# huangzh13/StyleGAN.pytorch

Hardware: AMD Instinct MI355X
Metric: img/s full G+D train step, 1024x1024 depth-9 bf16 (higher is better)
Workload: dtype bf16; 1 GPU; ffhq1024: StyleGAN 1024x1024, progressive depth index 8, logistic+R1, alpha 0.5, batch 4/GPU, global batch 4; global_batch=4, parallelism=dp1

## Files before the change

include/sgx.h:

```cpp
#ifndef SGX_H
#define SGX_H
#include <stddef.h>
#include <stdint.h>
#ifdef __cplusplus
extern "C" {
#endif

enum { SGX_F32 = 0, SGX_BF16 = 1 };
enum { SGX_ACT_NONE = 0, SGX_ACT_LRELU = 1, SGX_ACT_RELU = 2 };
enum { SGX_EINVAL = -1, SGX_EUNSUPPORTED = -2, SGX_EWORKSPACE = -3 };

int sgx_version(void);
const char* sgx_last_error(void);
int sgx_clear_error(void);
int sgx_stream_wait_stream(void* waiter, void* signaler);
int sgx_selftest_tr16(void* out256, void* stream);

int sgx_prof_start(int mode, int only_of);
int sgx_prof_count(void);
int sgx_prof_get(int i, char* name, int name_cap, float* ms, double* flops, double* bytes, char* desc, int desc_cap);

int sgx_conv3x3(const void* x, const void* w, const float* bias, void* y, int B, int H, int W, int Cin, int Cout,
                int act, const void* mask, int dtype, void* stream);
int sgx_conv4x4s2_down(const void* x, const void* w, const float* bias, void* y, int B, int H, int W, int Cin,
                       int Cout, int act, int dtype, void* stream);
int sgx_conv4x4s2_up(const void* x, const void* w, void* y, int B, int H, int W, int Cin, int Cout, int dtype,
                     void* stream);
int sgx_conv_variant(int geo, const void* x, const void* w, const float* bias, void* y, int B, int H, int W, int Cin, int Cout,
                     int act, int dtype, int variant, void* stream);
size_t sgx_conv_splitk_ws_bytes(int geo, int B, int H, int W, int Cin, int Cout, int dtype);
int sgx_conv_splitk(int geo, const void* x, const void* w, const float* bias, void* y, const void* mask, int B, int H, int W, int Cin, int Cout,
                    int act, int dtype, void* ws, size_t ws_bytes, void* stream);

int sgx_conv_config(int geo, int B, int H, int W, int Cin, int Cout, int dtype, int* cfg5);
enum { SGX_PACK_S = 0, SGX_PACK_D = 1, SGX_PACK_U = 2, SGX_PACK_UF = 3 };
int sgx_pack_weight(const float* w, void* fwd, void* adj, int O, int I, int Ipad, int mode, float scale, int dtype,
                    void* stream);
#define SGX_PACK_ROW 10
int sgx_pack_weight_blocks(int O, int Ipad);
int sgx_pack_weight_multi(const void* table, int n, int total_blocks, int dtype, void* stream);
size_t sgx_wgrad_ws_bytes(int taps, int B, int H, int W, int Ck, int Cn);
int sgx_wgrad3x3_param(const void* x, const void* dy, float* dW, float* db, void* ws, size_t ws_bytes, int B, int H, int W,
                       int Cx, int Cdy, int adjoint, float scale, int O, int I, int accumulate, int dtype, void* stream);
int sgx_wgrad4x4s2_param(const void* fine, const void* coarse, float* dW, float* db, void* ws, size_t ws_bytes, int B, int H,
                         int W, int Cfine, int Ccoarse, int mode, float scale, int O, int I, int accumulate, int dtype,
                         void* stream);

int sgx_bias_act(const void* x, const float* bias, float bscale, void* y, size_t npix, int C, int act, int dtype,
                 void* stream);
int sgx_lrelu_bwd(const void* dy, const void* y, void* dx, size_t n, float slope, float scale, const float* scale_dev, int dtype,
                  void* stream);
int sgx_lrelu_bwd_bits(const void* dy, const void* bits, void* dx, size_t n, float slope, float scale, const float* scale_dev, int dtype,
                       void* stream);
int sgx_conv4x4s2_down_fade_ok(int B, int H, int W, int Cin, int Cout, int dtype);
int sgx_conv4x4s2_down_fade(const void* x, const void* w, const float* bias, const void* resid, float alpha, float beta, const float* ab_dev,
                            void* y, void* bits, int B, int H, int W, int Cin, int Cout, int dtype, void* stream);
int sgx_conv4x4s2_down_fade_rgb(const void* x, const void* w, const float* bias, const float* pimg, const float* wr, float ws, const float* rb,
                                float bs1, float bs2, float alpha, float beta, const float* ab_dev, void* y, void* bits, int B, int H, int W,
                                int Cin, int Cout, int dtype, void* stream);
size_t sgx_fade_rgb_bwd_ws_bytes(size_t npix, int C);
int sgx_fade_rgb_bwd(const void* g, const void* bits, const float* pimg, const float* wr, float ws, float bs, float alpha, float beta,
                     const float* ab_dev, void* gy, float* dwr, float* drb, int acc, float* gpimg, void* wsbuf, size_t ws_bytes, size_t npix, int C,
                     int dtype, void* stream);
int sgx_fade_rgb_bwd_finish(const void* wsbuf, size_t ws_bytes, size_t npix, int C, float ws, float bs, float beta, const float* ab_dev,
                            float* dwr, float* drb, int acc, void* stream);
int sgx_fade_rgb_bwd2(const void* ggy, const float* ggp, const void* bits, const float* wr, float ws, float alpha, float beta, const float* ab_dev,
                      void* out, size_t npix, int C, int dtype, void* stream);
int sgx_axpby(const void* a, const void* b, void* out, float alpha, float beta, size_t n, int dtype, void* stream);
int sgx_axpby_dev(const void* a, const void* b, void* out, const float* alpha_dev, const float* beta_dev, size_t n, int dtype,
                  void* stream);
int sgx_blur3x3(const void* x, void* y, int B, int H, int W, int C, int dtype, void* stream);
int sgx_blur3x3_act(const void* x, const void* z, void* y, int B, int H, int W, int C, int mode, int dtype, void* stream);
int sgx_blur3x3_bits(const void* x, const void* bits, void* y, int B, int H, int W, int C, int mode, int dtype, void* stream);
int sgx_blur_kxk(const void* x, void* y, const float* taps_host, int K, int pad, int B, int IH, int IW, int OH, int OW, int C,
                 int dtype, void* stream);
int sgx_images_u8_to_nhwc(const void* src, void* dst, const int* flip, int B, int H, int W, int src_chw, int dtype, void* stream);
int sgx_pool2(const void* x, void* y, int B, int H, int W, int C, float scale, int dtype, void* stream);
int sgx_up2(const void* x, void* y, int B, int H, int W, int C, float scale, int dtype, void* stream);
int sgx_up2_add(const void* x, const void* a, void* y, int B, int H, int W, int C, float scale, int dtype, void* stream);
size_t sgx_colsum_ws_bytes(size_t npix, int C);
int sgx_colsum(const void* x, float* out, float scale, void* ws, size_t ws_bytes, size_t npix, int C, int dtype,
               void* stream);

int sgx_rgb_in(const float* img, const float* w, int sj, int sc, float wscale, const float* bias, void* y, size_t npix,
               int C, int dtype, void* stream);
int sgx_rgb_out(const void* x, const float* w, int sj, int sc, float wscale, const float* bias, float* img, size_t npix,
                int C, int dtype, void* stream);
int sgx_rgb_in_add(const float* img, const float* w, int sj, int sc, float wscale, const void* add, void* y, size_t npix, int C, int dtype,
                   void* stream);
size_t sgx_rgb_wgrad_ws_bytes(size_t npix, int C);
int sgx_downsample_fade_rgb(const float* x, float* out, int B, int H, int W, float alpha, float beta, const float* ab_dev, void* stream);
size_t sgx_diffaug_ws_bytes(int B, int H, int W);
int sgx_diffaug(const float* x, float* y, const float* u, int B, int H, int W, int policy_bits, int adjoint, int with_bias, void* ws,
                size_t ws_bytes, void* stream);
int sgx_ada_gates(const float* gu, const float* state, int policy_bits, int* img_bits, int B, void* stream);
int sgx_diffaug_gated(const float* x, float* y, const float* u, const int* img_bits, int B, int H, int W, int policy_bits, int adjoint,
                      int with_bias, void* ws, size_t ws_bytes, void* stream);
int sgx_ada_update(const float* real_logits, int B, float* state, float target, float adjust_per_image, int interval, void* stream);
int sgx_rgb_out_fade(const void* x, const float* w, int sj, int sc, float wscale, const float* bias, const float* low, float alpha,
                     float beta, const float* ab_dev, float* img, int B, int H, int W, int C, int dtype, void* stream);
int sgx_rgb_wgrad(const float* img, const void* f, float* dw, int sj, int sc, float wscale, void* ws, size_t ws_bytes,
                  size_t npix, int C, int dtype, void* stream);

enum { SGX_EPI_ACT = 1, SGX_EPI_NORM = 2 };
size_t sgx_gepi_ws_bytes(int B, int HW, int C);
int sgx_gepi_fwd(const void* x, const float* bias, const float* noise, const float* nw, const float* style, void* y,
                 float* mean, float* rstd, void* ws, size_t ws_bytes, const double* pre_part, int pre_npart, int B, int HW,
                 int C, int flags, int dtype, void* stream);
int sgx_blur3x3_stats_nparts(int B, int H, int W, int C, int dtype);
int sgx_conv3x3_stats_nparts(int B, int H, int W, int Cin, int Cout, int dtype);
int sgx_conv3x3_signbits_ok(int B, int H, int W, int Cin, int Cout, int dtype);
int sgx_conv3x3_signbits(const void* x, const void* w, const float* bias, void* y, void* bits, int B, int H, int W, int Cin, int Cout,
                         int act, const void* mask, int dtype, void* stream);
int sgx_conv4x4s2_up_blur_ok(int B, int H, int W, int Cin, int Cout, int dtype);
int sgx_conv4x4s2_up_blur(const void* x, const void* w, void* y, const void* mask, int B, int H, int W, int Cin, int Cout,
                          int dtype, void* stream);
int sgx_pack_upblur(const float* w, void* wc, int O, int I, int mode, int adjoint, float scale, void* stream);
int sgx_conv_upblur_ok(int B, int H, int W, int Cin, int Cout, int dtype);
int sgx_conv_upblur(const void* x, const void* wc, void* y, const void* maskbits, int B, int H, int W, int Cin, int Cout, int dtype, void* stream);
int sgx_conv4x4s2_up_blur_bits(const void* x, const void* w, void* y, const void* bits, int B, int H, int W, int Cin, int Cout,
                               int dtype, void* stream);
int sgx_conv3x3_stats(const void* x, const void* w, void* y, const float* ebias, const float* noise, const float* nw, double* part,
                      size_t part_bytes, int B, int H, int W, int Cin, int Cout, int dtype, void* stream);

int sgx_rgbconv_ok(int B, int H, int W, int C, int dtype);
int sgx_rgbconv_pack(const float* w0, float s0, const float* wr, float sr, const float* br, float bscale, void* wf, void* wd, int C,
                     void* stream);
int sgx_rgbconv_fwd(const float* img, const void* wf, const float* b0, void* y, void* bits, int B, int H, int W, int C, int epi, int ones,
                    int dtype, void* stream);
int sgx_rgbconv_tune(int fwd_variant, int nit, int dbg);
int sgx_rgbconv_dgrad(const void* gz, const void* wd, float* gi, int B, int H, int W, int C, int dtype, void* stream);
size_t sgx_rgbconv_wgrad_ws_bytes(int B, int H, int W, int C);
int sgx_rgbconv_wgrad(const float* img, const void* gz, int ones, const float* w0, float s0, const float* wr, float sr, const float* br,
                      float bscale, float* dw0, float* db0, float* dwr, float* dbr, int acc, void* ws, size_t ws_bytes, int B, int H, int W,
                      int C, int dtype, void* stream);
int sgx_blur3x3_stats(const void* x, void* y, const float* bias, const float* noise, const float* nw, double* part,
                      size_t part_bytes, int B, int H, int W, int C, int act, int dtype, void* stream);
int sgx_gepi_bwd(const void* dy, const void* x, const float* bias, const float* noise, const float* nw,
                 const float* style, const float* mean, const float* rstd, void* dx, float* dstyle, float* dnw,
                 float* dbias, void* ws, size_t ws_bytes, int B, int HW, int C, int flags, int dtype, void* stream);

int sgx_pixelnorm_fwd(const float* x, float* y, int B, int C, void* stream);
int sgx_pixelnorm_bwd(const float* dy, const float* x, float* dx, int B, int C, void* stream);
int sgx_mbstd_fwd(const void* x, void* y, int B, int HW, int C, int Cpad, int dtype, void* stream);
int sgx_mbstd_bwd(const void* dy, const void* x, void* dx, int B, int HW, int C, int Cpad, int dtype, void* stream);
int sgx_mbstd_bwd2(const void* ggx, const void* dy, const void* x, void* ddy, void* gx, int B, int HW, int C, int Cpad,
                   int dtype, void* stream);
size_t sgx_sumsq_ws_bytes(void);
int sgx_sumsq_f32(const float* x, size_t n, void* ws, size_t ws_bytes, float* out, void* stream);
int sgx_scale_dev_f32(const float* x, const float* s, float alpha, float* out, size_t n, void* stream);
int sgx_logistic_loss(const float* fake, int n_fake, const float* real, int n_real, float scale, int generator, float* loss,
                      float* g_fake, float* g_real, void* stream);
size_t sgx_gemm_ws_bytes(int M, int N, int K);
int sgx_gemm_f32(const float* A, const float* Bm, float* C, int M, int N, int K, int ta, int tb, float alpha,
                 void* ws, size_t ws_bytes, void* stream);
int sgx_linear_fwd(const float* x, const float* w, const float* bias, float* y, int B, int N, int K, float w_mul, float b_mul,
                   int act, void* stream);
int sgx_linear_bwd_data(const float* gy, const float* y_act, const float* w, float* gx, int B, int N, int K, float w_mul,
                        void* stream);
int sgx_linear_bwd_param(const float* gy, const float* y_act, const float* x, float* dw, float* db, int B, int N, int K, float w_mul,
                         float b_mul, void* stream);
#define SGX_STYLE_ROW 8
int sgx_style_fwd(const float* lm, const void* table, float* y, int G, int B, int D, int total_tiles, void* stream);
int sgx_style_bwd_data(const float* gy, const void* table, float* glm, int G, int B, int D, int max_n, void* stream);
int sgx_style_bwd_param(const float* gy, const float* lm, const void* table, float* dw, float* db, int G, int B, int D,
                        int total_tiles, void* stream);

int sgx_gepi_stats(const void* x, const float* bias, const float* noise, const float* nw, float* mean, float* rstd, void* ws, size_t ws_bytes,
                   const double* pre_part, int pre_npart, int B, int HW, int C, int flags, int dtype, void* stream);
int sgx_rgb_out_epi(const void* y, const float* ebias, const float* noise, const float* nw, const float* style, const float* mean,
                    const float* rstd, const float* w, int sj, int sc, float wscale, const float* rbias, const float* low, float alpha, float beta,
                    const float* ab_dev, float* img, int B, int H, int W, int C, int dtype, void* stream);
size_t sgx_rgb_wgrad_epi_ws_bytes(int B, int HW, int C);
int sgx_rgb_wgrad_epi(const void* y, const float* g, const float* ebias, const float* noise, const float* nw, const float* style, const float* mean,
                      const float* rstd, float* dw, float* db, int sj, int sc, float scale, float bscale, void* ws, size_t ws_bytes, int B, int HW,
                      int C, int dtype, void* stream);

int sgx_adam_multi(float* const* params, const float* const* grads, float* const* exp_avg, float* const* exp_avg_sq,
                   const int64_t* sizes, int n, float beta1, float beta2, float eps, const float* step_sizes,
                   const float* bc2_sqrts, const float* grad_scale, void* stream);
int sgx_ema_multi(float* const* tgt, const float* const* src, const int64_t* sizes, int n, float beta, void* stream);
int sgx_gradnorm_clip_coef(const float* const* grads, const int64_t* sizes, int n, float max_norm, double* partial,
                           float* out, void* stream);

#ifdef __cplusplus
}
#endif
#endif
```

stylegan/pytorch_amd/GAN.py:

```python
import contextlib
import copy
import datetime
import os
import random
import time
import timeit
from collections import OrderedDict

import numpy as np
import torch
import torch.nn as nn

from . import Losses
from . import functional as F
from .Blocks import DiscriminatorBlock, DiscriminatorTop, GSynthesisBlock, InputBlock
from .CustomLayers import EqualizedConv2d, EqualizedLinear, PixelNormLayer, Truncation, act_code, apply_act
from .data import get_data_loader
from . import native
from .native import ACT_LRELU
from .optim import FusedAdam, clip_and_step, ema_update


class DeferredLoss:

# ... 490 lines not shown
        if isinstance(loss, str):
            loss = loss.lower()
            mean_scale = 1.0 / self.dp.world_size if self.dp is not None else 1.0
            if self.conditional:
                assert loss in ["conditional-loss"]
                return Losses.ConditionalGANLoss(self.dis, mean_scale=mean_scale)
            assert loss in ["logistic", "hinge", "standard-gan", "relativistic-hinge"], "Unknown loss function"
            if loss == "logistic":
                return Losses.LogisticGAN(self.dis, mean_scale=mean_scale)
            if loss == "hinge":
                return Losses.HingeGAN(self.dis, mean_scale=mean_scale)
            if loss == "standard-gan":
                return Losses.StandardGAN(self.dis, mean_scale=mean_scale)
            return Losses.RelativisticAverageHingeGAN(self.dis, mean_scale=mean_scale,
                                                      batch_mean=self.dp.global_mean if self.dp is not None else None)
        return loss

    def progressive_down_sampling(self, real_batch, depth, alpha):
        if self.structure == 'fixed':
            return real_batch
        x = F.nhwc(real_batch, torch.float32)
        levels = self.depth - depth - 1
        for _ in range(levels):
            x = F.call(F.Pool2Fn, x, 0.25)
        if depth > 0:
            if FUSE_RGB_FADE and x.shape[3] == 3 and x.dtype == torch.float32 and not x.requires_grad:
                x = F.downsample_fade_rgb(x, alpha)
            else:
                prior = F.call(F.Up2Fn, F.call(F.Pool2Fn, x, 0.25), 1.0)
                x = F.fade(x, prior, alpha)
        else:
            x = F.fade(x, x, alpha)
        return F.nchw_view(x)

    _StyleGAN__progressive_down_sampling = progressive_down_sampling

    def _zero_grads(self, kind, depth):
        optim = self.dis_optim if kind == "d" else self.gen_optim
        optim.zero_grad()
        gb = self._grad_buckets.get((kind, int(depth))) if self.dp is not None else None
        if gb is not None:
            gb.attach()

    def _sched_begin(self, kind, depth, param_stream):
        from . import dist as D
        self.__dict__["_sched_active"] = None
        if self.dp is None or not self.dp.overlap_buckets or torch.cuda.is_current_stream_capturing():
            return
        if F.GRAD_NOTE is None:
            F.GRAD_NOTE = D.note_grad_write
        net = self.dis if kind == "d" else self.gen
        if not net.__dict__.get("_sgx_grad_hooks"):
            D.install_grad_hooks(net.parameters())
            net.__dict__["_sgx_grad_hooks"] = True
        scheds = self.__dict__.setdefault("_bucket_scheds", {})
        key = (kind, int(depth))
        sched = scheds.get(key)
        gb = self._grad_buckets.get(key)
        if sched is None or (not sched.recording and (gb is None or sched.gb is not gb or not gb.attached())):
            sched = scheds[key] = D.BucketScheduler(self.dp)
        if not sched.recording:
            sched.begin(param_stream)
        self.__dict__["_sched_active"] = sched
        D.set_active_scheduler(sched)

    def _sched_abort(self):
        if self.dp is not None:
            from . import dist as D
            D.set_active_scheduler(None)
            self.__dict__["_sched_active"] = None

    def _note_active_grads(self, kind, depth):
        if self.dp is None:
            return
        from . import dist as D
        D.set_active_scheduler(None)
        sched = self.__dict__.get("_sched_active")
        net = self.dis if kind == "d" else self.gen
        active = [p for p in net.parameters() if p.grad is not None]
        gb = self._grad_buckets.get((kind, int(depth)))
        recorded = sched is not None and sched.recording
        if active and (gb is None or not gb.matches(active) or recorded) and not torch.cuda.is_current_stream_capturing():
            for key in [k for k in self._grad_buckets if k[0] == kind and k[1] != int(depth)
                        and not any(g.depth == k[1] and g.graph is not None for g in self._step_graphs.values())]:
                del self._grad_buckets[key]
                self.__dict__.get("_bucket_scheds", {}).pop(key, None)
            new = None
            if sched is not None and sched.recording:
                new = sched.layout(self.dp.bucket_elems, only=active, canonical=list(net.parameters()))
                if new is None or not new.matches(active):
                    new = None
                    self.__dict__.get("_bucket_scheds", {}).pop((kind, int(depth)), None)
            self._grad_buckets[(kind, int(depth))] = new if new is not None else D.GradBuckets(active, self.dp.bucket_elems)
            self.__dict__["_sched_active"] = None

    def _aux_stream(self):
        if not self.aux_stream:
            return None
        st = self.__dict__.get("_aux_compute_stream")
        if st is None:
            st = self.__dict__["_aux_compute_stream"] = torch.cuda.Stream(device=self.device)
            quiet = getattr(torch.autograd.graph, "set_warn_on_accumulate_grad_stream_mismatch", None)
            if quiet is not None:
                quiet(False)
        return st

    def _param_stream(self, two_branches=False):
        if not self.param_stream:
            return torch.cuda.current_stream() if two_branches else None
        st = self.__dict__.get("_param_side_stream")
        if st is None:
            st = self.__dict__["_param_side_stream"] = torch.cuda.Stream(device=self.device)
        return st

    def _graphable(self, labels):
        return (self.use_graphs and labels is None and self.d_repeats == 1 and self.structure == "linear"
                and (self.dp is None or (self.gen.truncation is None
                                         and not isinstance(self.loss, Losses.RelativisticAverageHingeGAN))))

    def _d_grads(self, noise, real_batch, depth, alpha, labels=None):
        real_samples = self.progressive_down_sampling(real_batch, depth, alpha)

        def make_fakes():
            self._wait_update("g")
            with torch.no_grad():
                out = self.gen(noise, depth, alpha, labels)
            return out

        aux = self._aux_stream()
        lazy = isinstance(self.loss, Losses.LogisticGAN)
        self._wait_update("d")
        if aux is not None and lazy:
            self.dis.prepack(depth, (real_samples.shape[0], real_samples.shape[2], real_samples.shape[3], real_samples.shape[1]))
            cur = torch.cuda.current_stream()
            aux.wait_stream(cur)
            with torch.cuda.stream(aux):
                f_preds = self.dis(make_fakes(), depth, alpha)

            def fake_logits():
                cur.wait_stream(aux)
                f_preds.record_stream(cur)
                return f_preds
            loss = self.loss.dis_loss(real_samples, None, depth, alpha, fake_logits=fake_logits)
        elif self.conditional:
            loss = self.loss.dis_loss(real_samples, make_fakes(), labels, depth, alpha)
        else:
            loss = self.loss.dis_loss(real_samples, make_fakes if lazy else make_fakes(), depth, alpha)
        if self._ada_on():
            self.dis.ada_step()
        self._zero_grads("d", depth)
        side = self._param_stream(two_branches=aux is not None and lazy)
        self._sched_begin("d", depth, side)
        try:
            with F.accumulate_param_grads(), F.param_grad_stream(side):
                loss.backward()
        except BaseException:
            self._sched_abort()
            raise
        if side is not None:
            torch.cuda.current_stream().wait_stream(side)
        self._note_active_grads("d", depth)
        return loss.detach()

    def _reduce(self, kind):
        if self.dp is None:
            return
        sched = self.__dict__.pop("_sched_active", None)
        if sched is not None and not sched.recording and sched.gb is not None and sched.gb.attached():
            try:
                sched.finish()
            except RuntimeError:
                for key in [k for k, v in self.__dict__.get("_bucket_scheds", {}).items() if v is sched]:
                    self._bucket_scheds.pop(key, None)
                    self._grad_buckets.pop(key, None)
                raise
            self.__dict__["_last_sched"] = sched
            return
        gb = next((g for (k, _), g in self._grad_buckets.items() if k == kind and g.attached()), None)
        if gb is not None:
            self.dp.all_reduce_buckets(gb)
        else:
            self.dp.all_reduce_grads((self.dis if kind == "d" else self.gen).parameters())

    def _d_reduce(self):
        self._reduce("d")

    def _d_update(self):
        self.dis_optim.step()

    def _g_grads(self, noise, real_batch, depth, alpha, labels=None):
        real_samples = None
        if not isinstance(self.loss, (Losses.LogisticGAN, Losses.HingeGAN, Losses.StandardGAN, Losses.ConditionalGANLoss)):
            real_samples = self.progressive_down_sampling(real_batch, depth, alpha)
        self._wait_update("g")
        fake_samples = self.gen(noise, depth, alpha, labels)
        self._wait_update("d")
        d_all = self.__dict__.get("_sgx_dis_params")
        if d_all is None:
            d_all = self.__dict__["_sgx_dis_params"] = list(self.dis.parameters())
        d_params = [p for p in d_all if p.requires_grad]
        for p in d_params:
            p.requires_grad_(False)
        try:
            if self.conditional:
                loss = self.loss.gen_loss(real_samples, fake_samples, labels, depth, alpha)
            else:
                loss = self.loss.gen_loss(real_samples, fake_samples, depth, alpha)
            self._zero_grads("g", depth)
            side = self._param_stream()
            self._sched_begin("g", depth, side)
            try:
                with F.accumulate_param_grads(), F.param_grad_stream(side):
                    loss.backward()
            except BaseException:
                self._sched_abort()
                raise
            if side is not None:
                torch.cuda.current_stream().wait_stream(side)
            self._note_active_grads("g", depth)
        finally:
            for p in d_params:
                p.requires_grad_(True)
        return loss.detach()

    def _g_reduce(self):
        self._reduce("g")

    def _g_update(self):
        clip_and_step(self.gen_optim, max_norm=10.)
        if self.use_ema:
            self.ema_updater(self.gen_shadow, self.gen, self.ema_decay)

    def _async_update(self, kind, loss):
        upd = self.__dict__.get("_update_stream")
        if upd is None:
            upd = self.__dict__["_update_stream"] = torch.cuda.Stream(device=self.device)
        upd.wait_stream(torch.cuda.current_stream())
        with torch.cuda.stream(upd):
            (self._d_reduce if kind == "d" else self._g_reduce)()
            loss.record_stream(upd)
            loss = self.dp.all_reduce_scalar(loss)
            (self._d_update if kind == "d" else self._g_update)()
        ev = torch.cuda.Event()
        ev.record(upd)
        self.__dict__.setdefault("_pending_updates", {})[kind] = ev
        self.__dict__["_loss_stream"] = upd
        return loss

    def _wait_update(self, kind):
        ev = self.__dict__.get("_pending_updates", {}).pop(kind, None)
        if ev is not None:
            torch.cuda.current_stream().wait_event(ev)

    def _d_body(self, noise, real_batch, depth, alpha, labels=None):
        loss = self._d_grads(noise, real_batch, depth, alpha, labels)
        if self.dp is not None and not torch.cuda.is_current_stream_capturing():
            return self._async_update("d", loss)
        self._d_reduce()
        self._d_update()
        return loss

    def _g_body(self, noise, real_batch, depth, alpha, labels=None):
        loss = self._g_grads(noise, real_batch, depth, alpha, labels)
        if self.dp is not None and not torch.cuda.is_current_stream_capturing():
            return self._async_update("g", loss)
        self._g_reduce()
        self._g_update()
        return loss

    def _graphed(self, kind, noise, real_batch, depth, alpha):
        self._wait_update("d"); self._wait_update("g")
        key = (kind, int(depth), tuple(noise.shape), tuple(real_batch.shape), tuple(real_batch.stride()), real_batch.dtype,
               self.aux_stream, self.param_stream,
               self.dis._diffaug_bits, self.dis.training,
               None if self.dis.diffaug_override is None else self.dis.diffaug_override.data_ptr(),
               (self.dis.ada_target, self.dis.ada_interval, self.dis.ada_kimg) if self._ada_on() else None,
               None if not self._ada_on() or self.dis.ada_gate_override is None else self.dis.ada_gate_override.data_ptr())
        g = self._step_graphs.get(key)
        if g is None:
            g = self._step_graphs[key] = _StepGraph(self, kind, depth)
        return g.run(noise, real_batch, alpha)

    deferred_losses = False

    alpha_on_device = False

    def _alpha_arg(self, alpha):
        if not self.alpha_on_device or isinstance(alpha, torch.Tensor):
            return alpha
        return native.upload(torch.tensor([float(alpha), 1.0 - float(alpha)], dtype=torch.float32), self.device)[0]

    def _loss_out(self, deferred):
        return deferred if self.deferred_losses else deferred.item()

    def optimize_discriminator(self, noise, real_batch, depth, alpha, labels=None):
        if self._graphable(labels):
            return self._loss_out(self._graphed("d", noise, real_batch, depth, alpha))
        loss_val = None
        alpha = self._alpha_arg(alpha)
        for _ in range(self.d_repeats):
            loss = self._d_body(noise, real_batch, depth, alpha, labels)
            if loss_val is not None and self.__dict__.get("_loss_stream") is not None:
                torch.cuda.current_stream().wait_stream(self.__dict__.pop("_loss_stream"))
            loss_val = loss if loss_val is None else loss_val + loss
        return self._loss_out(DeferredLoss(loss_val, 1.0 / self.d_repeats, stream=self.__dict__.pop("_loss_stream", None)))

    def optimize_generator(self, noise, real_batch, depth, alpha, labels=None):
        if self._graphable(labels):
            return self._loss_out(self._graphed("g", noise, real_batch, depth, alpha))
        loss = self._g_body(noise, real_batch, depth, self._alpha_arg(alpha), labels)
        return self._loss_out(DeferredLoss(loss, stream=self.__dict__.pop("_loss_stream", None)))

    @staticmethod
    def fade_point_of(fade_in_percentage, epochs, total_batches):
        return int((fade_in_percentage / 100) * epochs * total_batches)

    @staticmethod
    def alpha_at(ticker, fade_point):
        return ticker / fade_point if ticker <= fade_point else 1

    @staticmethod
    def is_feedback_batch(i, total_batches, feedback_factor):
        return i % int(total_batches / feedback_factor + 1) == 0 or i == 1

    @staticmethod
    def is_checkpoint_epoch(epoch, epochs, checkpoint_factor):
        return epoch % checkpoint_factor == 0 or epoch == 1 or epoch == epochs

    @staticmethod
    def create_grid(samples, scale_factor, img_file):
        samples = samples.detach().float().cpu()
        if scale_factor > 1:
            samples = torch.nn.functional.interpolate(samples, scale_factor=scale_factor)
        n, c, h, w = samples.shape
        nrow = max(1, int(np.sqrt(n)))
        ncol = (n + nrow - 1) // nrow
        pad = 1
        grid = torch.full((c, ncol * (h + pad) + pad, nrow * (w + pad) + pad), 128.0)
        for k in range(n):
            t = samples[k]
            lo, hi = float(t.min()), float(t.max())
            t = (t - lo) / max(hi - lo, 1e-5)
            y, x = (k // nrow) * (h + pad) + pad, (k % nrow) * (w + pad) + pad
            grid[:, y:y + h, x:x + w] = t
        try:
            from PIL import Image
            arr = grid.mul(255).add_(0.5).clamp_(0, 255).permute(1, 2, 0).to(torch.uint8).numpy()
            Image.fromarray(arr[:, :, 0] if c == 1 else arr).save(img_file)
        except ImportError:
            torch.save(grid, img_file + ".pt")

    train_graphs = {"0": False, "1": True}.get(os.environ.get("SGX_TRAIN_GRAPHS", "auto"), "auto")

    def train(self, dataset, num_workers, epochs, batch_sizes, fade_in_percentage, logger, output,
              num_samples=36, start_depth=0, feedback_factor=100, checkpoint_factor=1):
        assert self.depth <= len(epochs), "epochs not compatible with depth"
        assert self.depth <= len(batch_sizes), "batch_sizes not compatible with depth"
        assert self.depth <= len(fade_in_percentage), "fade_in_percentage not compatible with depth"
        self.gen.train()
        self.dis.train()
        if self.use_ema:
            self.gen_shadow.train()
        was_deferred, self.deferred_losses = self.deferred_losses, True
        was_graphs = getattr(self, "use_graphs", False)
        self.use_graphs = bool(was_graphs or self.train_graphs is True)
        self._train_forced_graphs = self.use_graphs
# ... 282 lines not shown
```

stylegan/pytorch_amd/csrc/conv.hip:

```cpp
#include "common.h"
#include <stdlib.h>

enum { G3X3 = 0, GDOWN = 1, GUP = 2, GUPA = 3 };
int sgx_wgrad2_plan(int geo, int B, int H, int W, int Ck, int Cn, int* nct_n, int* nct_k, int* kbw, int* ntiles);
int sgx_wgrad2_launch(int geo, const void* kside, const void* nside, float* ws, size_t ws_bytes, int B, int H, int W, int Ck, int Cn,
                      int want_bias, hipStream_t st, int* nsplit_out);
int sgx_conv2_try(int geo, const void* x, const void* w, const float* bias, void* y, int B, int H, int W, int Cin, int Cout, int act,
                  const void* mask, int variant, hipStream_t st, int* launched);
int sgx_conv2_takes(int geo, int B, int H, int W, int Cin, int Cout);

template <typename T, int KC> struct Frag;
template <> struct Frag<float, 16> {
    static constexpr int NK = 4;
    static constexpr int rowb_w() { return 68; }
    static constexpr int rowb_in(int) { return 68; }
    static constexpr bool swz_w() { return false; }
    static constexpr bool swz_in(int) { return false; }
    typedef float frag_t;
    static constexpr int pad_pw(int pw, int) { return pw; }
    __device__ static __forceinline__ int rd_off(int row, int rowb, bool, int q) { return row * rowb + q * 4; }
    __device__ static __forceinline__ frag_t ld(const char* p, int kk) { return *reinterpret_cast<const float*>(p + kk * 16); }
    __device__ static __forceinline__ f32x4 mma(frag_t a, frag_t b, f32x4 c) {
        return __builtin_amdgcn_mfma_f32_16x16x4f32(a, b, c, 0, 0, 0);
    }
    __device__ static __forceinline__ int lds_off(int row, int rowb, bool, int v) { return row * rowb + v * 16; }
    __device__ static __forceinline__ void lstore_at(char* p, uint4 val) {
        unsigned* d = reinterpret_cast<unsigned*>(p);
        d[0] = val.x; d[1] = val.y; d[2] = val.z; d[3] = val.w;
    }
};
template <> struct Frag<bf16_t, 32> {
    static constexpr int NK = 1;
    static constexpr int rowb_w() { return 64; }
    static constexpr int rowb_in(int is) { return is == 1 ? 64 : 80; }
    static constexpr bool swz_w() { return true; }
    static constexpr bool swz_in(int is) { return is == 1; }
    typedef bf16x8 frag_t;
    static constexpr int pad_pw(int pw, int is) { return is == 1 ? (pw + 7) / 8 * 8 : pw; }
    __device__ static __forceinline__ int rd_off(int row, int rowb, bool sw, int q) {
        return row * rowb + (sw ? (q ^ ((row >> 1) & 3)) : q) * 16;
    }
    __device__ static __forceinline__ frag_t ld(const char* p, int) { return *reinterpret_cast<const bf16x8*>(p); }
    __device__ static __forceinline__ f32x4 mma(frag_t a, frag_t b, f32x4 c) {
        return __builtin_amdgcn_mfma_f32_16x16x32_bf16(a, b, c, 0, 0, 0);
    }
    __device__ static __forceinline__ int lds_off(int row, int rowb, bool sw, int v) {
        return row * rowb + (sw ? (v ^ ((row >> 1) & 3)) : v) * 16;
    }
    __device__ static __forceinline__ void lstore_at(char* p, uint4 val) { *reinterpret_cast<uint4*>(p) = val; }
};
template <> struct Frag<bf16_t, 16> {
    static constexpr int NK = 1;
    static constexpr int rowb_w() { return 32; }
    static constexpr int rowb_in(int is) { return is == 1 ? 32 : 48; }
    static constexpr bool swz_w() { return true; }
    static constexpr bool swz_in(int is) { return is == 1; }
    typedef s16x4 frag_t;
    static constexpr int pad_pw(int pw, int is) { return is == 1 ? (pw + 15) / 16 * 16 : pw; }
    __device__ static __forceinline__ int rd_off(int row, int rowb, bool sw, int q) {
        const int half = sw ? ((q >> 1) ^ ((row >> 3) & 1)) : (q >> 1);
        return row * rowb + half * 16 + (q & 1) * 8;
    }
    __device__ static __forceinline__ frag_t ld(const char* p, int) { return *reinterpret_cast<const s16x4*>(p); }
    __device__ static __forceinline__ f32x4 mma(frag_t a, frag_t b, f32x4 c) {
        return __builtin_amdgcn_mfma_f32_16x16x16bf16_1k(a, b, c, 0, 0, 0);
    }
    __device__ static __forceinline__ int lds_off(int row, int rowb, bool sw, int v) {
        return row * rowb + (sw ? (v ^ ((row >> 3) & 1)) : v) * 16;
    }
    __device__ static __forceinline__ void lstore_at(char* p, uint4 val) { *reinterpret_cast<uint4*>(p) = val; }
};

struct ConvArgs {
    const void* x; const void* w; const float* bias; void* y;
    int B, H, W, OH, OW, OHc, OWc, Cin, Cout, act, tiles_x, tiles_y, ntiles;
    const void* mask;
    int dbg;
    int bands;
    int ksplit; float* kws;
};

template <int GEO> struct Geo;
template <> struct Geo<G3X3> { static constexpr int IS = 1, TK = 3, NCLS = 1; };
template <> struct Geo<GDOWN> { static constexpr int IS = 2, TK = 4, NCLS = 1; };
template <> struct Geo<GUP> { static constexpr int IS = 1, TK = 2, NCLS = 4; };
template <> struct Geo<GUPA> { static constexpr int IS = 1, TK = 3, NCLS = 1; };

#ifndef SGX_CONV_OCC_SMALL
#define SGX_CONV_OCC_SMALL 3
#endif
constexpr int conv_min_waves(int tsize, int CT, int BP, int GEO, int KC) {
    if (KC > 32) return 2;
    if (GEO == GUPA) return CT * BP >= 512 ? 1 : 2;
    if (GEO == GDOWN && tsize == 2 && KC == 16) return 3;
    if (CT * BP >= 1024 || GEO == GDOWN) return 1;
    if (tsize == 2 && CT * BP <= 256) return SGX_CONV_OCC_SMALL;
    return 2;
}
template <typename T>
constexpr bool conv_bands_ok(int GEO, int TH, int TW, int BP) {
    return sizeof(T) == 2 && (GEO == G3X3 || GEO == GUPA) && TH == 16 && TW == 16 && BP == 256;
}
template <typename T, int KC, int GEO, int TH, int TW, int BP, int CT, bool SK = false>
__global__ __launch_bounds__(256, conv_min_waves(sizeof(T), CT, BP, GEO, KC)) void conv_kernel(ConvArgs a) {
    constexpr int FK = (sizeof(T) == 2 && KC > 32) ? 32 : KC;
    constexpr int NPL = KC / FK;
    using F = Frag<T, FK>;
    constexpr int IS = Geo<GEO>::IS, TK = Geo<GEO>::TK, NT = TK * TK;
    constexpr int PH = (TH - 1) * IS + TK, PW = (TW - 1) * IS + TK, PWP = F::pad_pw(PW, IS);
    constexpr int NI = BP / (TH * TW), SPW = BP / 64, BCO = CT * 16;
    constexpr int VE = 16 / (int)sizeof(T), VPP = KC / VE, VPR = FK / VE;
    constexpr int ROWI = F::rowb_in(IS), ROWW = F::rowb_w();
    constexpr bool SWI = F::swz_in(IS), SWW = F::swz_w();
    constexpr bool UPA = GEO == GUPA;
    constexpr int NTW = UPA ? 16 : NT;
    constexpr int NCL = UPA ? 4 : 1;
    constexpr int IN_PLANE = (NI * PH * PWP * ROWI + 15) / 16 * 16, W_PLANE = NTW * BCO * ROWW;
    constexpr int IN_BYTES = NPL * IN_PLANE;
    extern __shared__ __attribute__((aligned(16))) char smem[];
    char* in_lds = smem;
    char* w_lds = smem + IN_BYTES;

    const int tid = threadIdx.x, lane = tid & 63, wave = tid >> 6, q = lane >> 4, l15 = lane & 15;
    const int co0 = blockIdx.y * BCO;
    int py = 0, px = 0;
    constexpr int NCLS_Z = Geo<GEO>::NCLS;
    if (GEO == GUP) { py = (SK ? (int)(blockIdx.z % NCLS_Z) : (int)blockIdx.z) >> 1; px = blockIdx.z & 1; }
    int split = 0, k_lo = 0, k_hi = a.Cin;
    if constexpr (SK) {
        const int nkc = a.Cin / KC;
        split = (int)blockIdx.z / NCLS_Z;
        k_lo = (split * nkc / a.ksplit) * KC; k_hi = ((split + 1) * nkc / a.ksplit) * KC;
    }
    constexpr int NIN = (NI * PH * PW * VPP + 255) / 256, NWT = (NTW * BCO * VPP + 255) / 256;
    int in_rel[NIN], in_pos[NIN], in_dst[NIN], w_rel[NWT];
    const int w_dst0 = ((tid % VPP) / VPR) * W_PLANE + F::lds_off(tid / VPP, ROWW, SWW, (tid % VPP) % VPR);
#pragma unroll
    for (int j = 0; j < NIN; ++j) {
        const int idx = tid + j * 256;
        const int v = idx % VPP, pixel = idx / VPP;
        const int il = pixel / (PH * PW), rem = pixel % (PH * PW);
        const int pr = rem / PW, pc = rem % PW;
        const bool in_range = idx < NI * PH * PW * VPP;
        in_rel[j] = ((il * a.H + pr) * a.W + pc) * a.Cin + v * VE;
        in_pos[j] = in_range ? ((il << 20) | (pr << 10) | pc) : -1;
        in_dst[j] = (v / VPR) * IN_PLANE + F::lds_off((il * PH + pr) * PWP + pc, ROWI, SWI, v % VPR);
    }
#pragma unroll
    for (int j = 0; j < NWT; ++j) {
        const int idx = tid + j * 256;
        const int v = idx % VPP, row = idx / VPP;
        const int n = row % BCO, t = row / BCO;
        int tg = t;
        if (GEO == GUP) tg = (3 - py - 2 * (t >> 1)) * 4 + (3 - px - 2 * (t & 1));
// ... 706 lines not shown
        for (int j = 0; j < NNV; ++j) {
            const int idx = tid + j * 256;
            if (idx < BP * (NCH / VE)) *reinterpret_cast<uint4*>(n_lds + (idx / (NCH / VE)) * NROW + (idx % (NCH / VE)) * 16) = rn[j];
        }
#pragma unroll
        for (int j = 0; j < NKV; ++j) {
            const int idx = tid + j * 256;
            if (idx < NI * PH * PW * (KCH / VE)) *reinterpret_cast<uint4*>(k_lds + (idx / (KCH / VE)) * KROW + (idx % (KCH / VE)) * 16) = rk[j];
        }
    };
    if ((int)blockIdx.y < a.ntiles) gload(blockIdx.y);
    for (int tile = blockIdx.y; tile < a.ntiles; tile += gridDim.y) {
        __syncthreads();
        lstore();
        __syncthreads();
        if (tile + (int)gridDim.y < a.ntiles) gload(tile + gridDim.y);
        if constexpr (TR) {
            for (int ks = 0; ks < BP / 32; ++ks) {
                int noff2[2], koff2[2];
#pragma unroll
                for (int h = 0; h < 2; ++h) {
                    const int m = ks * 32 + h * 16 + q * 4 + (l15 >> 2);
                    const int il = m / (TH * TW), r = (m / TW) % TH, c = m % TW;
                    noff2[h] = m * NROW + (l15 & 3) * 8;
                    koff2[h] = ((il * PH + r * IS) * PW + c * IS) * KROW + (l15 & 3) * 8;
                }
                bf16x8 fa8[NSUB];
#pragma unroll
                for (int ns = 0; ns < NSUB; ++ns)
                    fa8[ns] = cat8(lds_tr16(n_lds + noff2[0] + ns * 32), lds_tr16(n_lds + noff2[1] + ns * 32));
                if (do_bias) {
                    const bf16x8 one8 = cat8(WFrag<bf16_t>::ones(), WFrag<bf16_t>::ones());
#pragma unroll
                    for (int ns = 0; ns < NSUB; ++ns) bacc[ns] = __builtin_amdgcn_mfma_f32_16x16x32_bf16(fa8[ns], one8, bacc[ns], 0, 0, 0);
                }
#pragma unroll
                for (int i = 0; i < TPW; ++i) {
                    const int t = wave + 4 * i;
                    if (t < NT) {
                        const int toff = ((t / TK) * PW + (t % TK)) * KROW;
#pragma unroll
                        for (int kk = 0; kk < KSUB; ++kk) {
                            const bf16x8 fb8 = cat8(lds_tr16(k_lds + toff + koff2[0] + kk * 32), lds_tr16(k_lds + toff + koff2[1] + kk * 32));
#pragma unroll
                            for (int ns = 0; ns < NSUB; ++ns)
                                acc[i][ns][kk] = __builtin_amdgcn_mfma_f32_16x16x32_bf16(fa8[ns], fb8, acc[i][ns][kk], 0, 0, 0);
                        }
                    }
                }
            }
        } else
        for (int ks = 0; ks < BP / F::KPS; ++ks) {
            int noff[4], koff[4];
#pragma unroll
            for (int j = 0; j < PPL; ++j) {
                const int m = ks * F::KPS + q * PPL + j;
                const int il = m / (TH * TW), r = (m / TW) % TH, c = m % TW;
                noff[j] = m * NROW;
                koff[j] = ((il * PH + r * IS) * PW + c * IS) * KROW;
            }
            typename F::frag_t fa[NSUB];
#pragma unroll
            for (int ns = 0; ns < NSUB; ++ns) fa[ns] = F::load(n_lds, noff, q, ns * 16 + l15);
            if (do_bias) {
#pragma unroll
                for (int ns = 0; ns < NSUB; ++ns) bacc[ns] = F::mma(fa[ns], F::ones(), bacc[ns]);
            }
#pragma unroll
            for (int i = 0; i < TPW; ++i) {
                const int t = wave + 4 * i;
                if (t < NT) {
                    const int toff = ((t / TK) * PW + (t % TK)) * KROW;
#pragma unroll
                    for (int kk = 0; kk < KSUB; ++kk) {
                        typename F::frag_t fb = F::load(k_lds + toff, koff, q, kk * 16 + l15);
#pragma unroll
                        for (int ns = 0; ns < NSUB; ++ns) acc[i][ns][kk] = F::mma(fa[ns], fb, acc[i][ns][kk]);
                    }
                }
            }
        }
    }
    if (a.direct) {
        constexpr int KP = KCH + 1;
        float* accl = reinterpret_cast<float*>(smem);
        __syncthreads();
#pragma unroll
        for (int i = 0; i < TPW; ++i) {
            const int t = wave + 4 * i;
            if (t < NT) {
#pragma unroll
                for (int ns = 0; ns < NSUB; ++ns)
#pragma unroll
                    for (int kk = 0; kk < KSUB; ++kk)
#pragma unroll
                        for (int r = 0; r < 4; ++r) accl[(t * NCH + ns * 16 + q * 4 + r) * KP + kk * 16 + l15] = acc[i][ns][kk][r];
            }
        }
        __syncthreads();
        const float c = a.scale * (a.mode == SGX_PACK_D ? 0.25f : 1.f);
        for (int idx = tid; idx < NCH * KCH * 9; idx += 256) {
            const int tap = idx % 9, kl = (idx / 9) % KCH, nl = idx / (9 * KCH);
            const int n = n0 + nl, k = kc0 + kl;
            const int o = a.transposed ? k : n, i = a.transposed ? n : k;
            if (i >= a.I || o >= a.O) continue;
            float v;
            if (NT == 9) {
                v = accl[((a.flip_t ? 8 - tap : tap) * NCH + nl) * KP + kl];
            } else {
                const int y = tap / 3, x = tap % 3;
                const float* pp = accl + nl * KP + kl;
                v = (pp[(y * 4 + x) * NCH * KP] + pp[(y * 4 + x + 1) * NCH * KP]) +
                    (pp[((y + 1) * 4 + x) * NCH * KP] + pp[((y + 1) * 4 + x + 1) * NCH * KP]);
            }
            float* d = a.dw + ((size_t)o * a.I + i) * 9 + (a.mode == SGX_PACK_UF ? 8 - tap : tap);
            *d = (a.accumulate & 1) ? *d + c * v : c * v;
        }
        if (do_bias && l15 == 0) {
#pragma unroll
            for (int ns = 0; ns < NSUB; ++ns)
#pragma unroll
                for (int r = 0; r < 4; ++r) {
                    float* d = a.db + n0 + ns * 16 + q * 4 + r;
                    *d = (a.accumulate & 2) ? *d + bacc[ns][r] : bacc[ns][r];
                }
        }
        return;
    }
    float* out = a.out + (size_t)blockIdx.y * ((size_t)NT * a.Cn * a.Ck + a.Cn);
    if (do_bias && l15 == 0) {
#pragma unroll
        for (int ns = 0; ns < NSUB; ++ns)
#pragma unroll
            for (int r = 0; r < 4; ++r) out[(size_t)NT * a.Cn * a.Ck + n0 + ns * 16 + q * 4 + r] = bacc[ns][r];
    }
#pragma unroll
    for (int i = 0; i < TPW; ++i) {
        const int t = wave + 4 * i;
        if (t < NT) {
#pragma unroll
            for (int ns = 0; ns < NSUB; ++ns)
#pragma unroll
                for (int kk = 0; kk < KSUB; ++kk)
#pragma unroll
                    for (int r = 0; r < 4; ++r)
                        out[((size_t)t * a.Cn + n0 + ns * 16 + q * 4 + r) * a.Ck + kc0 + kk * 16 + l15] = acc[i][ns][kk][r];
        }
    }
}

struct FinishArgs { const float* ws; float* dw; float* db; int nsplit, O, I, Ip, mode, transposed, flip_t; float scale; int accumulate; };

template <int EPB>
__global__ __launch_bounds__(256) void wgrad_finish_kernel(FinishArgs f) {
    constexpr int NSL = 256 / EPB;
    __shared__ float red[NSL][EPB][9];
    const int pl = threadIdx.x % EPB, sl = threadIdx.x / EPB;
    const int A = f.transposed ? f.Ip : f.O, Bd = f.transposed ? f.O : f.Ip;
    const int e = blockIdx.x * EPB + pl;
    const int taps = f.mode == SGX_PACK_S ? 9 : 16;
    const size_t tstride = (size_t)f.O * f.Ip, total = (size_t)taps * tstride + A;
    if ((int)blockIdx.x >= (A * Bd + EPB - 1) / EPB) {
        const int o = ((int)blockIdx.x - (A * Bd + EPB - 1) / EPB) * EPB + pl;
        float b = 0.f;
        if (o < f.O)
            for (int s = sl; s < f.nsplit; s += NSL) b += f.ws[(size_t)s * total + (size_t)taps * tstride + o];
        red[sl][pl][0] = b;
        __syncthreads();
        if (sl == 0 && o < f.O) {
            float sum = 0.f;
            for (int l = 0; l < NSL; ++l) sum += red[l][pl][0];
            f.db[o] = (f.accumulate & 2) ? f.db[o] + sum : sum;
        }
        return;
    }
    float acc[9];
#pragma unroll
    for (int k = 0; k < 9; ++k) acc[k] = 0.f;
    if (e < A * Bd) {
#pragma unroll 4
        for (int s = sl; s < f.nsplit; s += NSL) {
            const float* p = f.ws + (size_t)s * total + e;
            if (f.mode == SGX_PACK_S) {
#pragma unroll
                for (int t = 0; t < 9; ++t) acc[t] += p[(size_t)(f.flip_t ? 8 - t : t) * tstride];
            } else {
                float v[16];
#pragma unroll
                for (int t = 0; t < 16; ++t) v[t] = p[(size_t)t * tstride];
#pragma unroll
                for (int y = 0; y < 3; ++y)
#pragma unroll
                    for (int x = 0; x < 3; ++x)
                        acc[y * 3 + x] += (v[y * 4 + x] + v[y * 4 + x + 1]) + (v[(y + 1) * 4 + x] + v[(y + 1) * 4 + x + 1]);
            }
        }
    }
#pragma unroll
    for (int k = 0; k < 9; ++k) red[sl][pl][k] = acc[k];
    __syncthreads();
    for (int t = threadIdx.x; t < EPB * 9; t += 256) {
        const int el = t / 9, k = t % 9;
        const int ee = blockIdx.x * EPB + el;
        if (ee >= A * Bd) continue;
        const int a = ee / Bd, bb = ee % Bd;
        const int o = f.transposed ? bb : a, i = f.transposed ? a : bb;
        if (i >= f.I) continue;
        float sum = 0.f;
#pragma unroll 8
        for (int l = 0; l < NSL; ++l) sum += red[l][el][k];
        const float c = f.scale * (f.mode == SGX_PACK_D ? 0.25f : 1.f);
        float* d = f.dw + ((size_t)o * f.I + i) * 9 + (f.mode == SGX_PACK_UF ? 8 - k : k);
        *d = (f.accumulate & 1) ? *d + c * sum : c * sum;
    }
}

static int wgrad_nsplit(int pairs, int ntiles, size_t elems_per_split) {
    static const int env_target = [] { const char* e = getenv("SGX_WGRAD_BLOCKS"); return e && atoi(e) > 0 ? atoi(e) : 0; }();
    static const int env_cap = [] { const char* e = getenv("SGX_WGRAD_MAXSPLIT"); return e && atoi(e) > 0 ? atoi(e) : 0; }();
    const bool tiny = elems_per_split <= (size_t)16 * 32 * 32;
    static const int env_mid = [] { const char* e = getenv("SGX_WGRAD_BLOCKS_MID"); return e && atoi(e) > 0 ? atoi(e) : 0; }();
    const int target = env_target ? env_target : (tiny ? 2048 : (env_mid ? env_mid : 512)), cap = env_cap ? env_cap : (tiny ? 1024 : 512);
    int want = (target + pairs - 1) / pairs;
    if (!env_target && pairs >= 512 && ntiles <= 64) want = 1;
    if (want > cap) want = cap;
    if (want > ntiles) want = ntiles;
    if (want < 1) want = 1;
    return want;
}

template <typename T, int GEO, int TH, int TW, int BP, int NSUB, int KSUB, bool TR>
static int launch_wgrad(WgradArgs& a, void* ws, size_t ws_bytes, int* nsplit_out, hipStream_t st) {
    using F = WFrag<T>;
    constexpr int IS = Geo<GEO>::IS, TK = Geo<GEO>::TK, NT = TK * TK;
    constexpr int PH = (TH - 1) * IS + TK, PW = (TW - 1) * IS + TK, NI = BP / (TH * TW);
    constexpr int OPER = BP * wgrad_pitch<T>(NSUB * 16, TR, 1) + NI * PH * PW * wgrad_pitch<T>(KSUB * 16, TR, IS);
    constexpr int FOLD = NT * NSUB * 16 * (KSUB * 16 + 1) * 4;
    constexpr int LDS = OPER > FOLD ? OPER : FOLD;
    static_assert(LDS <= 160 * 1024, "LDS budget");
    a.tiles_y = (a.Hn + TH - 1) / TH; a.tiles_x = (a.Wn + TW - 1) / TW;
    a.ntiles = ((a.B + NI - 1) / NI) * a.tiles_y * a.tiles_x;
    const int pairs = (a.Cn / (NSUB * 16)) * (a.Ck / (KSUB * 16));
    int nsplit = wgrad_nsplit(pairs, a.ntiles, (size_t)NT * a.Cn * a.Ck);
    const size_t total = (size_t)NT * a.Cn * a.Ck + a.Cn;
    size_t fit = ws_bytes / (total * sizeof(float));
    if ((size_t)nsplit > fit) nsplit = (int)fit;
    SGX_REQUIRE(nsplit >= 1, SGX_EWORKSPACE, "wgrad: workspace too small (%zu bytes, need >= %zu)", ws_bytes, total * sizeof(float));
    a.out = static_cast<float*>(ws);
    a.direct = (nsplit == 1 && a.dw != nullptr) ? 1 : 0;
    auto kern = wgrad_kernel<T, GEO, TH, TW, BP, NSUB, KSUB, TR>;
    sgx_lds_opt_in<wgrad_kernel<T, GEO, TH, TW, BP, NSUB, KSUB, TR>>(LDS);
    hipLaunchKernelGGL(kern, dim3(pairs, nsplit), dim3(256), LDS, st, a);
    SGX_LAUNCH_CHECK("wgrad_kernel");
    *nsplit_out = nsplit;
    return 0;
}

template <typename T, int GEO, int BP, int NSUB, int KSUB, bool TR>
static int wgrad_tile(WgradArgs& a, void* ws, size_t wsb, int* ns, hipStream_t st) {
    if (a.Hn >= 16 && a.Wn >= 16) return launch_wgrad<T, GEO, BP / 16, 16, BP, NSUB, KSUB, TR>(a, ws, wsb, ns, st);
    if (a.Hn >= 8 && a.Wn >= 8) return launch_wgrad<T, GEO, (BP >= 64 ? 8 : BP / 8), 8, BP, NSUB, KSUB, TR>(a, ws, wsb, ns, st);
    return launch_wgrad<T, GEO, (BP >= 16 ? 4 : BP / 4), 4, BP, NSUB, KSUB, TR>(a, ws, wsb, ns, st);
}

static bool wgrad_use_tr() {
    static const int v = [] { const char* e = getenv("SGX_WGRAD_TR"); return e ? atoi(e) : 1; }();
    return v != 0;
}

template <typename T, int GEO, int BP, bool TR = false>
static int wgrad_ch(WgradArgs& a, void* ws, size_t wsb, int* ns, hipStream_t st) {
    SGX_REQUIRE(a.Cn % 16 == 0 && a.Ck % 16 == 0, SGX_EUNSUPPORTED, "wgrad: channels must be multiples of 16");
    const bool n32 = a.Cn % 32 == 0, k32 = a.Ck % 32 == 0;
    if (GEO == GDOWN) {
        if (n32) return wgrad_tile<T, GEO, BP, 2, 1, TR>(a, ws, wsb, ns, st);
        return wgrad_tile<T, GEO, BP, 1, 1, TR>(a, ws, wsb, ns, st);
    }
    const long npix = (long)a.B * a.Hn * a.Wn;
    const bool lowres_big = npix <= 64L * BP && (long)(a.Cn / 32) * (a.Ck / 32) < 512 && (long)(a.Cn / 32) * (a.Ck / 16) >= 512;
    if (n32 && k32 && !lowres_big) return wgrad_tile<T, GEO, BP, 2, 2, TR>(a, ws, wsb, ns, st);
    if (n32) return wgrad_tile<T, GEO, BP, 2, 1, TR>(a, ws, wsb, ns, st);
    if (k32) return wgrad_tile<T, GEO, BP, 1, 2, TR>(a, ws, wsb, ns, st);
    return wgrad_tile<T, GEO, BP, 1, 1, TR>(a, ws, wsb, ns, st);
}

static int wgrad_pre_groups() { static const int v = [] { const char* e = getenv("SGX_WGRAD_PRE"); return e ? atoi(e) : 32; }(); return v; }
static int wgrad_pre_min() { static const int v = [] { const char* e = getenv("SGX_WGRAD_PRE_MIN"); return e ? atoi(e) : 256; }(); return v; }
__global__ __launch_bounds__(256) void wgrad_prereduce_kernel(const float* __restrict__ ws, float* __restrict__ out, size_t total4,
                                                              int nsplit) {
    const size_t e = (size_t)blockIdx.x * 256 + threadIdx.x;
    if (e >= total4) return;
    const int g = blockIdx.y, per = (nsplit + (int)gridDim.y - 1) / (int)gridDim.y;
    const int s0 = g * per, s1 = (s0 + per < nsplit) ? s0 + per : nsplit;
    float4 acc = make_float4(0.f, 0.f, 0.f, 0.f);
#pragma unroll 4
    for (int sp = s0; sp < s1; ++sp) {
        const float4 v = reinterpret_cast<const float4*>(ws)[(size_t)sp * total4 + e];
        acc.x += v.x; acc.y += v.y; acc.z += v.z; acc.w += v.w;
    }
    reinterpret_cast<float4*>(out)[(size_t)g * total4 + e] = acc;
}
static size_t wgrad_pre_bytes(size_t total_floats, int nsplit) {
    const int G = wgrad_pre_groups();
    return (G > 0 && nsplit >= wgrad_pre_min() && nsplit > G && total_floats % 4 == 0) ? (size_t)G * total_floats * sizeof(float) : 0;
}

static int wgrad_finish(const void* ws, float* dw, float* db, int nsplit, int O, int I, int Ip, int mode, int transposed, int flip_t,
                        float scale, int accumulate, hipStream_t st, size_t ws_bytes = 0) {
    {
        const size_t total = (size_t)(mode == SGX_PACK_S ? 9 : 16) * O * Ip + (transposed ? Ip : O);
        const size_t pre = wgrad_pre_bytes(total, nsplit), used = (size_t)nsplit * total * sizeof(float);
        if (pre && ws_bytes >= used + pre) {
            float* out = reinterpret_cast<float*>(const_cast<char*>(static_cast<const char*>(ws)) + used);
            hipLaunchKernelGGL(wgrad_prereduce_kernel, dim3((unsigned)((total / 4 + 255) / 256), wgrad_pre_groups()), dim3(256), 0, st,
                               static_cast<const float*>(ws), out, total / 4, nsplit);
            SGX_LAUNCH_CHECK("wgrad_prereduce_kernel");
            ws = out;
            nsplit = wgrad_pre_groups();
        }
    }
    FinishArgs f{static_cast<const float*>(ws), dw, db, nsplit, O, I, Ip, mode, transposed, flip_t, scale, accumulate};
    SGX_NOTE(0.0, 4.0 * ((double)nsplit * (mode == SGX_PACK_S ? 9 : 16) * O * Ip + 9.0 * O * I), "finish %dx%d m%d tr%d ns%d", O, I, mode, transposed, nsplit);
    const int ne = O * Ip, nb = db ? O : 0;
    if (ne / 64 >= 128) hipLaunchKernelGGL(wgrad_finish_kernel<64>, dim3((unsigned)((ne + 63) / 64 + (nb + 63) / 64)), dim3(256), 0, st, f);
    else if (ne / 16 >= 128) hipLaunchKernelGGL(wgrad_finish_kernel<16>, dim3((unsigned)((ne + 15) / 16 + (nb + 15) / 16)), dim3(256), 0, st, f);
    else if (ne / 8 >= 128) hipLaunchKernelGGL(wgrad_finish_kernel<8>, dim3((unsigned)((ne + 7) / 8 + (nb + 7) / 8)), dim3(256), 0, st, f);
    else hipLaunchKernelGGL(wgrad_finish_kernel<4>, dim3((unsigned)((ne + 3) / 4 + (nb + 3) / 4)), dim3(256), 0, st, f);
    SGX_LAUNCH_CHECK("wgrad_finish_kernel");
    return 0;
}

extern "C" size_t sgx_wgrad_ws_bytes(int taps, int B, int H, int W, int Ck, int Cn) {
    size_t total = ((size_t)taps * Ck * Cn + Cn) * sizeof(float);
    int pairs = (Ck / 32 > 0 ? Ck / 32 : 1) * (Cn / 32 > 0 ? Cn / 32 : 1);
    size_t ntiles = (size_t)B * ((H + 3) / 4) * ((W + 3) / 4);
    size_t ns = (size_t)wgrad_nsplit(pairs, ntiles > (1u << 30) ? (1 << 30) : (int)ntiles, (size_t)taps * Ck * Cn);
    size_t need = total * ns + wgrad_pre_bytes(total / sizeof(float), (int)ns);
    int a0, a1, a2, a3;
    const int ns2 = taps == 9 ? sgx_wgrad2_plan(0, B, H, W, Ck, Cn, &a0, &a1, &a2, &a3) : sgx_wgrad2_plan(1, B, H / 2, W / 2, Ck, Cn, &a0, &a1, &a2, &a3);
    const size_t need2 = ns2 ? total * ns2 + wgrad_pre_bytes(total / sizeof(float), ns2) : 0;
    return need > need2 ? need : need2;
}

extern "C" int sgx_wgrad3x3_param(const void* x, const void* dy, float* dW, float* db, void* ws, size_t ws_bytes, int B, int H,
                                  int W, int Cx, int Cdy, int adjoint, float scale, int O, int I, int accumulate, int dtype,
                                  void* stream) {
    hipStream_t st = (hipStream_t)stream;
    const int Ip = adjoint ? Cdy : Cx;
    SGX_REQUIRE(!db || !adjoint, SGX_EINVAL, "wgrad3x3_param: bias gradient asked of the adjoint launch");
    SGX_REQUIRE((adjoint ? Cx : Cdy) == O && Ip >= I, SGX_EINVAL, "wgrad3x3_param: channel mismatch (Cx=%d Cdy=%d O=%d I=%d adj=%d)", Cx, Cdy, O, I, adjoint);
    WgradArgs a{x, dy, nullptr, B, H, W, H, W, Cx, Cdy, 0, 0, 0, db ? 1 : 0,
                0, dW, db, O, I, SGX_PACK_S, adjoint, adjoint, accumulate, scale};
    SGX_NOTE(2.0 * 9 * Cx * Cdy * B * H * W, (dtype == SGX_F32 ? 4.0 : 2.0) * B * H * W * (Cx + Cdy), "wgradS B%d %dx%d %dx%d", B, H, W, Cx, Cdy);
    int ns = 0, rc;
    if (dtype == SGX_BF16) {
        rc = sgx_wgrad2_launch(0, x, dy, static_cast<float*>(ws), ws_bytes, B, H, W, Cx, Cdy, db ? 1 : 0, st, &ns);
        if (rc) return rc;
        if (ns) return wgrad_finish(ws, dW, db, ns, O, I, Ip, SGX_PACK_S, adjoint, adjoint, scale, accumulate, st, ws_bytes);
    }
    if (dtype == SGX_F32) rc = wgrad_ch<float, G3X3, 128>(a, ws, ws_bytes, &ns, st);
    else if (dtype == SGX_BF16) rc = wgrad_use_tr() ? wgrad_ch<bf16_t, G3X3, 128, true>(a, ws, ws_bytes, &ns, st) : wgrad_ch<bf16_t, G3X3, 128>(a, ws, ws_bytes, &ns, st);
    else { SGX_REQUIRE(false, SGX_EINVAL, "wgrad3x3_param: bad dtype"); }
    if (rc) return rc;
    if (a.direct) return 0;
    return wgrad_finish(ws, dW, db, ns, O, I, Ip, SGX_PACK_S, adjoint, adjoint, scale, accumulate, st, ws_bytes);
}

extern "C" int sgx_wgrad4x4s2_param(const void* fine, const void* coarse, float* dW, float* db, void* ws, size_t ws_bytes, int B,
                                    int H, int W, int Cfine, int Ccoarse, int mode, float scale, int O, int I, int accumulate,
                                    int dtype, void* stream) {
    hipStream_t st = (hipStream_t)stream;
    SGX_REQUIRE(H % 2 == 0 && W % 2 == 0, SGX_EINVAL, "wgrad4x4s2_param: odd fine size");
    SGX_REQUIRE(mode == SGX_PACK_D || mode == SGX_PACK_U || mode == SGX_PACK_UF, SGX_EINVAL, "wgrad4x4s2_param: bad mode %d", mode);
    const int transposed = mode != SGX_PACK_D;
    SGX_REQUIRE(!db || !transposed, SGX_EINVAL, "wgrad4x4s2_param: bias gradient only for mode D (dy is the coarse side)");
    SGX_REQUIRE(transposed ? (Ccoarse == I && Cfine == O) : (Ccoarse == O && Cfine == I), SGX_EINVAL,
                "wgrad4x4s2_param: channel mismatch (fine %d coarse %d O %d I %d mode %d)", Cfine, Ccoarse, O, I, mode);
    WgradArgs a{fine, coarse, nullptr, B, H, W, H / 2, W / 2, Cfine, Ccoarse, 0, 0, 0, db ? 1 : 0,
                0, dW, db, O, I, mode, transposed, 0, accumulate, scale};
    SGX_NOTE(2.0 * 16 * Cfine * Ccoarse * B * (H / 2) * (W / 2), (dtype == SGX_F32 ? 4.0 : 2.0) * B * H * W * (Cfine + Ccoarse / 4.0), "wgradD B%d fine%dx%d %dx%d", B, H, W, Cfine, Ccoarse);
    int ns = 0, rc;
    if (dtype == SGX_BF16) {
        rc = sgx_wgrad2_launch(1, fine, coarse, static_cast<float*>(ws), ws_bytes, B, H / 2, W / 2, Cfine, Ccoarse, db ? 1 : 0, st, &ns);
        if (rc) return rc;
        if (ns) return wgrad_finish(ws, dW, db, ns, O, I, I, mode, transposed, 0, scale, accumulate, st, ws_bytes);
    }
    if (dtype == SGX_F32) rc = wgrad_ch<float, GDOWN, 64>(a, ws, ws_bytes, &ns, st);
    else if (dtype == SGX_BF16) rc = wgrad_use_tr() ? wgrad_ch<bf16_t, GDOWN, 64, true>(a, ws, ws_bytes, &ns, st) : wgrad_ch<bf16_t, GDOWN, 64>(a, ws, ws_bytes, &ns, st);
    else { SGX_REQUIRE(false, SGX_EINVAL, "wgrad4x4s2_param: bad dtype"); }
    if (rc) return rc;
    if (a.direct) return 0;
    return wgrad_finish(ws, dW, db, ns, O, I, I, mode, transposed, 0, scale, accumulate, st, ws_bytes);
}

#define PACK_T 32
__device__ __forceinline__ float pack_tap(const float (*raw)[PACK_T][PACK_T + 1], int r, int il, int t, int mode, float scale) {
    if (mode == SGX_PACK_S) return scale * raw[t][r][il];
    const int ky = t >> 2, kx = t & 3;
    float v = 0.f;
#pragma unroll
    for (int a = 0; a < 2; ++a)
#pragma unroll
        for (int b = 0; b < 2; ++b) {
            const int y = ky - a, x = kx - b;
            if (y >= 0 && y < 3 && x >= 0 && x < 3) v += raw[mode == SGX_PACK_UF ? (2 - y) * 3 + (2 - x) : y * 3 + x][r][il];
        }
    return v * scale * (mode == SGX_PACK_D ? 0.25f : 1.f);
}
template <typename T>
__device__ __forceinline__ void pack_weight_tile(const float* __restrict__ w, T* __restrict__ fwd, T* __restrict__ adj, int O, int I,
                                                 int Ip, int mode, float scale, unsigned tile) {
    __shared__ float raw[9][PACK_T][PACK_T + 1];
    const int tiles_i = (Ip + PACK_T - 1) / PACK_T;
    const int o0 = (int)(tile / tiles_i) * PACK_T, i0 = (int)(tile % tiles_i) * PACK_T;
    const int ni = (I - i0 < PACK_T ? (I - i0 > 0 ? I - i0 : 0) : PACK_T);
    if (ni == PACK_T && (I * 9) % 4 == 0 && ((size_t)i0 * 9) % 4 == 0) {
        constexpr int PER = PACK_T * (PACK_T * 9 / 4) / 256;
        static_assert(PER * 256 == PACK_T * (PACK_T * 9 / 4), "a tile is a whole number of 16-byte loads per thread");
        float4 v[PER];
#pragma unroll
        for (int u = 0; u < PER; ++u) {
            const int idx = threadIdx.x + u * 256, r = idx / (PACK_T * 9 / 4), c4 = (idx % (PACK_T * 9 / 4)) * 4;
            v[u] = *reinterpret_cast<const float4*>(w + ((size_t)(o0 + r < O ? o0 + r : O - 1) * I + i0) * 9 + c4);
        }
#pragma unroll
        for (int u = 0; u < PER; ++u) {
            const int idx = threadIdx.x + u * 256, r = idx / (PACK_T * 9 / 4), c4 = (idx % (PACK_T * 9 / 4)) * 4;
            const bool ok = o0 + r < O;
            const float e[4] = {ok ? v[u].x : 0.f, ok ? v[u].y : 0.f, ok ? v[u].z : 0.f, ok ? v[u].w : 0.f};
#pragma unroll
            for (int j = 0; j < 4; ++j) raw[(c4 + j) % 9][r][(c4 + j) / 9] = e[j];
        }
    } else
    for (int idx = threadIdx.x; idx < PACK_T * PACK_T * 9; idx += blockDim.x) {
        const int r = idx / (PACK_T * 9), c = idx % (PACK_T * 9);
        const int il = c / 9, k = c % 9;
        float v = 0.f;
        if (o0 + r < O && il < ni) v = w[((size_t)(o0 + r) * I + i0) * 9 + c];
        raw[k][r][il] = v;
    }
    __syncthreads();
    const int taps = mode == SGX_PACK_S ? 9 : 16;
    constexpr int VE = 16 / (int)sizeof(T), VPR = PACK_T / VE;
    const bool full = (o0 + PACK_T <= O) && (i0 + PACK_T <= Ip) && (O % VE == 0) && (Ip % VE == 0);
    if (full) {
        for (int e = threadIdx.x; e < taps * PACK_T * VPR; e += blockDim.x) {
            const int t = e / (PACK_T * VPR), r = (e / VPR) % PACK_T, v = e % VPR;
            float val[VE];
#pragma unroll
            for (int j = 0; j < VE; ++j) val[j] = pack_tap(raw, r, v * VE + j, t, mode, scale);
            VecTraits<T>::store(fwd + ((size_t)t * O + o0 + r) * Ip + i0 + v * VE, val);
        }
        for (int e = threadIdx.x; e < taps * PACK_T * VPR; e += blockDim.x) {
            const int t = e / (PACK_T * VPR), il = (e / VPR) % PACK_T, v = e % VPR;
            const int ta = mode == SGX_PACK_S ? 8 - t : t;
            float val[VE];
#pragma unroll
            for (int j = 0; j < VE; ++j) val[j] = pack_tap(raw, v * VE + j, il, t, mode, scale);
            VecTraits<T>::store(adj + ((size_t)ta * Ip + i0 + il) * O + o0 + v * VE, val);
        }
        return;
    }
    for (int e = threadIdx.x; e < taps * PACK_T * PACK_T; e += blockDim.x) {
        const int t = e / (PACK_T * PACK_T), r = (e / PACK_T) % PACK_T, il = e % PACK_T;
        if (o0 + r < O && i0 + il < Ip)
            fwd[((size_t)t * O + o0 + r) * Ip + i0 + il] = from_f<T>(pack_tap(raw, r, il, t, mode, scale));
    }
    for (int e = threadIdx.x; e < taps * PACK_T * PACK_T; e += blockDim.x) {
        const int t = e / (PACK_T * PACK_T), il = (e / PACK_T) % PACK_T, r = e % PACK_T;
        const int ta = mode == SGX_PACK_S ? 8 - t : t;
        if (o0 + r < O && i0 + il < Ip)
            adj[((size_t)ta * Ip + i0 + il) * O + o0 + r] = from_f<T>(pack_tap(raw, r, il, t, mode, scale));
    }
}
static inline unsigned pack_tiles(int O, int Ip) { return (unsigned)(((O + PACK_T - 1) / PACK_T) * ((Ip + PACK_T - 1) / PACK_T)); }
template <typename T>
__global__ __launch_bounds__(256) void pack_weight_kernel(const float* __restrict__ w, T* __restrict__ fwd, T* __restrict__ adj, int O,
                                                          int I, int Ip, int mode, float scale) {
    pack_weight_tile<T>(w, fwd, adj, O, I, Ip, mode, scale, blockIdx.x);
}
template <typename T>
// ... 36 lines not shown
```

stylegan/pytorch_amd/functional.py:

```python
import contextlib
import functools
import os
import weakref

import numpy as np
import torch
from torch.autograd import Function
from torch.autograd.function import once_differentiable

from . import native as N

_DATA_GRAD_ONLY = 0


@contextlib.contextmanager
def data_grad_only():
    global _DATA_GRAD_ONLY
    _DATA_GRAD_ONLY += 1
    try:
        yield
    finally:
        _DATA_GRAD_ONLY -= 1


def _c(t):
    return t if t.is_contiguous() else t.contiguous()


class _NoGradCtx:
    needs_input_grad = (False,) * 16
    saved_tensors = ()

    def save_for_backward(self, *tensors):
        pass

    def mark_non_differentiable(self, *tensors):
        pass

    def set_materialize_grads(self, value):
        pass


def call(fn, *args):
    if torch.is_grad_enabled():
        for a in args:
            if isinstance(a, torch.Tensor) and a.requires_grad:
                return fn.apply(*args)
    return fn.forward(_NoGradCtx(), *args)


_bcall = call if os.environ.get("SGX_BWD_BYPASS", "1") != "0" else (lambda fn, *args: fn.apply(*args))


MODES = {"S": N.PACK_S, "D": N.PACK_D, "U": N.PACK_U, "UF": N.PACK_UF}
FWD_GEO = {"S": "S", "D": "D", "U": "U", "UF": "U"}
ADJ_GEO = {"S": "S", "D": "U", "U": "D", "UF": "D"}
_PACKS = {}
GRAD_NOTE = None
_WEIGHT_GEN = 0
_ACCUM_PARAM_GRADS = False
_PARAM_GRAD_STREAM = None


@contextlib.contextmanager
def param_grad_stream(stream):
    global _PARAM_GRAD_STREAM
    prev, _PARAM_GRAD_STREAM = _PARAM_GRAD_STREAM, stream
    try:
        yield
    finally:
        _PARAM_GRAD_STREAM = prev


_FAST_FORK = os.environ.get("SGX_FAST_FORK", "1") != "0"
_STREAMS = {}
_set_stream = torch._C._cuda_setStream if hasattr(torch._C, "_cuda_setStream") else None


def _stream_of(raw):
    st = _STREAMS.get(raw)
    if st is None:
        st = _STREAMS[raw] = torch.cuda.current_stream()
        assert st.cuda_stream == raw
    return st


def _param_grads(mode, adjoint, x, gy, weight, scale, want_bias, into):
    side = _PARAM_GRAD_STREAM
    if side is None:
        return _wgrad_param(mode, adjoint, x, gy, weight, scale, want_bias, into)
    if not _FAST_FORK:
        cur = torch.cuda.current_stream()
        side.wait_stream(cur)
        with torch.cuda.stream(side):
            dW, db = _wgrad_param(mode, adjoint, x, gy, weight, scale, want_bias, into)
        for t in (x, gy):
            t.record_stream(side)
        for t in (dW, db):
            if t is not None:
                t.record_stream(cur)
        return dW, db
    cur_raw = N.stream()
    if side.cuda_stream == cur_raw:
        return _wgrad_param(mode, adjoint, x, gy, weight, scale, want_bias, into)
    cur = _stream_of(cur_raw)
    N.check(N.lib().sgx_stream_wait_stream(side.cuda_stream, cur_raw), "sgx_stream_wait_stream")
    _set_stream(stream_id=side.stream_id, device_index=side.device_index, device_type=side.device_type)
    try:
        dW, db = _wgrad_param(mode, adjoint, x, gy, weight, scale, want_bias, into)
    finally:
        _set_stream(stream_id=cur.stream_id, device_index=cur.device_index, device_type=cur.device_type)
    x.record_stream(side); gy.record_stream(side)
    dW.record_stream(cur)
    if db is not None:
        db.record_stream(cur)
    return dW, db


def _fork_to(side, cur_raw, launch, reads=(), fresh=()):
    if not _FAST_FORK or _set_stream is None:
        cur = torch.cuda.current_stream()
        side.wait_stream(cur)
        with torch.cuda.stream(side):
            launch()
    else:
        cur = _stream_of(cur_raw)
        N.check(N.lib().sgx_stream_wait_stream(side.cuda_stream, cur_raw), "sgx_stream_wait_stream")
        _set_stream(stream_id=side.stream_id, device_index=side.device_index, device_type=side.device_type)
        try:
            launch()
        finally:
            _set_stream(stream_id=cur.stream_id, device_index=cur.device_index, device_type=cur.device_type)
    for t in reads:
        t.record_stream(side)
    for t in fresh:
        t.record_stream(cur)


@contextlib.contextmanager
def accumulate_param_grads():
    global _ACCUM_PARAM_GRADS
    prev, _ACCUM_PARAM_GRADS = _ACCUM_PARAM_GRADS, True
    try:
        yield
    finally:
        _ACCUM_PARAM_GRADS = prev


def bump_weight_generation(params=None):
    global _WEIGHT_GEN
    if params is None:
        _WEIGHT_GEN += 1
        return
    for p in params:
        p._sgx_gen = getattr(p, "_sgx_gen", 0) + 1


def _pack_tag(weight):
    return (weight._version, _WEIGHT_GEN, getattr(weight, "_sgx_gen", 0), weight.data_ptr())


def _pack_alloc(weight, sub):
    mode, _, ipad, dtype = sub
    taps = 9 if mode == "S" else 16
    O = weight.shape[0]
    return (torch.empty((taps, O, ipad), dtype=dtype, device=weight.device), torch.empty((taps, ipad, O), dtype=dtype, device=weight.device))


def _pack_mark():
    ev = torch.cuda.Event()
    ev.record()
    raw = N.stream()
    return (ev, raw, {raw})


def prepack(weights):
    rows, blk, dtype, touched = [], 0, None, []
    for w in weights:
        ent = _PACKS.get(id(w))
        if ent is None or ent[0]() is not w or not ent[3]:
            continue
        tag = _pack_tag(w)
        if ent[1] == tag:
            continue
        if w.dtype != torch.float32 or not w.is_contiguous():
            raise N.SgxError("parameters must be contiguous fp32")
        ent[1], ent[2] = tag, {}
        touched.append(ent)
        for sub in ent[3]:
            if dtype is None:
                dtype = sub[3]
            if sub[3] != dtype:
                continue
            fwd, adj = _pack_alloc(w, sub)
            ent[2][sub] = (fwd, adj)
            O, I = w.shape[0], w.shape[1]
            nb = ((O + 31) // 32) * ((sub[2] + 31) // 32)
            rows.append([w.data_ptr(), fwd.data_ptr(), adj.data_ptr(), O, I, sub[2], MODES[sub[0]],
                         int(np.float32(sub[1]).view(np.uint32)), blk, nb])
            blk += nb
    if rows:
        table, _ = N.upload(torch.tensor(rows, dtype=torch.int64), weights[0].device)
        N.check(N.lib().sgx_pack_weight_multi(N.ptr(table), len(rows), blk, N.F32 if dtype == torch.float32 else N.BF16, N.stream()),
                "sgx_pack_weight_multi")
        if not N.capturing():
            table.record_stream(torch.cuda.current_stream())
        mark = _pack_mark()
        for ent in touched:
            ent[4] = mark


def packs(weight, mode, scale, ipad, dtype):
    key = id(weight)
    ent = _PACKS.get(key)
    tag = _pack_tag(weight)
    if ent is None or ent[0]() is not weight:
        ent = [weakref.ref(weight, lambda _r, k=key: _PACKS.pop(k, None)), tag, {}, set(), None]
        _PACKS[key] = ent
    elif ent[1] != tag:
        ent[1], ent[2] = tag, {}
    sub = (mode, float(scale), int(ipad), dtype)
    ent[3].add(sub)
    got = ent[2].get(sub)
    if got is not None and ent[4] is not None:
        raw = N.stream()
        if raw not in ent[4][2] or (not _FAST_FORK and raw != ent[4][1]):
            _stream_of(raw).wait_event(ent[4][0])
            ent[4][2].add(raw)
    if got is None:
        w = _c(weight.detach())
        if w.dtype != torch.float32:
            raise N.SgxError("parameters must be fp32")
        O, I = w.shape[0], w.shape[1]
        fwd, adj = _pack_alloc(w, sub)
        N.check(N.lib().sgx_pack_weight(N.ptr(w), N.ptr(fwd), N.ptr(adj), O, I, ipad, MODES[mode], float(scale),
                                        N.F32 if dtype == torch.float32 else N.BF16, N.stream()), "sgx_pack_weight")
        got = (fwd, adj)
        ent[2][sub] = got
        ent[4] = _pack_mark()
    return got


def clear_pack_cache():
    for ent in _PACKS.values():
        ent[1], ent[2] = None, {}
    _UPBLUR_PACKS.clear()


_UPBLUR_PACKS = {}


def upblur_pack(weight, mode, scale, ipad, adjoint):
    key = (id(weight), mode, float(scale), int(ipad), bool(adjoint))
    tag = _pack_tag(weight)
    ent = _UPBLUR_PACKS.get(key)
    if ent is not None and ent[0]() is weight and ent[1] == tag:
        raw = N.stream()
        if raw not in ent[3][2] or (not _FAST_FORK and raw != ent[3][1]):
            _stream_of(raw).wait_event(ent[3][0])
            ent[3][2].add(raw)
        return ent[2]
    w = _c(weight.detach())
    if w.dtype != torch.float32 or int(ipad) != w.shape[1]:
        raise N.SgxError("conv+blur composite pack: contiguous fp32 parameter without channel padding expected")
    O, I = w.shape[0], w.shape[1]
    Nn, K = (I, O) if adjoint else (O, I)
    wc = torch.empty(((9 * 4 + 22 * 2) * Nn * K,), dtype=torch.bfloat16, device=w.device)
    N.check(N.lib().sgx_pack_upblur(N.ptr(w), N.ptr(wc), O, I, MODES[mode], int(bool(adjoint)), float(scale) / 16.0, N.stream()), "sgx_pack_upblur")
    _UPBLUR_PACKS[key] = [weakref.ref(weight, lambda _r, k=key: _UPBLUR_PACKS.pop(k, None)), tag, wc, _pack_mark()]
    return wc


@functools.lru_cache(maxsize=None)
def _splitk_ws_bytes(gi, B, H, W, Cin, Cout, dt):
    return int(N.lib().sgx_conv_splitk_ws_bytes(gi, B, H, W, Cin, Cout, dt))


def _conv_launch(geo, x, wq, bias, act, mask=None):
    B, H, W, Cin = x.shape
    taps, Cout, K = wq.shape
    if K != Cin:
        raise N.SgxError(f"conv: weight pack expects {K} input channels, activation has {Cin}")
    L = N.lib()
    gi = "SDU".index(geo)
    wsb = _splitk_ws_bytes(gi, B, H, W, Cin, Cout, N.dt(x))
    if wsb:
        oh, ow = (H, W) if geo == "S" else ((H // 2, W // 2) if geo == "D" else (2 * H, 2 * W))
        y = torch.empty((B, oh, ow, Cout), dtype=x.dtype, device=x.device)
        if mask is not None and (geo != "S" or mask.shape != y.shape or mask.dtype != y.dtype):
            raise N.SgxError("conv: the output mask must have the output's shape and dtype (3x3 geometry)")
        ws = N.workspace(wsb, x.device)
        N.check(L.sgx_conv_splitk(gi, N.ptr(x), N.ptr(wq), N.ptr(bias), N.ptr(y), N.ptr(mask), B, H, W, Cin, Cout, act, N.dt(x), N.ptr(ws), wsb, N.stream()),
                "sgx_conv_splitk")
        return y
    if geo == "S":
        y = torch.empty((B, H, W, Cout), dtype=x.dtype, device=x.device)
        if mask is not None and (mask.shape != y.shape or mask.dtype != y.dtype):
            raise N.SgxError("conv: the output mask must have the output's shape and dtype")
        N.check(L.sgx_conv3x3(N.ptr(x), N.ptr(wq), N.ptr(bias), N.ptr(y), B, H, W, Cin, Cout, act, N.ptr(mask), N.dt(x), N.stream()), "sgx_conv3x3")
    elif geo == "D":
        assert mask is None
        y = torch.empty((B, H // 2, W // 2, Cout), dtype=x.dtype, device=x.device)
        N.check(L.sgx_conv4x4s2_down(N.ptr(x), N.ptr(wq), N.ptr(bias), N.ptr(y), B, H, W, Cin, Cout, act, N.dt(x), N.stream()), "sgx_conv4x4s2_down")
    else:
        assert bias is None and act == 0 and mask is None
        y = torch.empty((B, 2 * H, 2 * W, Cout), dtype=x.dtype, device=x.device)
        N.check(L.sgx_conv4x4s2_up(N.ptr(x), N.ptr(wq), N.ptr(y), B, H, W, Cin, Cout, N.dt(x), N.stream()), "sgx_conv4x4s2_up")
    return y


def _wgrad_param(mode, adjoint, x, gy, weight, scale, want_bias=False, into=None):
    L = N.lib()
    O, I = weight.shape[0], weight.shape[1]
    acc_w = into is not None and into[0] is not None
    acc_b = want_bias and into is not None and into[1] is not None
    dW = into[0] if acc_w else torch.empty((O, I, 3, 3), dtype=torch.float32, device=x.device)
    db = (into[1] if acc_b else torch.empty((O,), dtype=torch.float32, device=x.device)) if want_bias else None
    acc = (1 if acc_w else 0) | (2 if acc_b else 0)
    B = x.shape[0]
    if mode == "S":
        _, H, W, Cx = x.shape
        Cdy = gy.shape[3]
        wsb = L.sgx_wgrad_ws_bytes(9, B, H, W, Cx, Cdy)
        ws = N.workspace(wsb, x.device)
        N.check(L.sgx_wgrad3x3_param(N.ptr(x), N.ptr(gy), N.ptr(dW), N.ptr(db), N.ptr(ws), wsb, B, H, W, Cx, Cdy, int(adjoint),
                                     float(scale), O, I, acc, N.dt(x), N.stream()), "sgx_wgrad3x3_param")
        return dW, db
    launched = ADJ_GEO[mode] if adjoint else FWD_GEO[mode]
    fine, coarse = (x, gy) if launched == "D" else (gy, x)
    _, H, W, Cf = fine.shape
    Cc = coarse.shape[3]
    wsb = L.sgx_wgrad_ws_bytes(16, B, H, W, Cf, Cc)
    ws = N.workspace(wsb, x.device)
    N.check(L.sgx_wgrad4x4s2_param(N.ptr(fine), N.ptr(coarse), N.ptr(dW), N.ptr(db), N.ptr(ws), wsb, B, H, W, Cf, Cc, MODES[mode],
                                   float(scale), O, I, acc, N.dt(x), N.stream()), "sgx_wgrad4x4s2_param")
    return dW, db


class ConvFn(Function):

    @staticmethod
    def forward(ctx, x, weight, bias, mode, scale, ipad, adjoint, act, mask=None, defer_act=False, x_masked=False, stats=None,
                x_pre=None, bits_out=False, x_pre_bits=None):
        x = _c(x)
        fwd, adj = packs(weight, mode, scale, ipad, x.dtype)
        geo = ADJ_GEO[mode] if adjoint else FWD_GEO[mode]
        ctx.cfg = (mode, scale, ipad, adjoint, act, bias is not None, bool(defer_act), bool(x_masked))
        ctx.bias_ref = weakref.ref(bias) if bias is not None else (lambda: None)
        ctx.set_materialize_grads(False)
        if bits_out:
            assert geo == "S" and not adjoint and stats is None
            y, bits = _conv_bits_launch(x, fwd, None if bias is None else _c(bias.detach()), act, mask)
            ctx.mark_non_differentiable(bits)
            ctx.save_for_backward(x, weight, y if (act and not defer_act) else None, mask, x_pre, x_pre_bits)
            return y, bits
        if stats is not None:
            assert geo == "S" and not adjoint and bias is None and act == 0 and mask is None
            y, part = _conv_stats_launch(x, fwd, *stats)
            ctx.mark_non_differentiable(part)
            ctx.save_for_backward(x, weight, None, None, x_pre, x_pre_bits)
            return y, part
        y = _conv_launch(geo, x, adj if adjoint else fwd, None if bias is None else _c(bias.detach()), act, mask)
        ctx.save_for_backward(x, weight, y if (act and not defer_act) else None, mask, x_pre, x_pre_bits)
        return y

    @staticmethod
    def backward(ctx, gy, _gpart=None):
        if gy is None:
            return (None,) * 15
        x, weight, y, mask, x_pre, xb = ctx.saved_tensors[:6]
        mode, scale, ipad, adjoint, act, has_bias, defer_act, x_masked = ctx.cfg
        gy = _c(gy)
        if mask is not None:
            gy = _bcall(LReluBwdFn, gy, mask, 0.2, 1.0)
        if act and not defer_act:
            gy = _bcall(LReluBwdFn, gy, y, 0.2, 1.0)
        gx = gw = gb = None
        if ctx.needs_input_grad[0]:
            if x_pre is not None or xb is not None:
                assert not x_masked
                cout_b = weight.shape[1] if not adjoint else weight.shape[0]
                if xb is not None and conv_upblur_ok(gy, cout_b, mode, not adjoint):
                    gx = _bcall(ConvBlurFn, gy, weight, mode, scale, ipad, not adjoint, None, xb)
                elif x_pre is not None and conv_blur_ok(gy, cout_b, mode, not adjoint, has_mask_tensor=True):
                    gx = _bcall(ConvBlurFn, gy, weight, mode, scale, ipad, not adjoint, x_pre)
                else:
                    gx = _bcall(BlurMaskFn, _bcall(ConvFn, gy, weight, None, mode, scale, ipad, not adjoint, 0), x_pre, xb)
            else:
                gx = _bcall(ConvFn, gy, weight, None, mode, scale, ipad, not adjoint, 0, x if x_masked else None, False, False)
        if not _DATA_GRAD_ONLY:
            want_b = has_bias and ctx.needs_input_grad[2]
            fuse_b = want_b and ctx.needs_input_grad[1] and not adjoint and mode in ("S", "D")
            if ctx.needs_input_grad[1] and _ACCUM_PARAM_GRADS and weight.is_leaf and not torch.is_grad_enabled():
                bias = ctx.bias_ref() if fuse_b else None
                if fuse_b and (bias is None or not bias.is_leaf):
                    fuse_b, bias = False, None
                dW, db = _param_grads(mode, adjoint, _c(x), gy, weight, scale, fuse_b, (weight.grad, bias.grad if fuse_b else None))
                if weight.grad is None:
                    weight.grad = dW
                if fuse_b:
                    if bias.grad is None:
                        bias.grad = db
                    want_b = False
                if GRAD_NOTE is not None:
                    GRAD_NOTE(weight)
                    if fuse_b:
                        GRAD_NOTE(bias)
            elif ctx.needs_input_grad[1]:
                gw, gb = _bcall(WgradFn, x, gy, weight, mode, scale, adjoint, fuse_b)
            if want_b and not fuse_b:
                gb = _bcall(ColSumFn, gy, 1.0)
        return gx, gw, gb, None, None, None, None, None, None, None, None, None, None, None, None


CONV_BLUR_POLICY = os.environ.get("SGX_CONV_UP_BLUR_POLICY", "auto")
CONV_BLUR_MIN_PIXELS = 1 << 22


def conv_upblur_ok(x, cout, mode, adjoint):
    geo = ADJ_GEO[mode] if adjoint else FWD_GEO[mode]
    if CONV_BLUR_POLICY == "off" or not CONV_UPBLUR or geo != "U" or x.dtype != torch.bfloat16:
        return False
    B, H, W, Cin = x.shape
    return bool(N.lib().sgx_conv_upblur_ok(B, H, W, Cin, int(cout), N.BF16))


CONV_UPBLUR = os.environ.get("SGX_CONV_UPBLUR", "1") != "0"


def conv_blur_ok(x, cout, mode, adjoint, has_mask_tensor=False):
    geo = ADJ_GEO[mode] if adjoint else FWD_GEO[mode]
    if CONV_BLUR_POLICY == "off" or geo != "U" or x.dtype != torch.bfloat16:
        return False
    if not has_mask_tensor and conv_upblur_ok(x, cout, mode, adjoint):
        return True
    B, H, W, Cin = x.shape
    if CONV_BLUR_POLICY == "auto" and not (int(cout) == 16 and B * H * W >= CONV_BLUR_MIN_PIXELS):
        return False
    return bool(N.lib().sgx_conv4x4s2_up_blur_ok(B, H, W, Cin, int(cout), N.BF16))


class ConvBlurFn(Function):

    @staticmethod
    def forward(ctx, x, weight, mode, scale, ipad, adjoint, z=None, zbits=None):
        x = _c(x)
        geo = ADJ_GEO[mode] if adjoint else FWD_GEO[mode]
        assert geo == "U"
        B, H, W, Cin = x.shape
        cout_ = weight.shape[1] if adjoint else weight.shape[0]
        if z is None and conv_upblur_ok(x, cout_, mode, adjoint):
            if zbits is not None and (tuple(zbits.shape) != (B, 2 * H, 2 * W, cout_ // 8) or zbits.dtype != torch.uint8):
                raise N.SgxError("conv+blur: sign bits [B, 2H, 2W, Cout/8] uint8 expected")
            wc = upblur_pack(weight, mode, scale, ipad, adjoint)
            y = torch.empty((B, 2 * H, 2 * W, cout_), dtype=x.dtype, device=x.device)
            N.check(N.lib().sgx_conv_upblur(N.ptr(x), N.ptr(wc), N.ptr(y), N.ptr(None if zbits is None else _c(zbits)), B, H, W, Cin, cout_, N.dt(x),
                                            N.stream()), "sgx_conv_upblur")
            ctx.cfg = (mode, scale, ipad, adjoint, 0, False, False, False)
            ctx.bias_ref = lambda: None
            ctx.save_for_backward(x, weight, None, None, None, None, None, zbits)
            return y
        fwd, adj = packs(weight, mode, scale / 16.0, ipad, x.dtype)
        wq = adj if adjoint else fwd
        taps, Cout, K = wq.shape
        if K != Cin:
            raise N.SgxError(f"conv+blur: weight pack expects {K} input channels, activation has {Cin}")
        y = torch.empty((B, 2 * H, 2 * W, Cout), dtype=x.dtype, device=x.device)
        if z is not None and (z.shape != y.shape or z.dtype != y.dtype):
            raise N.SgxError("conv+blur: the mask must have the output's shape and dtype")
        if zbits is not None:
            if tuple(zbits.shape) != (B, 2 * H, 2 * W, Cout // 8) or zbits.dtype != torch.uint8:
                raise N.SgxError("conv+blur: sign bits [B, 2H, 2W, Cout/8] uint8 expected")
            N.check(N.lib().sgx_conv4x4s2_up_blur_bits(N.ptr(x), N.ptr(wq), N.ptr(y), N.ptr(_c(zbits)), B, H, W, Cin, Cout, N.dt(x), N.stream()),
                    "sgx_conv4x4s2_up_blur_bits")
        else:
            N.check(N.lib().sgx_conv4x4s2_up_blur(N.ptr(x), N.ptr(wq), N.ptr(y), N.ptr(None if z is None else _c(z)), B, H, W, Cin, Cout,
                                                  N.dt(x), N.stream()), "sgx_conv4x4s2_up_blur")
        ctx.cfg = (mode, scale, ipad, adjoint, 0, False, False, False)
        ctx.bias_ref = lambda: None
        ctx.save_for_backward(x, weight, None, None, None, None, z, zbits)
        return y

    @staticmethod
    def backward(ctx, gg):
        gg = _c(gg)
        z, zbits = ctx.saved_tensors[6:8]
        masked = z is not None or zbits is not None
        m = _bcall(MaskBlurFn, gg, z, zbits) if masked else _bcall(BlurFn, gg)
# ... 57 lines not shown
    bits = torch.empty((B, H, W, Cout // 8), dtype=torch.uint8, device=x.device)
    N.check(N.lib().sgx_conv3x3_signbits(N.ptr(x), N.ptr(wq), N.ptr(bias), N.ptr(y), N.ptr(bits), B, H, W, Cin, Cout, act, N.ptr(mask),
                                         N.dt(x), N.stream()), "sgx_conv3x3_signbits")
    return y, bits


def conv_stats_nparts(x, cout):
    if x.dtype != torch.bfloat16:
        return 0
    B, H, W, Cin = x.shape
    return N.lib().sgx_conv3x3_stats_nparts(B, H, W, Cin, int(cout), N.BF16)


def _conv_stats_launch(x, wq, ebias, noise, nw):
    B, H, W, Cin = x.shape
    taps, Cout, K = wq.shape
    if K != Cin or taps != 9:
        raise N.SgxError("conv+stats: 3x3 pack with the activation's channel count expected")
    L = N.lib()
    npart = L.sgx_conv3x3_stats_nparts(B, H, W, Cin, Cout, N.dt(x))
    if npart <= 0:
        raise N.SgxError("conv+stats: no fused kernel for this shape (ask conv_stats_nparts first)")
    y = torch.empty((B, H, W, Cout), dtype=x.dtype, device=x.device)
    part = torch.empty((B, npart, Cout, 2), dtype=torch.float64, device=x.device)
    noise_c = _c(noise.detach().reshape(B, H * W))
    if noise_c.dtype != torch.float32:
        noise_c = noise_c.float()
    N.check(L.sgx_conv3x3_stats(N.ptr(x), N.ptr(wq), N.ptr(y), N.ptr(None if ebias is None else _c(ebias.detach())), N.ptr(noise_c),
                                N.ptr(_c(nw.detach())), N.ptr(part), part.numel() * 8, B, H, W, Cin, Cout, N.dt(x), N.stream()),
            "sgx_conv3x3_stats")
    return y, part


_RGB_PACKS = {}


RGBCONV = os.environ.get("SGX_RGBCONV", "1") != "0"


def rgbconv_ok(B, H, W, C, dtype):
    return RGBCONV and dtype == torch.bfloat16 and bool(N.lib().sgx_rgbconv_ok(int(B), int(H), int(W), int(C), N.BF16))


def rgb_packs(w0, s0, wr, sr, br):
    key = (id(w0), id(wr))
    tag = (_pack_tag(w0), _pack_tag(wr), None if br is None else _pack_tag(br), float(s0), float(sr))
    ent = _RGB_PACKS.get(key)
    if ent is None or ent[0]() is not w0 or ent[1]() is not wr:
        ent = [weakref.ref(w0, lambda _r, k=key: _RGB_PACKS.pop(k, None)), weakref.ref(wr), None, None, None]
        _RGB_PACKS[key] = ent
    if ent[2] != tag:
        C = w0.shape[0]
        if w0.dtype != torch.float32 or wr.dtype != torch.float32 or tuple(w0.shape) != (C, C, 3, 3) or tuple(wr.shape) != (C, 3, 1, 1):
            raise N.SgxError("rgb_packs: conv0.weight [C,C,3,3] and from_rgb.weight [C,3,1,1] (fp32) expected")
        wf = torch.empty((3, C, 16), dtype=torch.bfloat16, device=w0.device)
        wd = torch.empty((3, 16, C), dtype=torch.bfloat16, device=w0.device)
        N.check(N.lib().sgx_rgbconv_pack(N.ptr(_c(w0.detach())), float(s0), N.ptr(_c(wr.detach())), float(sr),
                                         N.ptr(None if br is None else _c(br.detach())), 1.0, N.ptr(wf), N.ptr(wd), C, N.stream()), "sgx_rgbconv_pack")
        ent[2], ent[3], ent[4] = tag, (wf, wd), _pack_mark()
    else:
        raw = N.stream()
        if raw not in ent[4][2]:
            _stream_of(raw).wait_event(ent[4][0])
            ent[4][2].add(raw)
    return ent[3]


def _rgb_wgrad(img, gz, ones, w0, b0, wr, br, s0, sr, want):
    params = (w0, b0, wr, br)
    want = [bool(w) and p is not None for w, p in zip(want, params)]
    if not ones:
        want[1] = want[3] = False
    if not any(want):
        return None, None, None, None
    accum = _ACCUM_PARAM_GRADS and not torch.is_grad_enabled() and all(p.is_leaf for p, w in zip(params, want) if w)
    outs, acc, fresh = [None] * 4, 0, []

    def launch():
        nonlocal acc
        for k, (p, w) in enumerate(zip(params, want)):
            if not w:
                continue
            if accum and p.grad is not None:
                outs[k] = p.grad; acc |= 1 << k
            else:
                outs[k] = torch.empty(p.shape, dtype=torch.float32, device=gz.device); fresh.append(outs[k])
        L = N.lib()
        B, H, W, C = gz.shape
        wsb = L.sgx_rgbconv_wgrad_ws_bytes(B, H, W, C)
        ws = N.workspace(wsb, gz.device)
        N.check(L.sgx_rgbconv_wgrad(N.ptr(img), N.ptr(gz), int(bool(ones)), N.ptr(_c(w0.detach())), float(s0), N.ptr(_c(wr.detach())), float(sr),
                                    N.ptr(_c(br.detach())) if (ones and br is not None) else None, 1.0, N.ptr(outs[0]), N.ptr(outs[1]), N.ptr(outs[2]),
                                    N.ptr(outs[3]), acc, N.ptr(ws), wsb, B, H, W, C, N.BF16, N.stream()), "sgx_rgbconv_wgrad")
    side = _PARAM_GRAD_STREAM if accum else None
    cur_raw = N.stream()
    if side is None or side.cuda_stream == cur_raw:
        launch()
    elif not _FAST_FORK or _set_stream is None:
        cur = torch.cuda.current_stream()
        side.wait_stream(cur)
        with torch.cuda.stream(side):
            launch()
        img.record_stream(side); gz.record_stream(side)
        for o in fresh:
            o.record_stream(cur)
    else:
        cur = _stream_of(cur_raw)
        N.check(N.lib().sgx_stream_wait_stream(side.cuda_stream, cur_raw), "sgx_stream_wait_stream")
        _set_stream(stream_id=side.stream_id, device_index=side.device_index, device_type=side.device_type)
        try:
            launch()
        finally:
            _set_stream(stream_id=cur.stream_id, device_index=cur.device_index, device_type=cur.device_type)
        img.record_stream(side); gz.record_stream(side)
        for o in fresh:
            o.record_stream(cur)
    if not accum:
        return tuple(outs)
    for p, w, o in zip(params, want, outs):
        if w:
            if p.grad is None:
                p.grad = o
            if GRAD_NOTE is not None:
                GRAD_NOTE(p)
    return None, None, None, None


class RgbConvBlurFn(Function):
    @staticmethod
    def forward(ctx, img, w0, b0, wr, br, s0, sr):
        img = _c(img)
        if img.dtype != torch.float32 or img.dim() != 4 or img.shape[3] != 3:
            raise N.SgxError("RgbConvBlurFn: fp32 NHWC RGB image expected")
        B, H, W, _ = img.shape
        C = w0.shape[0]
        wf, wd = rgb_packs(w0, s0, wr, sr, br)
        xb = torch.empty((B, H, W, C), dtype=torch.bfloat16, device=img.device)
        bits = torch.empty((B, H, W, C // 8), dtype=torch.uint8, device=img.device)
        N.check(N.lib().sgx_rgbconv_fwd(N.ptr(img), N.ptr(wf), N.ptr(None if b0 is None else _c(b0.detach())), N.ptr(xb), N.ptr(bits), B, H, W, C,
                                        1, 1, N.BF16, N.stream()), "sgx_rgbconv_fwd")
        ctx.cfg = (float(s0), float(sr))
        ctx.save_for_backward(img, w0, b0, wr, br)
        ctx.mark_non_differentiable(bits)
        ctx.set_materialize_grads(False)
        return xb, bits

    @staticmethod
    def backward(ctx, gz, _gbits=None):
        if gz is None:
            return (None,) * 7
        img, w0, b0, wr, br = ctx.saved_tensors
        s0, sr = ctx.cfg
        gz = _c(gz)
        gi = _bcall(RgbConvAdjFn, gz, w0, wr, br, s0, sr) if ctx.needs_input_grad[0] else None
        gw0 = gb0 = gwr = gbr = None
        if not _DATA_GRAD_ONLY:
            gw0, gb0, gwr, gbr = _bcall_wgrad(img, gz, True, w0, b0, wr, br, s0, sr, ctx.needs_input_grad[1:5])
        return gi, gw0, gb0, gwr, gbr, None, None


class RgbConvAdjFn(Function):
    @staticmethod
    def forward(ctx, gz, w0, wr, br, s0, sr):
        gz = _c(gz)
        B, H, W, C = gz.shape
        wf, wd = rgb_packs(w0, s0, wr, sr, br)
        gi = torch.empty((B, H, W, 3), dtype=torch.float32, device=gz.device)
        N.check(N.lib().sgx_rgbconv_dgrad(N.ptr(gz), N.ptr(wd), N.ptr(gi), B, H, W, C, N.dt(gz), N.stream()), "sgx_rgbconv_dgrad")
        ctx.cfg = (float(s0), float(sr))
        ctx.save_for_backward(gz, w0, wr, br)
        return gi

    @staticmethod
    def backward(ctx, gg):
        gz, w0, wr, br = ctx.saved_tensors
        s0, sr = ctx.cfg
        gg = _c(gg.float())
        ggz = _bcall(RgbConvPlainFn, gg, w0, wr, br, s0, sr) if ctx.needs_input_grad[0] else None
        gw0 = gwr = None
        if not _DATA_GRAD_ONLY:
            gw0, _, gwr, _ = _bcall_wgrad(gg, gz, False, w0, None, wr, br, s0, sr, (ctx.needs_input_grad[1], False, ctx.needs_input_grad[2], False))
        return ggz, gw0, gwr, None, None, None


class RgbConvPlainFn(Function):
    @staticmethod
    def forward(ctx, img, w0, wr, br, s0, sr):
        img = _c(img)
        B, H, W, _ = img.shape
        C = w0.shape[0]
        wf, wd = rgb_packs(w0, s0, wr, sr, br)
        z = torch.empty((B, H, W, C), dtype=torch.bfloat16, device=img.device)
        N.check(N.lib().sgx_rgbconv_fwd(N.ptr(img), N.ptr(wf), None, N.ptr(z), None, B, H, W, C, 0, 0, N.BF16, N.stream()), "sgx_rgbconv_fwd")
        ctx.cfg = (float(s0), float(sr))
        ctx.save_for_backward(img, w0, wr, br)
        return z

    @staticmethod
    def backward(ctx, gz):
        img, w0, wr, br = ctx.saved_tensors
        s0, sr = ctx.cfg
        gz = _c(gz)
        gi = _bcall(RgbConvAdjFn, gz, w0, wr, br, s0, sr) if ctx.needs_input_grad[0] else None
        gw0 = gwr = None
        if not _DATA_GRAD_ONLY:
            gw0, _, gwr, _ = _bcall_wgrad(img, gz, False, w0, None, wr, br, s0, sr, (ctx.needs_input_grad[1], False, ctx.needs_input_grad[2], False))
        return gi, gw0, gwr, None, None, None


class RgbConvWgradFn(Function):

    @staticmethod
    def forward(ctx, img, gz, ones, w0, b0, wr, br, s0, sr, want):
        outs = _rgb_wgrad(img, gz, ones, w0, b0, wr, br, s0, sr, want)
        ctx.set_materialize_grads(False)
        return tuple(o if o is not None else torch.zeros((), device=gz.device) for o in outs)

    @staticmethod
    @once_differentiable
    def backward(ctx, *g):
        raise NotImplementedError("second derivative through a weight gradient is not part of the training path")


def _bcall_wgrad(img, gz, ones, w0, b0, wr, br, s0, sr, want):
    want = tuple(bool(w) for w in want)
    if not any(want):
        return None, None, None, None
    if not torch.is_grad_enabled():
        return _rgb_wgrad(_c(img), gz, ones, w0, b0, wr, br, s0, sr, want)
    params = (w0, b0, wr, br)
    outs = RgbConvWgradFn.apply(_c(img), gz, ones, w0, b0, wr, br, s0, sr, want)
    real = [w and p is not None and (ones or k in (0, 2)) for k, (w, p) in enumerate(zip(want, params))]
    return tuple(o if r else None for o, r in zip(outs, real))


def rgbconv_blur(img, w0, b0, wr, br, s0, sr):
    return call(RgbConvBlurFn, img, w0, b0, wr, br, float(s0), float(sr))


class LReluBwdFn(Function):

    @staticmethod
    def forward(ctx, g, y, slope, scale=1.0):
        g = _c(g)
        out = torch.empty_like(g)
        dev = isinstance(scale, torch.Tensor)
        N.check(N.lib().sgx_lrelu_bwd(N.ptr(g), N.ptr(y), N.ptr(out), g.numel(), float(slope), 1.0 if dev else float(scale),
                                      scale.data_ptr() if dev else None, N.dt(g), N.stream()), "sgx_lrelu_bwd")
        ctx.slope, ctx.scale = float(slope), scale
        ctx.save_for_backward(y)
        return out

    @staticmethod
    def backward(ctx, gg):
        (y,) = ctx.saved_tensors
        return _bcall(LReluBwdFn, gg, y, ctx.slope, ctx.scale), None, None, None


class LReluBwdBitsFn(Function):

    @staticmethod
    def forward(ctx, g, bits, slope, scale=1.0):
        g = _c(g)
        if g.dtype != torch.bfloat16 or bits.dtype != torch.uint8 or bits.numel() * 8 != g.numel():
            raise N.SgxError("LReluBwdBitsFn: bf16 gradient and one sign byte per 8 channels expected")
        out = torch.empty_like(g)
        dev = isinstance(scale, torch.Tensor)
        N.check(N.lib().sgx_lrelu_bwd_bits(N.ptr(g), N.ptr(bits), N.ptr(out), g.numel(), float(slope), 1.0 if dev else float(scale),
                                           scale.data_ptr() if dev else None, N.dt(g), N.stream()), "sgx_lrelu_bwd_bits")
        ctx.slope, ctx.scale = float(slope), scale
        ctx.save_for_backward(bits)
        return out

    @staticmethod
    def backward(ctx, gg):
        (bits,) = ctx.saved_tensors
        return _bcall(LReluBwdBitsFn, gg, bits, ctx.slope, ctx.scale), None, None, None


FUSE_FADE = os.environ.get("SGX_FUSE_FADE", "1") != "0"


def conv_down_fade_ok(x, cout):
    if not FUSE_FADE or x.dtype != torch.bfloat16:
        return False
    B, H, W, Cin = x.shape
    return bool(N.lib().sgx_conv4x4s2_down_fade_ok(B, H, W, Cin, int(cout), N.BF16))


class ConvDownFadeFn(Function):

    @staticmethod
    def forward(ctx, x, weight, bias, resid, scale, ipad, alpha, beta, x_pre=None, x_pre_bits=None):
        x, resid = _c(x), _c(resid)
        fwd, adj = packs(weight, "D", scale, ipad, x.dtype)
        B, H, W, Cin = x.shape
        taps, Cout, K = fwd.shape
        if K != Cin or tuple(resid.shape) != (B, H // 2, W // 2, Cout) or resid.dtype != x.dtype:
            raise N.SgxError("conv+fade: residual branch must have the output's shape and dtype")
        y = torch.empty((B, H // 2, W // 2, Cout), dtype=x.dtype, device=x.device)
        bits = torch.empty((B, H // 2, W // 2, Cout // 8), dtype=torch.uint8, device=x.device)
        dev = isinstance(alpha, torch.Tensor)
        if dev and not (alpha.dtype == torch.float32 and alpha.numel() == 2 and alpha.is_contiguous()):
            raise N.SgxError("conv+fade: device coefficients must be a contiguous fp32 [alpha, beta] pair")
        N.check(N.lib().sgx_conv4x4s2_down_fade(N.ptr(x), N.ptr(fwd), N.ptr(None if bias is None else _c(bias.detach())), N.ptr(resid),
                                                0.0 if dev else float(alpha), 0.0 if dev else float(beta), alpha.data_ptr() if dev else None,
                                                N.ptr(y), N.ptr(bits), B, H, W, Cin, Cout, N.dt(x), N.stream()), "sgx_conv4x4s2_down_fade")
        ctx.cfg = ("D", scale, ipad, False, 0, bias is not None, False, False)
        ctx.bias_ref = weakref.ref(bias) if bias is not None else (lambda: None)
        ctx.fade = (None, None) if dev else (float(alpha), float(beta))
        ctx.save_for_backward(x, weight, None, None, x_pre, x_pre_bits, bits, alpha if dev else None)
        return y

    @staticmethod
    def backward(ctx, g):
        g = _c(g)
        bits, alpha_dev = ctx.saved_tensors[6:8]
        alpha, beta = ctx.fade
        if alpha_dev is not None:
            alpha = alpha_dev
        g_res = None
        if isinstance(alpha, torch.Tensor):
            if ctx.needs_input_grad[3]:
                g_res = _bcall(ScaleDevFn, g, alpha[1:2])
            gy = _bcall(LReluBwdBitsFn, g, bits, 0.2, alpha[0:1])
        else:
            if ctx.needs_input_grad[3]:
                g_res = g if beta == 1.0 else _bcall(ScaleFn, g, beta)
            gy = _bcall(LReluBwdBitsFn, g, bits, 0.2, alpha)
        out = ConvFn.backward(ctx, gy)
        return out[0], out[1], out[2], g_res, None, None, None, None, None, None


FUSE_FADE_RGB = os.environ.get("SGX_FUSE_FADE_RGB", "1") != "0"


class RgbResidual:

    def __init__(self, pimg, layer, out_scale, dtype):
        self.pimg, self.layer, self.out_scale, self.dtype = pimg, layer, float(out_scale), dtype

    def materialize(self):
        return self.layer.forward_nhwc(self.pimg, out_dtype=self.dtype, out_scale=self.out_scale)


def fade_rgb_ok(layer, cout, dtype):
    return (FUSE_FADE and FUSE_FADE_RGB and dtype == torch.bfloat16 and int(cout) in (32, 64, 128) and layer.kernel_size == 1
            and tuple(layer.weight.shape) == (int(cout), 3, 1, 1))


FUSE_FADE_BWD2 = os.environ.get("SGX_FUSE_FADE_BWD2", "1") != "0"


class FadeRgbBwdFn(Function):

    @staticmethod
    def forward(ctx, g, bits, pimg, wr, ws, alpha, beta, alpha_dev, need_img):
        g = _c(g)
        dev = alpha_dev is not None
        with torch.no_grad():
            gy = LReluBwdBitsFn.forward(_NoGradCtx(), g, bits, 0.2, alpha_dev[0:1] if dev else alpha)
            gpimg = None
            if need_img:
                g_res = ScaleDevFn.forward(_NoGradCtx(), g, alpha_dev[1:2]) if dev else (g if beta == 1.0 else ScaleFn.forward(_NoGradCtx(), g, beta))
                gpimg = RgbOutFn.forward(_NoGradCtx(), g_res, wr, None, ws)
        ctx.cfg = (float(ws), None if dev else float(alpha), None if dev else float(beta), need_img)
        ctx.save_for_backward(g, bits, wr, alpha_dev)
        ctx.set_materialize_grads(False)
        return gy, gpimg

    @staticmethod
    @once_differentiable
    def backward(ctx, ggy, ggp):
        g, bits, wr, alpha_dev = ctx.saved_tensors
        ws, alpha, beta, need_img = ctx.cfg
        if ggy is None and ggp is None:
            return (None,) * 9
        dev = alpha_dev is not None
        L = N.lib()
        C = g.shape[-1]
        npix = g.numel() // C
        out = torch.empty_like(g)
        ggy_c = None if ggy is None else _c(ggy)
        ggp_c = None if ggp is None else _c(ggp)
        N.check(L.sgx_fade_rgb_bwd2(N.ptr(ggy_c), N.ptr(ggp_c), N.ptr(bits), N.ptr(_c(wr.detach())), ws * (1.0 if dev else beta), 0.0 if dev else alpha, 1.0,
                                    alpha_dev.data_ptr() if dev else None, N.ptr(out), npix, C, N.dt(g), N.stream()), "sgx_fade_rgb_bwd2")
        gwr = None
        if ggp_c is not None and ctx.needs_input_grad[3] and not _DATA_GRAD_ONLY:
            gwr = RgbWgradFn.forward(_NoGradCtx(), ggp_c, g, wr, ws * (1.0 if dev else beta))
            if dev:
                gwr = gwr * alpha_dev[1]
        return out, None, None, gwr, None, None, None, None, None


class ConvDownFadeRgbFn(Function):

    @staticmethod
    def forward(ctx, x, weight, bias, pimg, wr, br, scale, ipad, alpha, beta, ws, bs1, bs2, x_pre=None, x_pre_bits=None):
        x, pimg = _c(x), _c(pimg)
        fwd, adj = packs(weight, "D", scale, ipad, x.dtype)
        B, H, W, Cin = x.shape
        taps, Cout, K = fwd.shape
        if K != Cin or tuple(pimg.shape) != (B, H // 2, W // 2, 3) or pimg.dtype != torch.float32 or tuple(wr.shape) != (Cout, 3, 1, 1):
            raise N.SgxError("conv+fade(rgb): pooled fp32 image [B, H/2, W/2, 3] and a [Cout, 3, 1, 1] weight expected")
        y = torch.empty((B, H // 2, W // 2, Cout), dtype=x.dtype, device=x.device)
        bits = torch.empty((B, H // 2, W // 2, Cout // 8), dtype=torch.uint8, device=x.device)
        dev = isinstance(alpha, torch.Tensor)
        if dev and not (alpha.dtype == torch.float32 and alpha.numel() == 2 and alpha.is_contiguous()):
            raise N.SgxError("conv+fade(rgb): device coefficients must be a contiguous fp32 [alpha, beta] pair")
        N.check(N.lib().sgx_conv4x4s2_down_fade_rgb(N.ptr(x), N.ptr(fwd), N.ptr(None if bias is None else _c(bias.detach())), N.ptr(pimg),
                                                    N.ptr(_c(wr.detach())), float(ws), N.ptr(None if br is None else _c(br.detach())), float(bs1), float(bs2),
                                                    0.0 if dev else float(alpha), 0.0 if dev else float(beta), alpha.data_ptr() if dev else None,
                                                    N.ptr(y), N.ptr(bits), B, H, W, Cin, Cout, N.dt(x), N.stream()), "sgx_conv4x4s2_down_fade_rgb")
        ctx.cfg = ("D", scale, ipad, False, 0, bias is not None, False, False)
        ctx.bias_ref = weakref.ref(bias) if bias is not None else (lambda: None)
        ctx.br_ref = weakref.ref(br) if br is not None else (lambda: None)
        ctx.fade = ((None, None) if dev else (float(alpha), float(beta))) + (float(ws), float(bs1) * float(bs2))
        ctx.save_for_backward(x, weight, None, None, x_pre, x_pre_bits, bits, alpha if dev else None, pimg, wr)
        return y

    @staticmethod
    def backward(ctx, g):
        g = _c(g)
        bits, alpha_dev, pimg, wr = ctx.saved_tensors[6:10]
        alpha, beta, ws, bs = ctx.fade
        br = ctx.br_ref()
        need_img = ctx.needs_input_grad[3]
        want_w = ctx.needs_input_grad[4] and not _DATA_GRAD_ONLY
        want_b = br is not None and ctx.needs_input_grad[5] and not _DATA_GRAD_ONLY
        gpimg = gwr = gbr = None
        if torch.is_grad_enabled() and FUSE_FADE_BWD2 and not want_w and not want_b:
            gy, gpimg = FadeRgbBwdFn.apply(g, bits, pimg, wr, ws, alpha, beta, alpha_dev, bool(need_img))
        elif torch.is_grad_enabled():
            if alpha_dev is not None:
                g_res = _bcall(ScaleDevFn, g, alpha_dev[1:2])
                gy = _bcall(LReluBwdBitsFn, g, bits, 0.2, alpha_dev[0:1])
            else:
                g_res = g if beta == 1.0 else _bcall(ScaleFn, g, beta)
                gy = _bcall(LReluBwdBitsFn, g, bits, 0.2, alpha)
            if need_img:
                gpimg = _bcall(RgbOutFn, g_res, wr, None, ws)
            if want_w:
                gwr = _bcall(RgbWgradFn, pimg, g_res, wr, ws)
            if want_b:
                gbr = _bcall(ColSumFn, g_res, bs)
        else:
            L = N.lib()
            C = g.shape[-1]
            npix = g.numel() // C
            accum = _ACCUM_PARAM_GRADS and wr.is_leaf and (br is None or br.is_leaf)
            acc = 0
            dw = db = None
            if want_w and accum and wr.grad is not None:
                dw, acc = wr.grad, acc | 1
            if want_b and accum and br.grad is not None:
                db, acc = br.grad, acc | 2
            gy = torch.empty_like(g)
            if need_img:
                gpimg = torch.empty_like(pimg)
            wsb = L.sgx_fade_rgb_bwd_ws_bytes(npix, C)
            wsp = N.workspace(wsb, g.device)
            dev = alpha_dev is not None
            side = _PARAM_GRAD_STREAM if (accum and (want_w or want_b)) else None
            cur_raw = N.stream()
            if side is not None and side.cuda_stream == cur_raw:
                side = None
            if side is None:
                if want_w and dw is None:
                    dw = torch.empty(wr.shape, dtype=torch.float32, device=g.device)
                if want_b and db is None:
                    db = torch.empty(br.shape, dtype=torch.float32, device=g.device)
            N.check(L.sgx_fade_rgb_bwd(N.ptr(g), N.ptr(bits), N.ptr(pimg), N.ptr(_c(wr.detach())), ws, bs, 0.0 if dev else alpha, 0.0 if dev else beta,
                                       alpha_dev.data_ptr() if dev else None, N.ptr(gy), None if side is not None else N.ptr(dw),
                                       None if side is not None else N.ptr(db), acc, N.ptr(gpimg), N.ptr(wsp), wsb, npix, C,
                                       N.dt(g), cur_raw), "sgx_fade_rgb_bwd")
            if side is not None:
                fresh = []

                def finish():
                    nonlocal dw, db
                    if want_w and dw is None:
                        dw = torch.empty(wr.shape, dtype=torch.float32, device=g.device); fresh.append(dw)
                    if want_b and db is None:
                        db = torch.empty(br.shape, dtype=torch.float32, device=g.device); fresh.append(db)
                    N.check(L.sgx_fade_rgb_bwd_finish(N.ptr(wsp), wsb, npix, C, ws, bs, 0.0 if dev else beta, alpha_dev.data_ptr() if dev else None,
                                                      N.ptr(dw), N.ptr(db), acc, N.stream()), "sgx_fade_rgb_bwd_finish")
                _fork_to(side, cur_raw, finish, reads=(wsp,) + ((alpha_dev,) if dev else ()), fresh=fresh)
            if accum:
                for p_, d_ in ((wr, dw), (br, db)):
                    if d_ is not None:
                        if p_.grad is None:
                            p_.grad = d_
                        if GRAD_NOTE is not None:
                            GRAD_NOTE(p_)
            else:
                gwr, gbr = dw, db
        out = ConvFn.backward(ctx, gy)
        return (out[0], out[1], out[2], gpimg, gwr, gbr) + (None,) * 9


class ColSumFn(Function):

    @staticmethod
    def forward(ctx, x, scale):
        x = _c(x)
        C = x.shape[-1]
        npix = x.numel() // C
        out = torch.empty((C,), dtype=torch.float32, device=x.device)
        L = N.lib()
        ws = N.workspace(L.sgx_colsum_ws_bytes(npix, C), x.device)
        N.check(L.sgx_colsum(N.ptr(x), N.ptr(out), float(scale), N.ptr(ws), ws.numel(), npix, C, N.dt(x), N.stream()), "sgx_colsum")
        ctx.shape, ctx.dtype, ctx.scale = x.shape, x.dtype, float(scale)
        return out

    @staticmethod
    def backward(ctx, g):
        return (g * ctx.scale).to(ctx.dtype).expand(ctx.shape), None


class BiasActFn(Function):

    @staticmethod
    def forward(ctx, x, bias, bscale, act):
        x = _c(x)
        C = x.shape[-1]
        y = torch.empty_like(x)
        N.check(N.lib().sgx_bias_act(N.ptr(x), N.ptr(None if bias is None else _c(bias.detach())), float(bscale), N.ptr(y),
                                     x.numel() // C, C, act, N.dt(x), N.stream()), "sgx_bias_act")
        ctx.act, ctx.has_bias, ctx.bscale = act, bias is not None, float(bscale)
        ctx.save_for_backward(y if act else None)
        return y

    @staticmethod
    def backward(ctx, g):
        (y,) = ctx.saved_tensors
        g = _c(g)
        if ctx.act:
            g = _bcall(LReluBwdFn, g, y, 0.0 if ctx.act == N.ACT_RELU else 0.2, 1.0)
        gb = None
        if ctx.has_bias and ctx.needs_input_grad[1] and not _DATA_GRAD_ONLY:
            gb = _bcall(ColSumFn, g, ctx.bscale)
        return g, gb, None, None


class ScaleFn(Function):
    @staticmethod
    def forward(ctx, x, s):
        x = _c(x)
        out = torch.empty_like(x)
        N.check(N.lib().sgx_axpby(N.ptr(x), None, N.ptr(out), float(s), 0.0, x.numel(), N.dt(x), N.stream()), "sgx_axpby")
        ctx.s = float(s)
        return out

    @staticmethod
    def backward(ctx, g):
        return _bcall(ScaleFn, g, ctx.s), None


class AxpbyFn(Function):

    @staticmethod
    def forward(ctx, a, b, alpha, beta, a_act=False):
        a, b = _c(a), _c(b)
        assert a.shape == b.shape and a.dtype == b.dtype
        out = torch.empty_like(a)
        N.check(N.lib().sgx_axpby(N.ptr(a), N.ptr(b), N.ptr(out), float(alpha), float(beta), a.numel(), N.dt(a), N.stream()), "sgx_axpby")
        ctx.alpha, ctx.beta, ctx.a_act = float(alpha), float(beta), bool(a_act)
        ctx.save_for_backward(a if a_act else None)
        return out

    @staticmethod
    def backward(ctx, g):
        (a,) = ctx.saved_tensors
        ga = gb = None
        if ctx.needs_input_grad[0]:
            ga = _bcall(LReluBwdFn, g, a, 0.2, ctx.alpha) if ctx.a_act else _bcall(ScaleFn, g, ctx.alpha)
        if ctx.needs_input_grad[1]:
            gb = g if ctx.beta == 1.0 else _bcall(ScaleFn, g, ctx.beta)
        return ga, gb, None, None, None

# ... 79 lines not shown
        y = torch.empty_like(x)
        L = N.lib()
        npart = L.sgx_blur3x3_stats_nparts(B, H, W, C, N.dt(x))
        part = torch.empty((B, npart, C, 2), dtype=torch.float64, device=x.device)
        noise_c = _c(noise.detach().reshape(B, H * W))
        if noise_c.dtype != torch.float32:
            noise_c = noise_c.float()
        N.check(L.sgx_blur3x3_stats(N.ptr(x), N.ptr(y), N.ptr(None if bias is None else _c(bias.detach())), N.ptr(noise_c),
                                    N.ptr(_c(nw.detach())), N.ptr(part), part.numel() * 8, B, H, W, C, N.ACT_LRELU, N.dt(x), N.stream()),
                "sgx_blur3x3_stats")
        ctx.mark_non_differentiable(part)
        ctx.set_materialize_grads(False)
        return y, part

    @staticmethod
    def backward(ctx, g, _gpart):
        return (_bcall(BlurFn, g) if g is not None else None), None, None, None


class BlurGenFn(Function):

    @staticmethod
    def forward(ctx, x, taps, K, pad, OH, OW):
        import ctypes
        x = _c(x)
        B, IH, IW, C = x.shape
        y = torch.empty((B, OH, OW, C), dtype=x.dtype, device=x.device)
        arr = (ctypes.c_float * (K * K))(*taps)
        N.check(N.lib().sgx_blur_kxk(N.ptr(x), N.ptr(y), ctypes.addressof(arr), K, pad, B, IH, IW, OH, OW, C, N.dt(x), N.stream()), "sgx_blur_kxk")
        ctx.cfg = (taps, K, pad, IH, IW)
        return y

    @staticmethod
    def backward(ctx, g):
        taps, K, pad, IH, IW = ctx.cfg
        return _bcall(BlurGenFn, g, tuple(reversed(taps)), K, K - 1 - pad, IH, IW), None, None, None, None, None


def _blur_act(x, z, mode, bits=None):
    x = _c(x)
    B, H, W, C = x.shape
    y = torch.empty_like(x)
    if bits is not None:
        N.check(N.lib().sgx_blur3x3_bits(N.ptr(x), N.ptr(bits), N.ptr(y), B, H, W, C, mode, N.dt(x), N.stream()), "sgx_blur3x3_bits")
        return y
    N.check(N.lib().sgx_blur3x3_act(N.ptr(x), None if z is None else N.ptr(z), N.ptr(y), B, H, W, C, mode, N.dt(x), N.stream()), "sgx_blur3x3_act")
    return y


class ActBlurFn(Function):

    @staticmethod
    def forward(ctx, z):
        z = _c(z)
        ctx.save_for_backward(z)
        return _blur_act(z, None, 1)

    @staticmethod
    def backward(ctx, g):
        (z,) = ctx.saved_tensors
        return _bcall(BlurMaskFn, g, z)


class BlurMaskFn(Function):

    @staticmethod
    def forward(ctx, g, z, bits=None):
        ctx.save_for_backward(z, bits)
        return _blur_act(g, z, 2, bits)

    @staticmethod
    def backward(ctx, gg):
        z, bits = ctx.saved_tensors
        return _bcall(MaskBlurFn, gg, z, bits), None, None


class MaskBlurFn(Function):

    @staticmethod
    def forward(ctx, g, z, bits=None):
        ctx.save_for_backward(z, bits)
        return _blur_act(g, z, 3, bits)

    @staticmethod
    def backward(ctx, gg):
        z, bits = ctx.saved_tensors
        return _bcall(BlurMaskFn, gg, z, bits), None, None


class Pool2Fn(Function):

    @staticmethod
    def forward(ctx, x, scale):
        x = _c(x)
        B, H, W, C = x.shape
        y = torch.empty((B, H // 2, W // 2, C), dtype=x.dtype, device=x.device)
        N.check(N.lib().sgx_pool2(N.ptr(x), N.ptr(y), B, H, W, C, float(scale), N.dt(x), N.stream()), "sgx_pool2")
        ctx.scale = float(scale)
        return y

    @staticmethod
    def backward(ctx, g):
        return _bcall(Up2Fn, g, ctx.scale), None


class Up2Fn(Function):

    @staticmethod
    def forward(ctx, x, scale):
        x = _c(x)
        B, H, W, C = x.shape
        y = torch.empty((B, 2 * H, 2 * W, C), dtype=x.dtype, device=x.device)
        N.check(N.lib().sgx_up2(N.ptr(x), N.ptr(y), B, H, W, C, float(scale), N.dt(x), N.stream()), "sgx_up2")
        ctx.scale = float(scale)
        return y

    @staticmethod
    def backward(ctx, g):
        return _bcall(Pool2Fn, g, ctx.scale), None


class UpAddFn(Function):

    @staticmethod
    def forward(ctx, a, x, scale):
        a, x = _c(a), _c(x)
        B, H, W, C = x.shape
        if tuple(a.shape) != (B, 2 * H, 2 * W, C) or a.dtype != x.dtype:
            raise N.SgxError("UpAddFn: a must be [B, 2H, 2W, C] of x's dtype")
        y = torch.empty_like(a)
        N.check(N.lib().sgx_up2_add(N.ptr(x), N.ptr(a), N.ptr(y), B, H, W, C, float(scale), N.dt(x), N.stream()), "sgx_up2_add")
        ctx.scale = float(scale)
        return y

    @staticmethod
    def backward(ctx, g):
        return g, _bcall(Pool2Fn, g, ctx.scale), None


POOL_FORK = os.environ.get("SGX_POOL_FORK", "1") != "0"


class PoolForkFn(Function):

    @staticmethod
    def forward(ctx, x, scale):
        y = Pool2Fn.forward(_NoGradCtx(), x, scale)
        ctx.scale = float(scale)
        ctx.set_materialize_grads(False)
        return x.view_as(x), y

    @staticmethod
    def backward(ctx, gx, gy):
        if gy is None:
            return gx, None
        if gx is None:
            return _bcall(Up2Fn, gy, ctx.scale), None
        return _bcall(UpAddFn, gx, gy, ctx.scale), None


def _dtype_code(dtype):
    return N.F32 if dtype == torch.float32 else N.BF16


def rgb_layout(weight):
    if weight.shape[1] == 3 and weight.shape[0] != 3:
        return 1, 3, weight.shape[0]
    if weight.shape[0] == 3:
        return weight.shape[1], 1, weight.shape[1]
    raise N.SgxError("1x1 convolution is built for the RGB layers (3 channels on one side)")


class RgbInFn(Function):

    @staticmethod
    def forward(ctx, img, weight, bias, wscale, out_dtype):
        img, w = _c(img), _c(weight.detach())
        sj, sc, C = rgb_layout(w)
        B, H, W, _ = img.shape
        y = torch.empty((B, H, W, C), dtype=out_dtype, device=img.device)
        N.check(N.lib().sgx_rgb_in(N.ptr(img), N.ptr(w), sj, sc, float(wscale), N.ptr(None if bias is None else _c(bias.detach())), N.ptr(y),
                                   B * H * W, C, _dtype_code(out_dtype), N.stream()), "sgx_rgb_in")
        ctx.has_bias, ctx.wscale = bias is not None, float(wscale)
        ctx.save_for_backward(img, weight)
        return y

    @staticmethod
    def backward(ctx, g):
        img, weight = ctx.saved_tensors
        g = _c(g)
        gi = gw = gb = None
        if ctx.needs_input_grad[0]:
            gi = _bcall(RgbOutFn, g, weight, None, ctx.wscale)
        if not _DATA_GRAD_ONLY:
            if ctx.needs_input_grad[1]:
                gw = _bcall(RgbWgradFn, img, g, weight, ctx.wscale)
            if ctx.has_bias and ctx.needs_input_grad[2]:
                gb = _bcall(ColSumFn, g, 1.0)
        return gi, gw, gb, None, None


class RgbOutFn(Function):

    @staticmethod
    def forward(ctx, x, weight, bias, wscale):
        x, w = _c(x), _c(weight.detach())
        sj, sc, C = rgb_layout(w)
        B, H, W, Cx = x.shape
        assert Cx == C
        img = torch.empty((B, H, W, 3), dtype=torch.float32, device=x.device)
        N.check(N.lib().sgx_rgb_out(N.ptr(x), N.ptr(w), sj, sc, float(wscale), N.ptr(None if bias is None else _c(bias.detach())), N.ptr(img),
                                    B * H * W, C, N.dt(x), N.stream()), "sgx_rgb_out")
        ctx.has_bias, ctx.wscale = bias is not None, float(wscale)
        ctx.save_for_backward(x, weight)
        return img

    @staticmethod
    def backward(ctx, g):
        x, weight = ctx.saved_tensors
        g = _c(g)
        gx = gw = gb = None
        if ctx.needs_input_grad[0]:
            gx = _bcall(RgbInFn, g, weight, None, ctx.wscale, x.dtype)
        if not _DATA_GRAD_ONLY:
            if ctx.needs_input_grad[1]:
                gw = _bcall(RgbWgradFn, g, x, weight, ctx.wscale)
            if ctx.has_bias and ctx.needs_input_grad[2]:
                gb = _bcall(ColSumFn, g, 1.0)
        return gx, gw, gb, None


RGB_FORK = os.environ.get("SGX_RGB_FORK", "1") != "0"


class RgbOutForkFn(Function):

    @staticmethod
    def forward(ctx, x, weight, bias, wscale):
        img = RgbOutFn.forward(ctx, x, weight, bias, wscale)
        ctx.set_materialize_grads(False)
        return x.view_as(x), img

    @staticmethod
    def backward(ctx, gx, g):
        if g is None:
            return gx, None, None, None
        x, weight = ctx.saved_tensors
        g = _c(g)
        out = gw = gb = None
        if ctx.needs_input_grad[0]:
            if gx is None:
                out = _bcall(RgbInFn, g, weight, None, ctx.wscale, x.dtype)
            elif torch.is_grad_enabled():
                out = gx + _bcall(RgbInFn, g, weight, None, ctx.wscale, x.dtype)
            else:
                gx, w = _c(gx), _c(weight.detach())
                sj, sc, C = rgb_layout(w)
                B, H, W, _ = g.shape
                out = torch.empty_like(gx)
                N.check(N.lib().sgx_rgb_in_add(N.ptr(g), N.ptr(w), sj, sc, ctx.wscale, N.ptr(gx), N.ptr(out), B * H * W, C, N.dt(gx), N.stream()),
                        "sgx_rgb_in_add")
        else:
            out = gx
        if not _DATA_GRAD_ONLY:
            if ctx.needs_input_grad[1]:
                gw = _bcall(RgbWgradFn, g, x, weight, ctx.wscale)
            if ctx.has_bias and ctx.needs_input_grad[2]:
                gb = _bcall(ColSumFn, g, 1.0)
        return out, gw, gb, None


class RgbOutFadeFn(Function):

    @staticmethod
    def forward(ctx, x, weight, bias, wscale, low, alpha):
        x, w, low = _c(x), _c(weight.detach()), _c(low)
        sj, sc, C = rgb_layout(w)
        B, H, W, Cx = x.shape
        assert Cx == C and low.shape == (B, H // 2, W // 2, 3) and low.dtype == torch.float32
        img = torch.empty((B, H, W, 3), dtype=torch.float32, device=x.device)
        dev = isinstance(alpha, torch.Tensor)
        N.check(N.lib().sgx_rgb_out_fade(N.ptr(x), N.ptr(w), sj, sc, float(wscale), N.ptr(None if bias is None else _c(bias.detach())), N.ptr(low),
                                         0.0 if dev else float(alpha), 0.0 if dev else float(1 - alpha), alpha.data_ptr() if dev else None,
                                         N.ptr(img), B, H, W, C, N.dt(x), N.stream()), "sgx_rgb_out_fade")
        ctx.has_bias, ctx.wscale, ctx.alpha = bias is not None, float(wscale), alpha
        ctx.save_for_backward(x, weight)
        return img

    @staticmethod
    def backward(ctx, g):
        x, weight = ctx.saved_tensors
        g = _c(g)
        al = ctx.alpha
        gx = gw = gb = glow = None
        if isinstance(al, torch.Tensor):
            ga, a_s = _bcall(ScaleDevFn, g, al[0:1]), 1.0
            gl, b_s = (_bcall(ScaleDevFn, g, al[1:2]) if ctx.needs_input_grad[4] else None), 1.0
        else:
            ga, a_s, gl, b_s = g, float(al), g, float(1 - al)
        if ctx.needs_input_grad[0]:
            gx = _bcall(RgbInFn, ga, weight, None, ctx.wscale * a_s, x.dtype)
        if not _DATA_GRAD_ONLY:
            if ctx.needs_input_grad[1]:
                gw = _bcall(RgbWgradFn, ga, x, weight, ctx.wscale * a_s)
            if ctx.has_bias and ctx.needs_input_grad[2]:
                gb = _bcall(ColSumFn, ga, a_s)
        if ctx.needs_input_grad[4]:
            glow = _bcall(Pool2Fn, gl, b_s)
        return gx, gw, gb, None, glow, None


class RgbWgradFn(Function):

    @staticmethod
    def forward(ctx, img, f, weight, wscale):
        img, f = _c(img), _c(f)
        sj, sc, C = rgb_layout(weight)
        npix = img.numel() // 3
        dw = torch.empty_like(weight, dtype=torch.float32, memory_format=torch.contiguous_format)
        L = N.lib()
        ws = N.workspace(L.sgx_rgb_wgrad_ws_bytes(npix, C), f.device)
        N.check(L.sgx_rgb_wgrad(N.ptr(img), N.ptr(f), N.ptr(dw), sj, sc, float(wscale), N.ptr(ws), ws.numel(), npix, C, N.dt(f),
                                N.stream()), "sgx_rgb_wgrad")
        return dw

    @staticmethod
    @once_differentiable
    def backward(ctx, g):
        raise NotImplementedError("second derivative through a weight gradient is not part of the training path")


class GEpilogueFn(Function):

    @staticmethod
    def forward(ctx, x, bias, noise, nw, style, flags=N.EPI_ACT | N.EPI_NORM, pre=None):
        x = _c(x)
        B, H, W, C = x.shape
        ctx.has_noise, ctx.has_style = nw is not None, style is not None
        if nw is None:
            noise = torch.zeros((B, H * W), dtype=torch.float32, device=x.device)
            nw_c = torch.zeros((C,), dtype=torch.float32, device=x.device)
        else:
            noise = _c(noise.detach().reshape(B, H * W))
            if noise.dtype != torch.float32:
                noise = noise.float()
# ... 356 lines not shown
        lm = _c(lm)
        L_, B, D = lm.shape
        key = (tuple(w.data_ptr() for w in ws), tuple(b.data_ptr() for b in bs), meta, B)
        ent = _STYLE_TABLES.get(key)
        if ent is None:
            rows, yoff, tile = [], 0, 0
            for (layer, w_mul, b_mul), w, b in zip(meta, ws, bs):
                n = w.shape[0]
                assert w.shape[1] == D and w.is_contiguous() and w.dtype == torch.float32
                rows.append([w.data_ptr(), b.data_ptr(), n, yoff, tile, int(np.float32(w_mul).view(np.uint32)),
                             int(np.float32(b_mul).view(np.uint32)), layer])
                yoff += B * n; tile += (n + 15) // 16
            table, _ = N.upload(torch.tensor(rows, dtype=torch.int64), lm.device)
            ent = _STYLE_TABLES[key] = (table, [r[2] for r in rows], [r[3] for r in rows], yoff, tile)
        table, ns, yoffs, ytotal, tiles = ent
        y = torch.empty(ytotal, dtype=torch.float32, device=lm.device)
        N.check(N.lib().sgx_style_fwd(N.ptr(lm), N.ptr(table), N.ptr(y), G, B, D, tiles, N.stream()), "sgx_style_fwd")
        ctx.ent, ctx.G, ctx.shape = ent, G, (L_, B, D)
        ctx.save_for_backward(lm)
        return tuple(y[o:o + B * n].view(B, n) for o, n in zip(yoffs, ns))

    @staticmethod
    @once_differentiable
    def backward(ctx, *gys):
        (lm,) = ctx.saved_tensors
        table, ns, yoffs, ytotal, tiles = ctx.ent
        L_, B, D = ctx.shape
        G = ctx.G
        gy = torch.cat([(g if g is not None else torch.zeros(B, n, device=lm.device)).reshape(-1) for g, n in zip(gys, ns)])
        L = N.lib()
        glm = None
        if ctx.needs_input_grad[0]:
            glm = torch.zeros_like(lm) if G < L_ else torch.empty_like(lm)
            N.check(L.sgx_style_bwd_data(N.ptr(gy), N.ptr(table), N.ptr(glm), G, B, D, max(ns), N.stream()), "sgx_style_bwd_data")
        ntot = sum(ns)
        dw = torch.empty((ntot, D), dtype=torch.float32, device=lm.device)
        db = torch.empty((ntot,), dtype=torch.float32, device=lm.device)
        N.check(L.sgx_style_bwd_param(N.ptr(gy), N.ptr(lm), N.ptr(table), N.ptr(dw), N.ptr(db), G, B, D, tiles, N.stream()),
                "sgx_style_bwd_param")
        offs = [o // B for o in yoffs]
        gws = tuple(dw[o:o + n] for o, n in zip(offs, ns))
        gbs = tuple(db[o:o + n] for o, n in zip(offs, ns))
        return (glm, None) + gws + gbs


class NoiseArena:

    def __init__(self, numel, device):
        self.buf = torch.randn(int(numel), device=device, dtype=torch.float32)
        self.off = 0

    def take(self, b, h, w):
        n = b * h * w
        if self.off + n > self.buf.numel():
            return torch.randn(b, 1, h, w, device=self.buf.device, dtype=torch.float32)
        out = self.buf[self.off:self.off + n].view(b, 1, h, w)
        self.off += n
        return out


NOISE_ARENA = None


def linear(x, weight, bias, w_mul, b_mul, act=N.ACT_NONE):
    y = call(MatMulFn, x, weight, 0, 1, w_mul)
    if bias is None and act == N.ACT_NONE:
        return y
    return call(BiasActFn, y, bias, b_mul, act)


def nhwc(x_nchw, dtype=None):
    t = x_nchw.permute(0, 2, 3, 1)
    if dtype is not None and t.dtype != dtype:
        t = t.to(dtype)
    return t.contiguous()


def images_from_uint8(u8, flip=None, out_dtype=torch.float32, layout=None):
    if not (u8.is_cuda and u8.dtype == torch.uint8 and u8.dim() == 4):
        raise N.SgxError("images_from_uint8: need a 4-d uint8 GPU tensor")
    if layout is None:
        hwc, chw = u8.shape[3] == 3, u8.shape[1] == 3
        if hwc == chw:
            raise N.SgxError(f"images_from_uint8: cannot infer the layout of {tuple(u8.shape)}; pass layout='hwc' or 'chw'")
        layout = "hwc" if hwc else "chw"
    u8 = _c(u8)
    B, H, W = (u8.shape[0], u8.shape[1], u8.shape[2]) if layout == "hwc" else (u8.shape[0], u8.shape[2], u8.shape[3])
    fl = None
    if flip is not None:
        fl = torch.as_tensor(flip).to(device=u8.device, dtype=torch.int32).contiguous()
        if fl.numel() != B:
            raise N.SgxError("images_from_uint8: one flip decision per image")
    out = torch.empty((B, H, W, 3), dtype=out_dtype, device=u8.device)
    N.check(N.lib().sgx_images_u8_to_nhwc(N.ptr(u8), N.ptr(out), N.ptr(fl), B, H, W, int(layout == "chw"), N.dt(out), N.stream()),
            "sgx_images_u8_to_nhwc")
    return nchw_view(out)


def nchw_view(x_nhwc):
    return x_nhwc.permute(0, 3, 1, 2)


DIFFAUG_OPS = ("color", "translation", "cutout")


def diffaug_policy_bits(policy):
    if policy is None:
        return 0
    if not isinstance(policy, str):
        raise ValueError(f"diffaug_policy must be a string, got {type(policy).__name__}")
    bits, last = 0, -1
    for name in (s.strip() for s in policy.split(",")) if policy.strip() else ():
        if name not in DIFFAUG_OPS:
            raise ValueError(f"unknown DiffAugment op {name!r} in {policy!r} (known: {','.join(DIFFAUG_OPS)})")
        k = DIFFAUG_OPS.index(name)
        if k <= last:
            raise ValueError(f"DiffAugment policy {policy!r}: ops must appear once each, in the order {','.join(DIFFAUG_OPS)}")
        bits |= 1 << k
        last = k
    return bits


def _diffaug(x, u, bits, adjoint, with_bias, img_bits=None):
    x, u = _c(x), _c(u)
    if x.dim() != 4 or x.shape[3] != 3 or x.dtype != torch.float32:
        raise N.SgxError(f"diffaug: need fp32 [B,H,W,3] images, got {tuple(x.shape)} {x.dtype}")
    B, H, W, _ = x.shape
    if tuple(u.shape) != (B, 7) or u.dtype != torch.float32 or u.device != x.device:
        raise N.SgxError(f"diffaug: need fp32 [{B},7] draws on {x.device}, got {tuple(u.shape)} {u.dtype} on {u.device}")
    y = torch.empty_like(x)
    L = N.lib()
    ws, nb = None, 0
    if bits & 1:
        nb = L.sgx_diffaug_ws_bytes(B, H, W)
        ws = N.workspace(nb, x.device)
    if img_bits is None:
        N.check(L.sgx_diffaug(N.ptr(x), N.ptr(y), N.ptr(u), B, H, W, int(bits), int(adjoint), int(with_bias), N.ptr(ws), nb, N.stream()),
                "sgx_diffaug")
        return y
    if tuple(img_bits.shape) != (B,) or img_bits.dtype != torch.int32 or img_bits.device != x.device:
        raise N.SgxError(f"diffaug: need int32 [{B}] image bits on {x.device}, got {tuple(img_bits.shape)} {img_bits.dtype} on "
                         f"{img_bits.device}")
    N.check(L.sgx_diffaug_gated(N.ptr(x), N.ptr(y), N.ptr(u), N.ptr(_c(img_bits)), B, H, W, int(bits), int(adjoint), int(with_bias),
                                N.ptr(ws), nb, N.stream()), "sgx_diffaug_gated")
    return y


class DiffAugFn(Function):

    @staticmethod
    def forward(ctx, x, u, bits, img_bits=None):
        ctx.save_for_backward(u, img_bits)
        ctx.bits = bits
        return _diffaug(x, u, bits, False, True, img_bits)

    @staticmethod
    def backward(ctx, g):
        if not ctx.needs_input_grad[0]:
            return None, None, None, None
        u, img_bits = ctx.saved_tensors
        return _bcall(DiffAugAdjFn, g, u, ctx.bits, img_bits), None, None, None


class DiffAugAdjFn(Function):

    @staticmethod
    def forward(ctx, g, u, bits, img_bits=None):
        ctx.save_for_backward(u, img_bits)
        ctx.bits = bits
        return _diffaug(g, u, bits, True, False, img_bits)

    @staticmethod
    def backward(ctx, gg):
        u, img_bits = ctx.saved_tensors
        return _bcall(DiffAugLinFn, gg, u, ctx.bits, img_bits), None, None, None


class DiffAugLinFn(Function):

    @staticmethod
    def forward(ctx, x, u, bits, img_bits=None):
        ctx.save_for_backward(u, img_bits)
        ctx.bits = bits
        return _diffaug(x, u, bits, False, False, img_bits)

    @staticmethod
    def backward(ctx, g):
        u, img_bits = ctx.saved_tensors
        return _bcall(DiffAugAdjFn, g, u, ctx.bits, img_bits), None, None, None


def _ada_state_ok(state, device, what):
    if tuple(state.shape) != (8,) or state.dtype != torch.float32 or state.device != device or not state.is_contiguous():
        raise N.SgxError(f"{what}: need a contiguous fp32 [8] state on {device}, got {tuple(state.shape)} {state.dtype} on {state.device}")


def ada_gates(gu, state, bits):
    gu = _c(gu)
    if gu.dim() != 2 or gu.shape[1] != 3 or gu.dtype != torch.float32:
        raise N.SgxError(f"ada_gates: need fp32 [B,3] uniforms, got {tuple(gu.shape)} {gu.dtype}")
    _ada_state_ok(state, gu.device, "ada_gates")
    out = torch.empty(gu.shape[0], dtype=torch.int32, device=gu.device)
    N.check(N.lib().sgx_ada_gates(N.ptr(gu), N.ptr(state), int(bits), N.ptr(out), gu.shape[0], N.stream()), "sgx_ada_gates")
    return out


def ada_update(real_logits, state, target, adjust_per_image, interval):
    lg = _c(real_logits.detach()).reshape(-1)
    if lg.dtype != torch.float32:
        raise N.SgxError(f"ada_update: need fp32 logits, got {lg.dtype}")
    _ada_state_ok(state, lg.device, "ada_update")
    N.check(N.lib().sgx_ada_update(N.ptr(lg), lg.numel(), N.ptr(state), float(target), float(adjust_per_image), int(interval), N.stream()),
            "sgx_ada_update")
    return state
```

stylegan/pytorch_amd/native.py:

```python
import ctypes
import os
import subprocess
import threading

import torch

_HERE = os.path.dirname(os.path.abspath(__file__))
LIB_PATH = os.environ.get("SGX_HIP_LIB") or os.path.join(_HERE, "libsgx_hip.so")
CSRC = os.path.join(_HERE, "csrc")

F32, BF16 = 0, 1
ACT_NONE, ACT_LRELU, ACT_RELU = 0, 1, 2
EPI_ACT, EPI_NORM = 1, 2
PACK_S, PACK_D, PACK_U, PACK_UF = 0, 1, 2, 3

_lib = None
_lock = threading.Lock()

c_void_p, c_int, c_float, c_size_t = ctypes.c_void_p, ctypes.c_int, ctypes.c_float, ctypes.c_size_t
P, I, F, Z = c_void_p, c_int, c_float, c_size_t

SIGNATURES = {
    "sgx_version": (I, []),
    "sgx_last_error": (ctypes.c_char_p, []),
    "sgx_clear_error": (I, []),
    "sgx_stream_wait_stream": (I, [P, P]),
    "sgx_conv3x3": (I, [P, P, P, P, I, I, I, I, I, I, P, I, P]),
    "sgx_conv_variant": (I, [I, P, P, P, P, I, I, I, I, I, I, I, I, P]),
    "sgx_conv4x4s2_down": (I, [P, P, P, P, I, I, I, I, I, I, I, P]),
    "sgx_conv4x4s2_up": (I, [P, P, P, I, I, I, I, I, I, P]),
    "sgx_wgrad_ws_bytes": (Z, [I, I, I, I, I, I]),
    "sgx_images_u8_to_nhwc": (I, [P, P, P, I, I, I, I, I, P]),
    "sgx_selftest_tr16": (I, [P, P]),
    "sgx_conv_splitk_ws_bytes": (Z, [I, I, I, I, I, I, I]),
    "sgx_conv_splitk": (I, [I, P, P, P, P, P, I, I, I, I, I, I, I, P, Z, P]),
    "sgx_conv_config": (I, [I, I, I, I, I, I, I, P]),
    "sgx_prof_start": (I, [I, I]),
    "sgx_prof_count": (I, []),
    "sgx_prof_get": (I, [I, P, I, P, P, P, P, I]),
    "sgx_pack_weight": (I, [P, P, P, I, I, I, I, F, I, P]),
    "sgx_pack_weight_multi": (I, [P, I, I, I, P]),
    "sgx_pack_weight_blocks": (I, [I, I]),
    "sgx_wgrad3x3_param": (I, [P, P, P, P, P, Z, I, I, I, I, I, I, F, I, I, I, I, P]),
    "sgx_wgrad4x4s2_param": (I, [P, P, P, P, P, Z, I, I, I, I, I, I, F, I, I, I, I, P]),
    "sgx_bias_act": (I, [P, P, F, P, Z, I, I, I, P]),
    "sgx_lrelu_bwd": (I, [P, P, P, Z, F, F, P, I, P]),
    "sgx_lrelu_bwd_bits": (I, [P, P, P, Z, F, F, P, I, P]),
    "sgx_conv4x4s2_down_fade_ok": (I, [I, I, I, I, I, I]),
    "sgx_conv4x4s2_down_fade": (I, [P, P, P, P, F, F, P, P, P, I, I, I, I, I, I, P]),
    "sgx_conv4x4s2_down_fade_rgb": (I, [P, P, P, P, P, F, P, F, F, F, F, P, P, P, I, I, I, I, I, I, P]),
    "sgx_fade_rgb_bwd_ws_bytes": (Z, [Z, I]),
    "sgx_fade_rgb_bwd": (I, [P, P, P, P, F, F, F, F, P, P, P, P, I, P, P, Z, Z, I, I, P]),
    "sgx_fade_rgb_bwd_finish": (I, [P, Z, Z, I, F, F, F, P, P, P, I, P]),
    "sgx_fade_rgb_bwd2": (I, [P, P, P, P, F, F, F, P, P, Z, I, I, P]),
    "sgx_axpby": (I, [P, P, P, F, F, Z, I, P]),
    "sgx_axpby_dev": (I, [P, P, P, P, P, Z, I, P]),
    "sgx_blur3x3": (I, [P, P, I, I, I, I, I, P]),
    "sgx_blur3x3_act": (I, [P, P, P, I, I, I, I, I, I, P]),
    "sgx_blur_kxk": (I, [P, P, P, I, I, I, I, I, I, I, I, I, P]),
    "sgx_pool2": (I, [P, P, I, I, I, I, F, I, P]),
    "sgx_up2": (I, [P, P, I, I, I, I, F, I, P]),
    "sgx_up2_add": (I, [P, P, P, I, I, I, I, F, I, P]),
    "sgx_colsum_ws_bytes": (Z, [Z, I]),
    "sgx_colsum": (I, [P, P, F, P, Z, Z, I, I, P]),
    "sgx_rgb_in": (I, [P, P, I, I, F, P, P, Z, I, I, P]),
    "sgx_rgb_in_add": (I, [P, P, I, I, F, P, P, Z, I, I, P]),
    "sgx_rgb_out": (I, [P, P, I, I, F, P, P, Z, I, I, P]),
    "sgx_downsample_fade_rgb": (I, [P, P, I, I, I, F, F, P, P]),
    "sgx_diffaug_ws_bytes": (Z, [I, I, I]),
    "sgx_diffaug": (I, [P, P, P, I, I, I, I, I, I, P, Z, P]),
    "sgx_ada_gates": (I, [P, P, I, P, I, P]),
    "sgx_diffaug_gated": (I, [P, P, P, P, I, I, I, I, I, I, P, Z, P]),
    "sgx_ada_update": (I, [P, I, P, F, F, I, P]),
    "sgx_rgb_out_fade": (I, [P, P, I, I, F, P, P, F, F, P, P, I, I, I, I, I, P]),
    "sgx_rgb_wgrad_ws_bytes": (Z, [Z, I]),
    "sgx_rgb_wgrad": (I, [P, P, P, I, I, F, P, Z, Z, I, I, P]),
    "sgx_gepi_ws_bytes": (Z, [I, I, I]),
    "sgx_gepi_fwd": (I, [P, P, P, P, P, P, P, P, P, Z, P, I, I, I, I, I, I, P]),
    "sgx_gepi_stats": (I, [P, P, P, P, P, P, P, Z, P, I, I, I, I, I, I, P]),
    "sgx_rgb_out_epi": (I, [P, P, P, P, P, P, P, P, I, I, F, P, P, F, F, P, P, I, I, I, I, I, P]),
    "sgx_rgb_wgrad_epi_ws_bytes": (Z, [I, I, I]),
    "sgx_rgb_wgrad_epi": (I, [P, P, P, P, P, P, P, P, P, P, I, I, F, F, P, Z, I, I, I, I, P]),
    "sgx_blur3x3_stats_nparts": (I, [I, I, I, I, I]),
    "sgx_conv3x3_stats_nparts": (I, [I, I, I, I, I, I]),
    "sgx_conv3x3_signbits_ok": (I, [I, I, I, I, I, I]),
    "sgx_conv3x3_signbits": (I, [P, P, P, P, P, I, I, I, I, I, I, P, I, P]),
    "sgx_blur3x3_bits": (I, [P, P, P, I, I, I, I, I, I, P]),
    "sgx_conv4x4s2_up_blur_ok": (I, [I, I, I, I, I, I]),
    "sgx_conv4x4s2_up_blur": (I, [P, P, P, P, I, I, I, I, I, I, P]),
    "sgx_conv4x4s2_up_blur_bits": (I, [P, P, P, P, I, I, I, I, I, I, P]),
    "sgx_pack_upblur": (I, [P, P, I, I, I, I, F, P]),
    "sgx_conv_upblur_ok": (I, [I, I, I, I, I, I]),
    "sgx_conv_upblur": (I, [P, P, P, P, I, I, I, I, I, I, P]),
    "sgx_rgbconv_ok": (I, [I, I, I, I, I]),
    "sgx_rgbconv_pack": (I, [P, F, P, F, P, F, P, P, I, P]),
    "sgx_rgbconv_fwd": (I, [P, P, P, P, P, I, I, I, I, I, I, I, P]),
    "sgx_rgbconv_tune": (I, [I, I, I]),
    "sgx_rgbconv_dgrad": (I, [P, P, P, I, I, I, I, I, P]),
    "sgx_rgbconv_wgrad_ws_bytes": (Z, [I, I, I, I]),
    "sgx_rgbconv_wgrad": (I, [P, P, I, P, F, P, F, P, F, P, P, P, P, I, P, Z, I, I, I, I, I, P]),
    "sgx_conv3x3_stats": (I, [P, P, P, P, P, P, P, Z, I, I, I, I, I, I, P]),
    "sgx_blur3x3_stats": (I, [P, P, P, P, P, P, Z, I, I, I, I, I, I, P]),
    "sgx_gepi_bwd": (I, [P, P, P, P, P, P, P, P, P, P, P, P, P, Z, I, I, I, I, I, P]),
    "sgx_pixelnorm_fwd": (I, [P, P, I, I, P]),
    "sgx_pixelnorm_bwd": (I, [P, P, P, I, I, P]),
    "sgx_mbstd_fwd": (I, [P, P, I, I, I, I, I, P]),
    "sgx_mbstd_bwd": (I, [P, P, P, I, I, I, I, I, P]),
    "sgx_mbstd_bwd2": (I, [P, P, P, P, P, I, I, I, I, I, P]),
    "sgx_sumsq_ws_bytes": (Z, []),
    "sgx_sumsq_f32": (I, [P, Z, P, Z, P, P]),
    "sgx_scale_dev_f32": (I, [P, P, F, P, Z, P]),
    "sgx_logistic_loss": (I, [P, I, P, I, F, I, P, P, P, P]),
    "sgx_gemm_ws_bytes": (Z, [I, I, I]),
    "sgx_gemm_f32": (I, [P, P, P, I, I, I, I, I, F, P, Z, P]),
    "sgx_linear_fwd": (I, [P, P, P, P, I, I, I, F, F, I, P]),
    "sgx_linear_bwd_data": (I, [P, P, P, P, I, I, I, F, P]),
    "sgx_linear_bwd_param": (I, [P, P, P, P, P, I, I, I, F, F, P]),
    "sgx_style_fwd": (I, [P, P, P, I, I, I, I, P]),
    "sgx_style_bwd_data": (I, [P, P, P, I, I, I, I, P]),
    "sgx_style_bwd_param": (I, [P, P, P, P, P, I, I, I, I, P]),
    "sgx_adam_multi": (I, [P, P, P, P, P, I, F, F, F, P, P, P, P]),
    "sgx_ema_multi": (I, [P, P, P, I, F, P]),
    "sgx_gradnorm_clip_coef": (I, [P, P, I, F, P, P, P]),
}


def build(verbose: bool = False) -> str:
    cmd = ["make", "-C", CSRC, "-j", str(min(8, os.cpu_count() or 1))]
    r = subprocess.run(cmd, capture_output=True, text=True)
    if r.returncode != 0:
        raise RuntimeError("building libsgx_hip.so failed:\n" + r.stdout[-4000:] + r.stderr[-4000:])
    if verbose:
        print(r.stdout[-2000:])
    return LIB_PATH


def lib():
    global _lib
    if _lib is None:
        with _lock:
            if _lib is None:
                if not os.path.exists(LIB_PATH):
                    raise RuntimeError(f"{LIB_PATH} is missing: run `python -c 'import __graft_entry__ as g; g.build()'` "
                                       "(there is no non-HIP fallback for this path)")
                l = ctypes.CDLL(LIB_PATH)
                for name, (res, args) in SIGNATURES.items():
                    fn = getattr(l, name)
                    fn.restype, fn.argtypes = res, args
                _lib = l
    return _lib


class SgxError(RuntimeError):
    pass


def check(rc: int, what: str):
    if rc != 0:
        msg = lib().sgx_last_error().decode(errors="replace")
        raise SgxError(f"{what} failed (code {rc}): {msg}")


_raw_stream = getattr(torch._C, "_cuda_getCurrentRawStream", None)
_get_device = getattr(torch._C, "_cuda_getDevice", None) or torch.cuda.current_device


def stream() -> int:
    if _raw_stream is not None:
        return _raw_stream(_get_device())
    return torch.cuda.current_stream().cuda_stream


def dt(t: torch.Tensor) -> int:
    if t.dtype == torch.float32:
        return F32
    if t.dtype == torch.bfloat16:
        return BF16
    raise TypeError(f"unsupported activation dtype {t.dtype}")


def ptr(t):
    if t is None:
        return None
    if not t.is_cuda:
        raise SgxError("libsgx_hip kernels need GPU tensors (no CPU fallback exists for this path)")
    if not t.is_contiguous():
        raise SgxError("internal: non-contiguous tensor passed to a kernel")
    return t.data_ptr()


_ARENA = []


def capturing() -> bool:
    return torch.cuda.is_available() and torch.cuda.is_current_stream_capturing()


# ... 138 lines not shown
```

Baseline: 281.6 img/s.

## Defer and batch wgrad finish kernels into table-driven multi-launch; skip image grads

Per-layer weight-gradient finish and pre-reduce launches are recorded instead of issued. They are then flushed at the end of backward as a few table-driven multi-kernel launches, and the finish kernel chains rows that target the same dW/db. Separately, a no_image_grad context skips computing gradients with respect to input images during the discriminator backward when they are not needed. The aim is to cut kernel launch count and host overhead and to avoid unneeded image-gradient work. In exchange it adds global defer state, a host-built table upload, and extra complexity around accumulation ordering.

```diff
diff --git a/include/sgx.h b/include/sgx.h
--- a/include/sgx.h
+++ b/include/sgx.h
@@ -45,6 +45,12 @@
 int sgx_wgrad4x4s2_param(const void* fine, const void* coarse, float* dW, float* db, void* ws, size_t ws_bytes, int B, int H,
                          int W, int Cfine, int Ccoarse, int mode, float scale, int O, int I, int accumulate, int dtype,
                          void* stream);
+#define SGX_FINISH_ROW 16
+#define SGX_PRE_ROW 6
+int sgx_wgrad_defer(int on);
+int sgx_wgrad_defer_pending(void);
+int sgx_wgrad_defer_plan(long long* table, int cap_words, int* counts);
+int sgx_wgrad_defer_flush(const void* table, void* stream);
 
 int sgx_bias_act(const void* x, const float* bias, float bscale, void* y, size_t npix, int C, int act, int dtype,
                  void* stream);
diff --git a/stylegan/pytorch_amd/GAN.py b/stylegan/pytorch_amd/GAN.py
--- a/stylegan/pytorch_amd/GAN.py
+++ b/stylegan/pytorch_amd/GAN.py
@@ -666,8 +666,9 @@
         side = self._param_stream(two_branches=aux is not None and lazy)
         self._sched_begin("d", depth, side)
         try:
-            with F.accumulate_param_grads(), F.param_grad_stream(side):
+            with F.accumulate_param_grads(), F.param_grad_stream(side), F.no_image_grad():
                 loss.backward()
+                F.flush_param_grads()
         except BaseException:
             self._sched_abort()
             raise
@@ -726,6 +727,7 @@
             try:
                 with F.accumulate_param_grads(), F.param_grad_stream(side):
                     loss.backward()
+                    F.flush_param_grads()
             except BaseException:
                 self._sched_abort()
                 raise
diff --git a/stylegan/pytorch_amd/csrc/conv.hip b/stylegan/pytorch_amd/csrc/conv.hip
--- a/stylegan/pytorch_amd/csrc/conv.hip
+++ b/stylegan/pytorch_amd/csrc/conv.hip
@@ -1,5 +1,8 @@
 #include "common.h"
 #include <stdlib.h>
+#include <string.h>
+#include <mutex>
+#include <vector>
 
 enum { G3X3 = 0, GDOWN = 1, GUP = 2, GUPA = 3 };
 int sgx_wgrad2_plan(int geo, int B, int H, int W, int Ck, int Cn, int* nct_n, int* nct_k, int* kbw, int* ntiles);
@@ -1012,67 +1015,152 @@
 struct FinishArgs { const float* ws; float* dw; float* db; int nsplit, O, I, Ip, mode, transposed, flip_t; float scale; int accumulate; };
 
 template <int EPB>
-__global__ __launch_bounds__(256) void wgrad_finish_kernel(FinishArgs f) {
-    constexpr int NSL = 256 / EPB;
-    __shared__ float red[NSL][EPB][9];
+__device__ __forceinline__ void wgrad_finish_block(FinishArgs f, const unsigned blk, float* __restrict__ red,
+                                                   const long long* __restrict__ tab, int next) {
+    constexpr int NSL = 256 / EPB, NOUT = (EPB * 9 + 255) / 256;
     const int pl = threadIdx.x % EPB, sl = threadIdx.x / EPB;
     const int A = f.transposed ? f.Ip : f.O, Bd = f.transposed ? f.O : f.Ip;
-    const int e = blockIdx.x * EPB + pl;
+    const int e = blk * EPB + pl;
     const int taps = f.mode == SGX_PACK_S ? 9 : 16;
     const size_t tstride = (size_t)f.O * f.Ip, total = (size_t)taps * tstride + A;
-    if ((int)blockIdx.x >= (A * Bd + EPB - 1) / EPB) {
-        const int o = ((int)blockIdx.x - (A * Bd + EPB - 1) / EPB) * EPB + pl;
-        float b = 0.f;
-        if (o < f.O)
-            for (int s = sl; s < f.nsplit; s += NSL) b += f.ws[(size_t)s * total + (size_t)taps * tstride + o];
-        red[sl][pl][0] = b;
+    if ((int)blk >= (A * Bd + EPB - 1) / EPB) {
+        const int o = ((int)blk - (A * Bd + EPB - 1) / EPB) * EPB + pl;
+        float cur = 0.f;
+        bool have = false;
+        for (;;) {
+            float b = 0.f;
+            if (o < f.O)
+                for (int s = sl; s < f.nsplit; s += NSL) b += f.ws[(size_t)s * total + (size_t)taps * tstride + o];
+            red[(sl * EPB + pl) * 9] = b;
+            __syncthreads();
+            if (sl == 0 && o < f.O) {
+                float sum = 0.f;
+                for (int l = 0; l < NSL; ++l) sum += red[(l * EPB + pl) * 9];
+                cur = (f.accumulate & 2) ? (have ? cur : f.db[o]) + sum : sum;
+            }
+            have = true;
+            if (next < 0) break;
+            const long long* r = tab + (size_t)next * SGX_FINISH_ROW;
+            f.ws = reinterpret_cast<const float*>(r[0]); f.nsplit = (int)r[3]; f.accumulate = (int)r[10];
+            next = (int)r[15];
+            __syncthreads();
+        }
+        if (sl == 0 && o < f.O) f.db[o] = cur;
+        return;
+    }
+    float cur[NOUT];
+    bool have = false;
+    for (;;) {
+        float acc[9];
+#pragma unroll
+        for (int k = 0; k < 9; ++k) acc[k] = 0.f;
+        if (e < A * Bd) {
+#pragma unroll 4
+            for (int s = sl; s < f.nsplit; s += NSL) {
+                const float* p = f.ws + (size_t)s * total + e;
+                if (f.mode == SGX_PACK_S) {
+#pragma unroll
+                    for (int t = 0; t < 9; ++t) acc[t] += p[(size_t)(f.flip_t ? 8 - t : t) * tstride];
+                } else {
+                    float v[16];
+#pragma unroll
+                    for (int t = 0; t < 16; ++t) v[t] = p[(size_t)t * tstride];
+#pragma unroll
+                    for (int y = 0; y < 3; ++y)
+#pragma unroll
+                        for (int x = 0; x < 3; ++x)
+                            acc[y * 3 + x] += (v[y * 4 + x] + v[y * 4 + x + 1]) + (v[(y + 1) * 4 + x] + v[(y + 1) * 4 + x + 1]);
+                }
+            }
+        }
+#pragma unroll
+        for (int k = 0; k < 9; ++k) red[(sl * EPB + pl) * 9 + k] = acc[k];
         __syncthreads();
-        if (sl == 0 && o < f.O) {
+#pragma unroll
+        for (int j = 0; j < NOUT; ++j) {
+            const int t = threadIdx.x + j * 256;
+            if (t >= EPB * 9) continue;
+            const int el = t / 9, k = t % 9;
+            const int ee = blk * EPB + el;
+            if (ee >= A * Bd) continue;
+            const int a = ee / Bd, bb = ee % Bd;
+            const int o = f.transposed ? bb : a, i = f.transposed ? a : bb;
+            if (i >= f.I) continue;
             float sum = 0.f;
-            for (int l = 0; l < NSL; ++l) sum += red[l][pl][0];
-            f.db[o] = (f.accumulate & 2) ? f.db[o] + sum : sum;
-        }
-        return;
-    }
-    float acc[9];
-#pragma unroll
-    for (int k = 0; k < 9; ++k) acc[k] = 0.f;
-    if (e < A * Bd) {
-#pragma unroll 4
-        for (int s = sl; s < f.nsplit; s += NSL) {
-            const float* p = f.ws + (size_t)s * total + e;
-            if (f.mode == SGX_PACK_S) {
-#pragma unroll
-                for (int t = 0; t < 9; ++t) acc[t] += p[(size_t)(f.flip_t ? 8 - t : t) * tstride];
-            } else {
-                float v[16];
-#pragma unroll
-                for (int t = 0; t < 16; ++t) v[t] = p[(size_t)t * tstride];
-#pragma unroll
-                for (int y = 0; y < 3; ++y)
-#pragma unroll
-                    for (int x = 0; x < 3; ++x)
-                        acc[y * 3 + x] += (v[y * 4 + x] + v[y * 4 + x + 1]) + (v[(y + 1) * 4 + x] + v[(y + 1) * 4 + x + 1]);
-            }
-        }
-    }
-#pragma unroll
-    for (int k = 0; k < 9; ++k) red[sl][pl][k] = acc[k];
-    __syncthreads();
-    for (int t = threadIdx.x; t < EPB * 9; t += 256) {
+#pragma unroll 8
+            for (int l = 0; l < NSL; ++l) sum += red[(l * EPB + el) * 9 + k];
+            const float c = f.scale * (f.mode == SGX_PACK_D ? 0.25f : 1.f);
+            const float* d = f.dw + ((size_t)o * f.I + i) * 9 + (f.mode == SGX_PACK_UF ? 8 - k : k);
+            cur[j] = (f.accumulate & 1) ? (have ? cur[j] : *d) + c * sum : c * sum;
+        }
+        have = true;
+        if (next < 0) break;
+        const long long* r = tab + (size_t)next * SGX_FINISH_ROW;
+        f.ws = reinterpret_cast<const float*>(r[0]); f.nsplit = (int)r[3]; f.scale = __uint_as_float((unsigned)r[9]);
+        f.accumulate = (int)r[10];
+        next = (int)r[15];
+        __syncthreads();
+    }
+#pragma unroll
+    for (int j = 0; j < NOUT; ++j) {
+        const int t = threadIdx.x + j * 256;
+        if (t >= EPB * 9) continue;
         const int el = t / 9, k = t % 9;
-        const int ee = blockIdx.x * EPB + el;
+        const int ee = blk * EPB + el;
         if (ee >= A * Bd) continue;
         const int a = ee / Bd, bb = ee % Bd;
         const int o = f.transposed ? bb : a, i = f.transposed ? a : bb;
         if (i >= f.I) continue;
-        float sum = 0.f;
-#pragma unroll 8
-        for (int l = 0; l < NSL; ++l) sum += red[l][el][k];
-        const float c = f.scale * (f.mode == SGX_PACK_D ? 0.25f : 1.f);
-        float* d = f.dw + ((size_t)o * f.I + i) * 9 + (f.mode == SGX_PACK_UF ? 8 - k : k);
-        *d = (f.accumulate & 1) ? *d + c * sum : c * sum;
-    }
+        f.dw[((size_t)o * f.I + i) * 9 + (f.mode == SGX_PACK_UF ? 8 - k : k)] = cur[j];
+    }
+}
+
+template <int EPB>
+__global__ __launch_bounds__(256) void wgrad_finish_kernel(FinishArgs f) {
+    __shared__ float red[256 * 9];
+    wgrad_finish_block<EPB>(f, blockIdx.x, red, nullptr, -1);
+}
+
+__device__ __forceinline__ int table_row_of_block(const long long* __restrict__ tab, int n, int stride, int col) {
+    if (n <= 64) {
+        const int l = threadIdx.x & 63;
+        return __builtin_amdgcn_readfirstlane(__popcll(__ballot(l < n && (unsigned)tab[(l < n ? l : 0) * stride + col] <= blockIdx.x)) - 1);
+    }
+    int t = 0;
+    while (t + 1 < n && (unsigned)tab[(t + 1) * stride + col] <= blockIdx.x) ++t;
+    return t;
+}
+
+__global__ __launch_bounds__(256) void wgrad_finish_multi_kernel(const long long* __restrict__ tab, int lo, int n) {
+    __shared__ float red[256 * 9];
+    const long long* r = tab + (size_t)(lo + table_row_of_block(tab + (size_t)lo * SGX_FINISH_ROW, n, SGX_FINISH_ROW, 13)) * SGX_FINISH_ROW;
+    const FinishArgs f{reinterpret_cast<const float*>(r[0]), reinterpret_cast<float*>(r[1]), reinterpret_cast<float*>(r[2]), (int)r[3], (int)r[4],
+                       (int)r[5], (int)r[6], (int)r[7], (int)(r[8] & 1), (int)((r[8] >> 1) & 1), __uint_as_float((unsigned)r[9]), (int)r[10]};
+    const unsigned blk = blockIdx.x - (unsigned)r[13];
+    const int next = (int)r[15];
+    switch ((int)r[11]) {
+        case 64: wgrad_finish_block<64>(f, blk, red, tab, next); break;
+        case 16: wgrad_finish_block<16>(f, blk, red, tab, next); break;
+        case 8: wgrad_finish_block<8>(f, blk, red, tab, next); break;
+        default: wgrad_finish_block<4>(f, blk, red, tab, next); break;
+    }
+}
+
+struct FinishRow { FinishArgs f; int epb; const float* pre_src; float* pre_out; size_t total4; int pre_nsplit; int launch, next; unsigned first, blocks; };
+struct FinishLaunch { int lo, n; unsigned blocks; };
+static std::mutex g_defer_mu;
+static bool g_defer_on = false;
+static std::vector<FinishRow> g_defer_rows;
+static std::vector<FinishLaunch> g_defer_launches;
+static int g_defer_npre = 0, g_defer_planned = 0;
+static unsigned g_defer_pre_blocks = 0;
+static double g_defer_bytes = 0.0;
+static bool wgrad_defer_pending_for(const float* dw, const float* db) {
+    std::lock_guard<std::mutex> lk(g_defer_mu);
+    if (!g_defer_on) return false;
+    for (const FinishRow& r : g_defer_rows)
+        if (r.f.dw == dw || (db && r.f.db == db)) return true;
+    return false;
 }
 
 static int wgrad_nsplit(int pairs, int ntiles, size_t elems_per_split) {
@@ -1107,7 +1195,7 @@
     if ((size_t)nsplit > fit) nsplit = (int)fit;
     SGX_REQUIRE(nsplit >= 1, SGX_EWORKSPACE, "wgrad: workspace too small (%zu bytes, need >= %zu)", ws_bytes, total * sizeof(float));
     a.out = static_cast<float*>(ws);
-    a.direct = (nsplit == 1 && a.dw != nullptr) ? 1 : 0;
+    a.direct = (nsplit == 1 && a.dw != nullptr && !wgrad_defer_pending_for(a.dw, a.db)) ? 1 : 0;
     auto kern = wgrad_kernel<T, GEO, TH, TW, BP, NSUB, KSUB, TR>;
     sgx_lds_opt_in<wgrad_kernel<T, GEO, TH, TW, BP, NSUB, KSUB, TR>>(LDS);
     hipLaunchKernelGGL(kern, dim3(pairs, nsplit), dim3(256), LDS, st, a);
@@ -1146,11 +1234,11 @@
 
 static int wgrad_pre_groups() { static const int v = [] { const char* e = getenv("SGX_WGRAD_PRE"); return e ? atoi(e) : 32; }(); return v; }
 static int wgrad_pre_min() { static const int v = [] { const char* e = getenv("SGX_WGRAD_PRE_MIN"); return e ? atoi(e) : 256; }(); return v; }
-__global__ __launch_bounds__(256) void wgrad_prereduce_kernel(const float* __restrict__ ws, float* __restrict__ out, size_t total4,
-                                                              int nsplit) {
-    const size_t e = (size_t)blockIdx.x * 256 + threadIdx.x;
+__device__ __forceinline__ void wgrad_prereduce_block(const float* __restrict__ ws, float* __restrict__ out, size_t total4, int nsplit,
+                                                      unsigned bx, int g, int groups) {
+    const size_t e = (size_t)bx * 256 + threadIdx.x;
     if (e >= total4) return;
-    const int g = blockIdx.y, per = (nsplit + (int)gridDim.y - 1) / (int)gridDim.y;
+    const int per = (nsplit + groups - 1) / groups;
     const int s0 = g * per, s1 = (s0 + per < nsplit) ? s0 + per : nsplit;
     float4 acc = make_float4(0.f, 0.f, 0.f, 0.f);
 #pragma unroll 4
@@ -1160,6 +1248,15 @@
     }
     reinterpret_cast<float4*>(out)[(size_t)g * total4 + e] = acc;
 }
+__global__ __launch_bounds__(256) void wgrad_prereduce_kernel(const float* __restrict__ ws, float* __restrict__ out, size_t total4,
+                                                              int nsplit) {
+    wgrad_prereduce_block(ws, out, total4, nsplit, blockIdx.x, blockIdx.y, gridDim.y);
+}
+__global__ __launch_bounds__(256) void wgrad_prereduce_multi_kernel(const long long* __restrict__ tab, int n) {
+    const long long* r = tab + (size_t)table_row_of_block(tab, n, SGX_PRE_ROW, 4) * SGX_PRE_ROW;
+    wgrad_prereduce_block(reinterpret_cast<const float*>(r[0]), reinterpret_cast<float*>(r[1]), (size_t)r[2], (int)r[3],
+                          blockIdx.x - (unsigned)r[4], blockIdx.y, gridDim.y);
+}
 static size_t wgrad_pre_bytes(size_t total_floats, int nsplit) {
     const int G = wgrad_pre_groups();
     return (G > 0 && nsplit >= wgrad_pre_min() && nsplit > G && total_floats % 4 == 0) ? (size_t)G * total_floats * sizeof(float) : 0;
@@ -1167,26 +1264,133 @@
 
 static int wgrad_finish(const void* ws, float* dw, float* db, int nsplit, int O, int I, int Ip, int mode, int transposed, int flip_t,
                         float scale, int accumulate, hipStream_t st, size_t ws_bytes = 0) {
+    const size_t total = (size_t)(mode == SGX_PACK_S ? 9 : 16) * O * Ip + (transposed ? Ip : O);
+    const size_t pre = wgrad_pre_bytes(total, nsplit), used = (size_t)nsplit * total * sizeof(float);
+    const float* pre_src = nullptr;
+    float* pre_out = nullptr;
+    const int pre_nsplit = nsplit;
+    if (pre && ws_bytes >= used + pre) {
+        pre_src = static_cast<const float*>(ws);
+        pre_out = reinterpret_cast<float*>(const_cast<char*>(static_cast<const char*>(ws)) + used);
+        ws = pre_out;
+        nsplit = wgrad_pre_groups();
+    }
+    FinishArgs f{static_cast<const float*>(ws), dw, db, nsplit, O, I, Ip, mode, transposed, flip_t, scale, accumulate};
+    const int ne = O * Ip, nb = db ? O : 0;
+    const int epb = ne / 64 >= 128 ? 64 : (ne / 16 >= 128 ? 16 : (ne / 8 >= 128 ? 8 : 4));
+    const unsigned blocks = (unsigned)((ne + epb - 1) / epb + (nb + epb - 1) / epb);
+    const double bytes = 4.0 * ((double)nsplit * (mode == SGX_PACK_S ? 9 : 16) * O * Ip + 9.0 * O * I);
     {
-        const size_t total = (size_t)(mode == SGX_PACK_S ? 9 : 16) * O * Ip + (transposed ? Ip : O);
-        const size_t pre = wgrad_pre_bytes(total, nsplit), used = (size_t)nsplit * total * sizeof(float);
-        if (pre && ws_bytes >= used + pre) {
-            float* out = reinterpret_cast<float*>(const_cast<char*>(static_cast<const char*>(ws)) + used);
-            hipLaunchKernelGGL(wgrad_prereduce_kernel, dim3((unsigned)((total / 4 + 255) / 256), wgrad_pre_groups()), dim3(256), 0, st,
-                               static_cast<const float*>(ws), out, total / 4, nsplit);
-            SGX_LAUNCH_CHECK("wgrad_prereduce_kernel");
-            ws = out;
-            nsplit = wgrad_pre_groups();
-        }
-    }
-    FinishArgs f{static_cast<const float*>(ws), dw, db, nsplit, O, I, Ip, mode, transposed, flip_t, scale, accumulate};
-    SGX_NOTE(0.0, 4.0 * ((double)nsplit * (mode == SGX_PACK_S ? 9 : 16) * O * Ip + 9.0 * O * I), "finish %dx%d m%d tr%d ns%d", O, I, mode, transposed, nsplit);
-    const int ne = O * Ip, nb = db ? O : 0;
-    if (ne / 64 >= 128) hipLaunchKernelGGL(wgrad_finish_kernel<64>, dim3((unsigned)((ne + 63) / 64 + (nb + 63) / 64)), dim3(256), 0, st, f);
-    else if (ne / 16 >= 128) hipLaunchKernelGGL(wgrad_finish_kernel<16>, dim3((unsigned)((ne + 15) / 16 + (nb + 15) / 16)), dim3(256), 0, st, f);
-    else if (ne / 8 >= 128) hipLaunchKernelGGL(wgrad_finish_kernel<8>, dim3((unsigned)((ne + 7) / 8 + (nb + 7) / 8)), dim3(256), 0, st, f);
-    else hipLaunchKernelGGL(wgrad_finish_kernel<4>, dim3((unsigned)((ne + 3) / 4 + (nb + 3) / 4)), dim3(256), 0, st, f);
+        std::lock_guard<std::mutex> lk(g_defer_mu);
+        if (g_defer_on) {
+            g_defer_rows.push_back(FinishRow{f, epb, pre_src, pre_out, total / 4, pre_nsplit, 0, -1, 0u, blocks});
+            g_defer_bytes += bytes;
+            return 0;
+        }
+    }
+    if (pre_src) {
+        hipLaunchKernelGGL(wgrad_prereduce_kernel, dim3((unsigned)((total / 4 + 255) / 256), wgrad_pre_groups()), dim3(256), 0, st,
+                           pre_src, pre_out, total / 4, pre_nsplit);
+        SGX_LAUNCH_CHECK("wgrad_prereduce_kernel");
+    }
+    SGX_NOTE(0.0, bytes, "finish %dx%d m%d tr%d ns%d", O, I, mode, transposed, nsplit);
+    if (epb == 64) hipLaunchKernelGGL(wgrad_finish_kernel<64>, dim3(blocks), dim3(256), 0, st, f);
+    else if (epb == 16) hipLaunchKernelGGL(wgrad_finish_kernel<16>, dim3(blocks), dim3(256), 0, st, f);
+    else if (epb == 8) hipLaunchKernelGGL(wgrad_finish_kernel<8>, dim3(blocks), dim3(256), 0, st, f);
+    else hipLaunchKernelGGL(wgrad_finish_kernel<4>, dim3(blocks), dim3(256), 0, st, f);
     SGX_LAUNCH_CHECK("wgrad_finish_kernel");
+    return 0;
+}
+
+extern "C" int sgx_wgrad_defer(int on) {
+    std::lock_guard<std::mutex> lk(g_defer_mu);
+    if (on == 2 || on == 3) { g_defer_on = on == 3; return 0; }
+    g_defer_on = on != 0;
+    g_defer_rows.clear(); g_defer_launches.clear();
+    g_defer_npre = g_defer_planned = 0; g_defer_pre_blocks = 0; g_defer_bytes = 0.0;
+    return 0;
+}
+extern "C" int sgx_wgrad_defer_pending(void) {
+    std::lock_guard<std::mutex> lk(g_defer_mu);
+    return (int)g_defer_rows.size();
+}
+extern "C" int sgx_wgrad_defer_plan(long long* table, int cap_words, int* counts) {
+    std::lock_guard<std::mutex> lk(g_defer_mu);
+    g_defer_on = false;
+    std::vector<FinishRow>& rows = g_defer_rows;
+    const int n = (int)rows.size();
+    SGX_REQUIRE(table && counts && cap_words >= n * (SGX_FINISH_ROW + SGX_PRE_ROW), SGX_EINVAL, "wgrad_defer_plan: table too small for %d rows", n);
+    std::vector<int> head(n, -1);
+    int nlaunch = 0;
+    for (int i = 0; i < n; ++i) {
+        FinishRow& r = rows[i];
+        int prev = -1;
+        for (int j = i - 1; j >= 0 && prev < 0; --j)
+            if (rows[j].f.dw == r.f.dw || (r.f.db && rows[j].f.db == r.f.db)) prev = j;
+        r.next = -1; r.launch = 0;
+        if (prev >= 0) {
+            const FinishArgs &a = rows[prev].f, &b = r.f;
+            const bool same = a.dw == b.dw && a.db == b.db && a.O == b.O && a.I == b.I && a.Ip == b.Ip && a.mode == b.mode &&
+                              a.transposed == b.transposed && a.flip_t == b.flip_t && rows[prev].epb == r.epb;
+            if (same) { rows[prev].next = i; head[i] = head[prev] >= 0 ? head[prev] : prev; r.launch = rows[prev].launch; }
+            else r.launch = rows[prev].launch + 1;
+        }
+        if (r.launch + 1 > nlaunch) nlaunch = r.launch + 1;
+    }
+    std::vector<int> order, pos(n, -1);
+    g_defer_launches.clear();
+    for (int L = 0; L < nlaunch; ++L) {
+        FinishLaunch fl{(int)order.size(), 0, 0u};
+        for (int i = 0; i < n; ++i)
+            if (rows[i].launch == L && head[i] < 0) { rows[i].first = fl.blocks; fl.blocks += rows[i].blocks; pos[i] = (int)order.size(); order.push_back(i); ++fl.n; }
+        g_defer_launches.push_back(fl);
+    }
+    for (int i = 0; i < n; ++i)
+        if (head[i] >= 0) { rows[i].first = rows[head[i]].first; pos[i] = (int)order.size(); order.push_back(i); }
+    for (int k = 0; k < n; ++k) {
+        const FinishRow& r = rows[order[k]];
+        long long* w = table + (size_t)k * SGX_FINISH_ROW;
+        unsigned sbits; memcpy(&sbits, &r.f.scale, 4);
+        w[0] = (long long)(uintptr_t)r.f.ws; w[1] = (long long)(uintptr_t)r.f.dw; w[2] = (long long)(uintptr_t)r.f.db; w[3] = r.f.nsplit;
+        w[4] = r.f.O; w[5] = r.f.I; w[6] = r.f.Ip; w[7] = r.f.mode; w[8] = (r.f.transposed ? 1 : 0) | (r.f.flip_t ? 2 : 0); w[9] = sbits;
+        w[10] = r.f.accumulate; w[11] = r.epb; w[12] = r.launch; w[13] = r.first; w[14] = head[order[k]] < 0 ? r.blocks : 0;
+        w[15] = r.next >= 0 ? pos[r.next] : -1;
+    }
+    long long* pw = table + (size_t)n * SGX_FINISH_ROW;
+    g_defer_npre = 0; g_defer_pre_blocks = 0;
+    for (int i = 0; i < n; ++i) {
+        const FinishRow& r = rows[i];
+        if (!r.pre_src) continue;
+        const unsigned nb = (unsigned)((r.total4 + 255) / 256);
+        long long* w = pw + (size_t)g_defer_npre * SGX_PRE_ROW;
+        w[0] = (long long)(uintptr_t)r.pre_src; w[1] = (long long)(uintptr_t)r.pre_out; w[2] = (long long)r.total4; w[3] = r.pre_nsplit;
+        w[4] = g_defer_pre_blocks; w[5] = nb;
+        g_defer_pre_blocks += nb; ++g_defer_npre;
+    }
+    g_defer_planned = 1;
+    counts[0] = n; counts[1] = g_defer_npre; counts[2] = nlaunch; counts[3] = n * SGX_FINISH_ROW + g_defer_npre * SGX_PRE_ROW;
+    return 0;
+}
+extern "C" int sgx_wgrad_defer_flush(const void* table, void* stream) {
+    hipStream_t st = (hipStream_t)stream;
+    std::lock_guard<std::mutex> lk(g_defer_mu);
+    SGX_REQUIRE(g_defer_planned && table, SGX_EINVAL, "wgrad_defer_flush: no plan (sgx_wgrad_defer_plan first)");
+    const long long* tab = static_cast<const long long*>(table);
+    const int n = (int)g_defer_rows.size();
+    if (g_defer_npre) {
+        SGX_NOTE(0.0, 0.0, "prereduce_multi n%d", g_defer_npre);
+        hipLaunchKernelGGL(wgrad_prereduce_multi_kernel, dim3(g_defer_pre_blocks, wgrad_pre_groups()), dim3(256), 0, st,
+                           tab + (size_t)n * SGX_FINISH_ROW, g_defer_npre);
+        SGX_LAUNCH_CHECK("wgrad_prereduce_multi_kernel");
+    }
+    for (size_t L = 0; L < g_defer_launches.size(); ++L) {
+        const FinishLaunch& fl = g_defer_launches[L];
+        SGX_NOTE(0.0, L == 0 ? g_defer_bytes : 0.0, "finish_multi n%d of %d L%d", fl.n, n, (int)L);
+        hipLaunchKernelGGL(wgrad_finish_multi_kernel, dim3(fl.blocks), dim3(256), 0, st, tab, fl.lo, fl.n);
+        SGX_LAUNCH_CHECK("wgrad_finish_multi_kernel");
+    }
+    g_defer_rows.clear(); g_defer_launches.clear();
+    g_defer_npre = g_defer_planned = 0; g_defer_pre_blocks = 0; g_defer_bytes = 0.0;
     return 0;
 }
 
diff --git a/stylegan/pytorch_amd/functional.py b/stylegan/pytorch_amd/functional.py
--- a/stylegan/pytorch_amd/functional.py
+++ b/stylegan/pytorch_amd/functional.py
@@ -1,4 +1,5 @@
 import contextlib
+import ctypes
 import functools
 import os
 import weakref
@@ -23,6 +24,21 @@
         _DATA_GRAD_ONLY -= 1
 
 
+NO_IMAGE_GRAD = os.environ.get("SGX_NO_IMAGE_GRAD", "1") != "0"
+_NO_IMAGE_GRAD = 0
+
+
+@contextlib.contextmanager
+def no_image_grad():
+    global _NO_IMAGE_GRAD
+    on = 1 if NO_IMAGE_GRAD else 0
+    _NO_IMAGE_GRAD += on
+    try:
+        yield
+    finally:
+        _NO_IMAGE_GRAD -= on
+
+
 def _c(t):
     return t if t.is_contiguous() else t.contiguous()
 
@@ -88,12 +104,12 @@
 def _param_grads(mode, adjoint, x, gy, weight, scale, want_bias, into):
     side = _PARAM_GRAD_STREAM
     if side is None:
-        return _wgrad_param(mode, adjoint, x, gy, weight, scale, want_bias, into)
+        return _wgrad_param(mode, adjoint, x, gy, weight, scale, want_bias, into, True)
     if not _FAST_FORK:
         cur = torch.cuda.current_stream()
         side.wait_stream(cur)
         with torch.cuda.stream(side):
-            dW, db = _wgrad_param(mode, adjoint, x, gy, weight, scale, want_bias, into)
+            dW, db = _wgrad_param(mode, adjoint, x, gy, weight, scale, want_bias, into, True)
         for t in (x, gy):
             t.record_stream(side)
         for t in (dW, db):
@@ -102,12 +118,12 @@
         return dW, db
     cur_raw = N.stream()
     if side.cuda_stream == cur_raw:
-        return _wgrad_param(mode, adjoint, x, gy, weight, scale, want_bias, into)
+        return _wgrad_param(mode, adjoint, x, gy, weight, scale, want_bias, into, True)
     cur = _stream_of(cur_raw)
     N.check(N.lib().sgx_stream_wait_stream(side.cuda_stream, cur_raw), "sgx_stream_wait_stream")
     _set_stream(stream_id=side.stream_id, device_index=side.device_index, device_type=side.device_type)
     try:
-        dW, db = _wgrad_param(mode, adjoint, x, gy, weight, scale, want_bias, into)
+        dW, db = _wgrad_param(mode, adjoint, x, gy, weight, scale, want_bias, into, True)
     finally:
         _set_stream(stream_id=cur.stream_id, device_index=cur.device_index, device_type=cur.device_type)
     x.record_stream(side); gy.record_stream(side)
@@ -137,14 +153,61 @@
         t.record_stream(cur)
 
 
+WGRAD_DEFER = os.environ.get("SGX_WGRAD_DEFER", "1") != "0"
+_DEFER_ACTIVE = False
+_DEFER_PENDING = []
+
+
+def flush_param_grads():
+    global _DEFER_ACTIVE
+    if not _DEFER_ACTIVE:
+        return
+    _DEFER_ACTIVE = False
+    L = N.lib()
+    try:
+        n = L.sgx_wgrad_defer_pending()
+        if n == 0:
+            return
+        host = torch.empty((n * (N.FINISH_ROW + N.PRE_ROW),), dtype=torch.int64)
+        counts = (ctypes.c_int * 4)()
+        N.check(L.sgx_wgrad_defer_plan(host.data_ptr(), host.numel(), ctypes.addressof(counts)), "sgx_wgrad_defer_plan")
+        host = host[:counts[3]]
+        device = _DEFER_PENDING[0].device
+
+        def launch():
+            table, _ = N.upload(host, device)
+            N.check(L.sgx_wgrad_defer_flush(N.ptr(table), N.stream()), "sgx_wgrad_defer_flush")
+            if not N.capturing():
+                table.record_stream(torch.cuda.current_stream())
+        side, cur_raw = _PARAM_GRAD_STREAM, N.stream()
+        if side is None or side.cuda_stream == cur_raw:
+            launch()
+        else:
+            _fork_to(side, cur_raw, launch)
+    finally:
+        L.sgx_wgrad_defer(0)
+        del _DEFER_PENDING[:]
+
+
 @contextlib.contextmanager
 def accumulate_param_grads():
-    global _ACCUM_PARAM_GRADS
+    global _ACCUM_PARAM_GRADS, _DEFER_ACTIVE
     prev, _ACCUM_PARAM_GRADS = _ACCUM_PARAM_GRADS, True
+    defer = WGRAD_DEFER and GRAD_NOTE is None and not _DEFER_ACTIVE and not prev
+    if defer:
+        N.check(N.lib().sgx_wgrad_defer(1), "sgx_wgrad_defer")
+        del _DEFER_PENDING[:]
+        _DEFER_ACTIVE = True
     try:
         yield
+        if defer:
+            flush_param_grads()
     finally:
         _ACCUM_PARAM_GRADS = prev
+        if defer and _DEFER_ACTIVE:
+            _DEFER_ACTIVE = False
+            N.lib().sgx_wgrad_defer(0)
+            del _DEFER_PENDING[:]
 
 
 def bump_weight_generation(params=None):
@@ -309,8 +372,14 @@
     return y
 
 
-def _wgrad_param(mode, adjoint, x, gy, weight, scale, want_bias=False, into=None):
+def _wgrad_param(mode, adjoint, x, gy, weight, scale, want_bias=False, into=None, defer=False):
     L = N.lib()
+    if _DEFER_ACTIVE and not defer:
+        L.sgx_wgrad_defer(2)
+        try:
+            return _wgrad_param(mode, adjoint, x, gy, weight, scale, want_bias, into, True)
+        finally:
+            L.sgx_wgrad_defer(3)
     O, I = weight.shape[0], weight.shape[1]
     acc_w = into is not None and into[0] is not None
     acc_b = want_bias and into is not None and into[1] is not None
@@ -325,6 +394,8 @@
         ws = N.workspace(wsb, x.device)
         N.check(L.sgx_wgrad3x3_param(N.ptr(x), N.ptr(gy), N.ptr(dW), N.ptr(db), N.ptr(ws), wsb, B, H, W, Cx, Cdy, int(adjoint),
                                      float(scale), O, I, acc, N.dt(x), N.stream()), "sgx_wgrad3x3_param")
+        if _DEFER_ACTIVE:
+            _DEFER_PENDING.extend((ws, dW) if db is None else (ws, dW, db))
         return dW, db
     launched = ADJ_GEO[mode] if adjoint else FWD_GEO[mode]
     fine, coarse = (x, gy) if launched == "D" else (gy, x)
@@ -334,6 +405,8 @@
     ws = N.workspace(wsb, x.device)
     N.check(L.sgx_wgrad4x4s2_param(N.ptr(fine), N.ptr(coarse), N.ptr(dW), N.ptr(db), N.ptr(ws), wsb, B, H, W, Cf, Cc, MODES[mode],
                                    float(scale), O, I, acc, N.dt(x), N.stream()), "sgx_wgrad4x4s2_param")
+    if _DEFER_ACTIVE:
+        _DEFER_PENDING.extend((ws, dW) if db is None else (ws, dW, db))
     return dW, db
 
 
@@ -697,7 +770,7 @@
         img, w0, b0, wr, br = ctx.saved_tensors
         s0, sr = ctx.cfg
         gz = _c(gz)
-        gi = _bcall(RgbConvAdjFn, gz, w0, wr, br, s0, sr) if ctx.needs_input_grad[0] else None
+        gi = _bcall(RgbConvAdjFn, gz, w0, wr, br, s0, sr) if ctx.needs_input_grad[0] and not _NO_IMAGE_GRAD else None
         gw0 = gb0 = gwr = gbr = None
         if not _DATA_GRAD_ONLY:
             gw0, gb0, gwr, gbr = _bcall_wgrad(img, gz, True, w0, b0, wr, br, s0, sr, ctx.needs_input_grad[1:5])
@@ -970,7 +1043,7 @@
         bits, alpha_dev, pimg, wr = ctx.saved_tensors[6:10]
         alpha, beta, ws, bs = ctx.fade
         br = ctx.br_ref()
-        need_img = ctx.needs_input_grad[3]
+        need_img = ctx.needs_input_grad[3] and not (_NO_IMAGE_GRAD and not torch.is_grad_enabled())
         want_w = ctx.needs_input_grad[4] and not _DATA_GRAD_ONLY
         want_b = br is not None and ctx.needs_input_grad[5] and not _DATA_GRAD_ONLY
         gpimg = gwr = gbr = None
@@ -1356,6 +1429,8 @@
 
     @staticmethod
     def backward(ctx, gx, gy):
+        if _NO_IMAGE_GRAD and not torch.is_grad_enabled():
+            return None, None
         if gy is None:
             return gx, None
         if gx is None:
@@ -1394,7 +1469,7 @@
         img, weight = ctx.saved_tensors
         g = _c(g)
         gi = gw = gb = None
-        if ctx.needs_input_grad[0]:
+        if ctx.needs_input_grad[0] and not (_NO_IMAGE_GRAD and not torch.is_grad_enabled()):
             gi = _bcall(RgbOutFn, g, weight, None, ctx.wscale)
         if not _DATA_GRAD_ONLY:
             if ctx.needs_input_grad[1]:
@@ -2057,11 +2132,12 @@
     def forward(ctx, x, u, bits, img_bits=None):
         ctx.save_for_backward(u, img_bits)
         ctx.bits = bits
+        ctx.set_materialize_grads(False)
         return _diffaug(x, u, bits, False, True, img_bits)
 
     @staticmethod
     def backward(ctx, g):
-        if not ctx.needs_input_grad[0]:
+        if g is None or not ctx.needs_input_grad[0] or (_NO_IMAGE_GRAD and not torch.is_grad_enabled()):
             return None, None, None, None
         u, img_bits = ctx.saved_tensors
         return _bcall(DiffAugAdjFn, g, u, ctx.bits, img_bits), None, None, None
diff --git a/stylegan/pytorch_amd/native.py b/stylegan/pytorch_amd/native.py
--- a/stylegan/pytorch_amd/native.py
+++ b/stylegan/pytorch_amd/native.py
@@ -13,6 +13,7 @@
 ACT_NONE, ACT_LRELU, ACT_RELU = 0, 1, 2
 EPI_ACT, EPI_NORM = 1, 2
 PACK_S, PACK_D, PACK_U, PACK_UF = 0, 1, 2, 3
+FINISH_ROW, PRE_ROW = 16, 6
 
 _lib = None
 _lock = threading.Lock()
@@ -43,6 +44,10 @@
     "sgx_pack_weight_blocks": (I, [I, I]),
     "sgx_wgrad3x3_param": (I, [P, P, P, P, P, Z, I, I, I, I, I, I, F, I, I, I, I, P]),
     "sgx_wgrad4x4s2_param": (I, [P, P, P, P, P, Z, I, I, I, I, I, I, F, I, I, I, I, P]),
+    "sgx_wgrad_defer": (I, [I]),
+    "sgx_wgrad_defer_pending": (I, []),
+    "sgx_wgrad_defer_plan": (I, [P, I, P]),
+    "sgx_wgrad_defer_flush": (I, [P, P]),
     "sgx_bias_act": (I, [P, P, F, P, Z, I, I, I, P]),
     "sgx_lrelu_bwd": (I, [P, P, P, Z, F, F, P, I, P]),
     "sgx_lrelu_bwd_bits": (I, [P, P, P, Z, F, F, P, I, P]),
```

After: 284.4 img/s (median of 6 runs). Within noise of the previous version (+1.0%).
